# marlam/wurblpt

Measured on AMD Instinct MI355X. Metric: Msamples/s, higher is better.
Workload: dtype f32; 1 GPU; cornell_1024x1024_1024spp_ggx_glass; width=1024, height=1024, spp=1024, triangles=36, bvh_nodes=71, parallelism=1 launch

## Files before the change

### include/wurblpt_hip.h

```cpp
#ifndef WURBLPT_HIP_H
#define WURBLPT_HIP_H

#include <stdint.h>
#include <stddef.h>

#ifdef __cplusplus
extern "C" {
#endif

#define WPT_ABI_VERSION 5u

typedef enum {
    WPT_OK = 0,
    WPT_ERR_INVALID_ARGUMENT = 1,
    WPT_ERR_NO_DEVICE = 2,
    WPT_ERR_HIP = 3,
    WPT_ERR_UNSUPPORTED = 4,
    WPT_ERR_OUT_OF_MEMORY = 5
} wpt_status;


enum { WPT_NODE_INNER = 0, WPT_NODE_TRIANGLE = 1, WPT_NODE_SPHERE = 2, WPT_NODE_EMPTY = 3 };
typedef struct wpt_bvh_node {
    float lo[3];
// ... 392 lines not shown
wpt_status wpt_postproc_host(int op, const float* rgb_host, void* out_host, uint64_t pixels, float a, float b);

#define WPT_DENOISE_MAX_ITERATIONS 8u
#define WPT_DENOISE_MAX_NORMAL_LOG2 16u
typedef struct wpt_denoise_params {
    float sigma_l;
    float sigma_z;
    uint32_t normal_log2;
    uint32_t iterations;
} wpt_denoise_params;
wpt_status wpt_postproc_denoise(const float* frame_device, const float* moments_device, const uint16_t* samples_sqrt_device,
        const float* positions_device, const float* normals_device, const int32_t* materials_device, uint32_t width, uint32_t height,
        const wpt_denoise_params* params, float* out_device, float* variance_device, void* hip_stream);
wpt_status wpt_postproc_denoise_host(const float* frame_host, const float* moments_host, const uint16_t* samples_sqrt_host,
        const float* positions_host, const float* normals_host, const int32_t* materials_host, uint32_t width, uint32_t height,
        const wpt_denoise_params* params, float* out_host, float* variance_host);
const char* wpt_postproc_denoise_form(uint32_t step);

wpt_status wpt_first_hit_colours_device(wpt_scene* scene, const wpt_camera* camera, const wpt_params* params, uint32_t width,
        uint32_t height, float* albedo_device, float* emission_device, void* const guide_device[3], void* hip_stream);
wpt_status wpt_first_hit_colours(wpt_scene* scene, const wpt_camera* camera, const wpt_params* params, uint32_t width, uint32_t height,
        float* albedo_host, float* emission_host, void* const guide_host[3]);

wpt_status wpt_postproc_denoise_demodulated(const float* frame_device, const float* moments_device, const uint16_t* samples_sqrt_device,
        const float* positions_device, const float* normals_device, const int32_t* materials_device, const float* albedo_device,
        const float* emission_device, uint32_t width, uint32_t height, const wpt_denoise_params* params, float albedo_floor,
        float* out_device, float* variance_device, void* hip_stream);
wpt_status wpt_postproc_denoise_demodulated_host(const float* frame_host, const float* moments_host, const uint16_t* samples_sqrt_host,
        const float* positions_host, const float* normals_host, const int32_t* materials_host, const float* albedo_host,
        const float* emission_host, uint32_t width, uint32_t height, const wpt_denoise_params* params, float albedo_floor,
        float* out_host, float* variance_host);

#define WPT_TEMPORAL_HISTORY_BYTES_PER_PIXEL 48u
typedef struct wpt_temporal_params {
    float max_history;
    float normal_cos_min;
    float position_tolerance;
    uint32_t reserved;
} wpt_temporal_params;
wpt_status wpt_postproc_temporal_accumulate(const float* frame_device, const float* moments_device, const uint16_t* samples_sqrt_device,
        const float* positions_device, const float* normals_device, const int32_t* materials_device,
        const float* pixel_offset_to_prev_device, const float* camera_offset_to_prev_device, const void* history_prev_device,
        uint32_t width, uint32_t height, const wpt_temporal_params* params, void* history_out_device, float* length_out_device,
        void* hip_stream);
wpt_status wpt_postproc_temporal_accumulate_host(const float* frame_host, const float* moments_host, const uint16_t* samples_sqrt_host,
        const float* positions_host, const float* normals_host, const int32_t* materials_host, const float* pixel_offset_to_prev_host,
        const float* camera_offset_to_prev_host, const void* history_prev_host, uint32_t width, uint32_t height,
        const wpt_temporal_params* params, void* history_out_host, float* length_out_host);
wpt_status wpt_postproc_denoise_history(const void* history_device, uint32_t width, uint32_t height, const wpt_denoise_params* params,
        float* out_device, float* variance_device, void* hip_stream);
wpt_status wpt_postproc_denoise_history_host(const void* history_host, uint32_t width, uint32_t height, const wpt_denoise_params* params,
        float* out_host, float* variance_host);

wpt_status wpt_postproc_resample(const float* image_device, uint32_t width, uint32_t height, uint32_t components, uint32_t new_width,
        uint32_t new_height, float* out_device, void* hip_stream);
wpt_status wpt_postproc_resample_host(const float* image_host, uint32_t width, uint32_t height, uint32_t components, uint32_t new_width,
        uint32_t new_height, float* out_host);
wpt_status wpt_postproc_lens_warp(const float* image_device, uint32_t width, uint32_t height, uint32_t components, const wpt_camera* camera,
        int forward, float* out_device, void* hip_stream);
wpt_status wpt_postproc_lens_warp_host(const float* image_host, uint32_t width, uint32_t height, uint32_t components, const wpt_camera* camera,
        int forward, float* out_host);
wpt_status wpt_postproc_despeckle(const float* rgb_device, uint32_t width, uint32_t height, uint32_t components, float min_factor,
        float* out_device, void* hip_stream);
wpt_status wpt_postproc_despeckle_host(const float* rgb_host, uint32_t width, uint32_t height, uint32_t components, float min_factor,
        float* out_host);
wpt_status wpt_postproc_distance_to_coords(const float* distances_device, uint32_t width, uint32_t height, uint32_t components,
        const wpt_camera* camera, int pmd_space, float* coords_device, void* hip_stream);
wpt_status wpt_postproc_distance_to_coords_host(const float* distances_host, uint32_t width, uint32_t height, uint32_t components,
        const wpt_camera* camera, int pmd_space, float* coords_host);
const char* wpt_postproc_despeckle_form(void);
wpt_status wpt_set_despeckle_form(int form);
void wpt_postproc_image_ops_tile(uint32_t* width, uint32_t* height);

wpt_status wpt_set_launch_config(uint32_t threads_per_group, uint32_t variant);
wpt_status wpt_set_top_nodes(uint32_t nodes);
#define WPT_WALK_WIDE 1u
#define WPT_WALK_FULL_SHADOW 2u
#define WPT_WALK_COUNT_PRODUCT 4u
#define WPT_WALK_TRIANGLES_AS_GIVEN 8u
#define WPT_WALK_SELECT_CORNERS 16u
#define WPT_WALK_NO_FOLD 32u
#define WPT_WALK_NO_BYPASS 64u
#define WPT_WALK_SMALL_WORKGROUPS 128u
wpt_status wpt_set_walk(uint32_t flags);
wpt_status wpt_scene_folded_links(const wpt_scene* scene, uint32_t* folded);
wpt_status wpt_fold_plan(const wpt_scene_desc* desc, uint32_t* folded, uint32_t* lds_words);
wpt_status wpt_scene_bypassed_nodes(const wpt_scene* scene, uint32_t* count);
wpt_status wpt_bypass_plan(const wpt_scene_desc* desc, uint32_t* count, uint32_t* words);
wpt_status wpt_set_bypass(uint32_t mode);
#define WPT_SLICES_DECLINE_ODD 0x100u
wpt_status wpt_slices_plan(uint32_t block_size, uint32_t lanes_at_once, uint32_t samples_sqrt, uint32_t* units, uint32_t* rows);
wpt_status wpt_set_slices(uint32_t n);
wpt_status wpt_last_slice_stats(uint64_t* taken, uint64_t* continued);
wpt_status wpt_set_wavefront(uint32_t mode, uint32_t groups, uint32_t chunk, uint32_t flags);

#define WPT_SCHED_STATS 72
wpt_status wpt_set_scheduler_stats(unsigned long long* stats_device);

const char* wpt_kernel_name(void);
const char* wpt_kernel_form(void);
uint32_t wpt_kernel_workgroup(uint32_t* ordered_boxes);
wpt_status wpt_kernel_choice(uint32_t need, uint32_t sensor, uint32_t count, uint32_t node_count, uint32_t tri_count, uint32_t material_count,
        uint32_t scene_has_wide, uint32_t variant, uint32_t walk, const char** name, const char** form, uint32_t key[4],
        uint64_t* scene_lds_bytes, uint32_t* materials_in_lds);
wpt_status wpt_kernel_table_entry(uint32_t index, uint32_t key[4], const char** name);
enum { WPT_PLAN_WAVEFRONT, WPT_PLAN_WAVEFRONT_FALLS_BACK, WPT_PLAN_POOLED, WPT_PLAN_STRATEGY, WPT_PLAN_UNITS, WPT_PLAN_ROWS, WPT_PLAN_PASSES,
    WPT_PLAN_WORDS };
enum { WPT_STRATEGY_ONE_PASS, WPT_STRATEGY_TWO_PASSES, WPT_STRATEGY_ADAPTIVE_ORDER, WPT_STRATEGY_SLICED };
wpt_status wpt_launch_plan(uint32_t sensor, uint32_t count, uint32_t need, uint32_t scene_in_lds, uint32_t block_size, uint32_t samples_sqrt,
        uint32_t cu_count, uint32_t variant, uint32_t wavefront_mode, uint32_t slices, uint32_t plan[WPT_PLAN_WORDS]);
const char* wpt_device_name(int device);
uint32_t wpt_last_render_passes(void);
const char* wpt_build_info(void);

const char* wpt_last_error(void);

#ifdef __cplusplus
}
#endif

#endif
```

### wurblpt_amd/_abi.py

```python
import ctypes as C

WPT_ABI_VERSION = 5
WPT_OK = 0

NODE_INNER, NODE_TRIANGLE, NODE_SPHERE, NODE_EMPTY = 0, 1, 2, 3
MATF_TOF_LIGHT = 16
TOF_MAX_PHASES = 8
LIGHT_GROUPS_MAX, LIGHT_GROUP_NONE = 255, 0xff
VIEWS_MAX_PIXELS = 0x7fffffff
SPLIT_PIXELS_PER_LANE = 4
MAT_NONE, MAT_LAMBERTIAN, MAT_LIGHT_DIFFUSE, MAT_MIRROR, MAT_GGX, MAT_GLASS, MAT_MODPHONG, MAT_TWOSIDED, MAT_RGL, MAT_LIGHT_SPOT = range(10)


class BvhNode(C.Structure):
    _fields_ = [("lo", C.c_float * 3), ("hi", C.c_float * 3), ("link", C.c_uint32), ("kind", C.c_uint32)]


class TriGeom(C.Structure):
    _fields_ = [("v0", C.c_float * 3), ("instance", C.c_uint32), ("v1", C.c_float * 3), ("material", C.c_uint32),
                ("v2", C.c_float * 3), ("flags", C.c_uint32)]


class TriAttr(C.Structure):
    _fields_ = [("n0", C.c_float * 3), ("n1", C.c_float * 3), ("n2", C.c_float * 3),
# ... 156 lines not shown
    "wpt_scene_bypassed_nodes": (_I, [_P, _pU]),
    "wpt_render_block_device": (_I, _SCP + [_U] * 5 + [_P] * 3),
    "wpt_render_block": (_I, _SCP + [_U] * 5 + [_P]),
    "wpt_render_bands_device": (_I, [_P] * 3 + [_U] * 6 + [_P] * 3),
    "wpt_render_bands": (_I, [_P] * 3 + [_U] * 6 + [_P]),
    "wpt_render_transient_block_device": (_I, _SCP + [_P] + [_U] * 6 + [_P] * 3),
    "wpt_render_transient_block": (_I, _SCP + [_P] + [_U] * 6 + [_P] * 2),
    "wpt_render_light_groups_block_device": (_I, _SCP + [_P] + [_U] * 8 + [_P] * 3),
    "wpt_render_light_groups_block": (_I, _SCP + [_P] + [_U] * 8 + [_P] * 2),
    "wpt_render_tof_block_device": (_I, _SCP + [_TOF] + [_U] * 5 + [_P] * 2),
    "wpt_render_tof_block": (_I, _SCP + [_TOF] + [_U] * 5 + [_P]),
    "wpt_tof_accumulate_host": (_I, [_TOF, _U, _F, _F, _I, _P]),
    "wpt_render_views_device": (_I, [_P, _CAM, _U, _PAR, _U, _U, _U] + [_P] * 3),
    "wpt_render_views": (_I, [_P, _CAM, _U, _PAR, _U, _U, _U, _P]),
    "wpt_render_view_streams_device": (_I, [_P, _CAM, _P, _U, _PAR, _U, _U, _U] + [_P] * 3),
    "wpt_render_view_streams": (_I, [_P, _CAM, _P, _U, _PAR, _U, _U, _U, _P]),
    "wpt_render_split_device": (_I, _SCP + [_U] * 5 + [_P] * 4),
    "wpt_render_split": (_I, _SCP + [_U] * 5 + [_P] * 2),
    "wpt_split_plan": (_I, [_Q, _U, _U, _pU, _pU]),
    "wpt_render_adaptive_block_device": (_I, _SCP + [_U, _U, _P, _U, _U] + [_P] * 3),
    "wpt_render_adaptive_block": (_I, _SCP + [_U, _U, _P, _U, _U] + [_P] * 2),
    "wpt_ground_truth_device": (_I, [_P] * 6 + [_U, _U, _P, _P]),
    "wpt_ground_truth": (_I, [_P] * 6 + [_U, _U, _P]),
    "wpt_first_hit_colours_device": (_I, [_P] * 3 + [_U, _U] + [_P] * 4),
    "wpt_first_hit_colours": (_I, [_P] * 3 + [_U, _U] + [_P] * 3),
    "wpt_progress_covers": (_I, [_U, _U, _U]),
    "wpt_progress_begin": (_I, _SCP + [_U] * 5 + [_Q, _pP]),
    "wpt_progress_advance_device": (_I, [_P, _U, _P, _P]),
    "wpt_progress_advance": (_I, [_P, _U, _P]),
    "wpt_progress_rows_done": (_U, [_P]),
    "wpt_progress_rows_total": (_U, [_P]),
    "wpt_progress_preview_device": (_I, [_P, _P, _P]),
    "wpt_progress_preview": (_I, [_P, _P]),
    "wpt_progress_end": (None, [_P]),
    "wpt_progress_state_bytes": (_I, [_P, _pQ]),
    "wpt_progress_save": (_I, [_P, _P, _Q]),
    "wpt_progress_restore": (_I, [_P, _P, _Q, _CAM, _PAR, _Q, _pP]),
    "wpt_progress_state_info": (_I, [_P, _Q, C.POINTER(ProgressInfo)]),
    "wpt_postproc_to_srgb": (_I, [_P, _P, _Q, _P]),
    "wpt_postproc_max_luminance": (_I, [_P, _Q, _P, _P]),
    "wpt_postproc_uniform_rational_quantization": (_I, [_P, _P, _Q, _F, _F, _P]),
    "wpt_postproc_scale_luminance": (_I, [_P, _P, _Q, _F, _F, _P]),
    "wpt_postproc_host": (_I, [_I, _P, _P, _Q, _F, _F]),
    "wpt_postproc_mix_planes": (_I, [_P, _U, _Q, _Q, _P, _P, _P]),
    "wpt_postproc_mix_planes_host": (_I, [_P, _U, _Q, _Q, _P, _P]),
    "wpt_postproc_mean_planes": (_I, [_P, _U, _Q, _Q, _P, _P, _P]),
    "wpt_postproc_mean_planes_host": (_I, [_P, _U, _Q, _Q, _P, _P]),
    "wpt_postproc_merge_means": (_I, [_P, _U, _P, _U, _Q, _P, _P]),
    "wpt_postproc_merge_means_host": (_I, [_P, _U, _P, _U, _Q, _P]),
    "wpt_postproc_denoise": (_I, [_P] * 6 + [_U, _U, _DEN] + [_P] * 3),
    "wpt_postproc_denoise_host": (_I, [_P] * 6 + [_U, _U, _DEN] + [_P] * 2),
    "wpt_postproc_denoise_form": (_S, [_U]),
    "wpt_postproc_denoise_demodulated": (_I, [_P] * 8 + [_U, _U, _DEN, _F] + [_P] * 3),
    "wpt_postproc_denoise_demodulated_host": (_I, [_P] * 8 + [_U, _U, _DEN, _F] + [_P] * 2),
    "wpt_postproc_temporal_accumulate": (_I, [_P] * 9 + [_U, _U, _TMP] + [_P] * 3),
    "wpt_postproc_temporal_accumulate_host": (_I, [_P] * 9 + [_U, _U, _TMP] + [_P] * 2),
    "wpt_postproc_denoise_history": (_I, [_P, _U, _U, _DEN] + [_P] * 3),
    "wpt_postproc_denoise_history_host": (_I, [_P, _U, _U, _DEN] + [_P] * 2),
    "wpt_postproc_resample": (_I, [_P] + [_U] * 5 + [_P, _P]),
    "wpt_postproc_resample_host": (_I, [_P] + [_U] * 5 + [_P]),
    "wpt_postproc_lens_warp": (_I, _WARP + [_P]),
    "wpt_postproc_lens_warp_host": (_I, _WARP),
    "wpt_postproc_distance_to_coords": (_I, _WARP + [_P]),
    "wpt_postproc_distance_to_coords_host": (_I, _WARP),
    "wpt_postproc_despeckle": (_I, [_P, _U, _U, _U, _F, _P, _P]),
    "wpt_postproc_despeckle_host": (_I, [_P, _U, _U, _U, _F, _P]),
    "wpt_postproc_despeckle_form": (_S, []),
    "wpt_postproc_image_ops_tile": (None, [_pU, _pU]),
    "wpt_set_despeckle_form": (_I, [_I]),
    "wpt_set_launch_config": (_I, [_U, _U]),
    "wpt_set_wavefront": (_I, [_U] * 4),
    "wpt_set_walk": (_I, [_U]),
    "wpt_set_top_nodes": (_I, [_U]),
    "wpt_set_slices": (_I, [_U]),
    "wpt_set_bypass": (_I, [_U]),
    "wpt_set_scheduler_stats": (_I, [_P]),
    "wpt_slices_plan": (_I, [_U, _U, _U, _pU, _pU]),
    "wpt_last_slice_stats": (_I, [_pQ, _pQ]),
    "wpt_fold_plan": (_I, [_P, _pU, _P]),
    "wpt_bypass_plan": (_I, [_P, _pU, _P]),
    "wpt_kernel_name": (_S, []),
    "wpt_kernel_form": (_S, []),
    "wpt_kernel_workgroup": (_U, [_pU]),
    "wpt_kernel_choice": (_I, [_U] * 9 + [_pS, _pS, _pU, _pQ, _pU]),
    "wpt_kernel_table_entry": (_I, [_U, _pU, _pS]),
    "wpt_launch_plan": (_I, [_U] * 10 + [_pU]),
    "wpt_last_render_passes": (_U, []),
}

TEST_HOOK_FUNCTIONS = {
    "wpt_selftest_math": (_I, [_I, _I, _P, _P, _P]),
    "wpt_selftest_aabb": (_I, [_I, _P, _P, _P]),
    "wpt_selftest_triangle": (_I, [_I, _I, _P, _P]),
    "wpt_selftest_rayaux": (_I, [_I, _P, _P]),
    "wpt_selftest_sphere": (_I, [_I, _P, _P, _P]),
    "wpt_selftest_hits": (_I, [_P, _I, _P, _P]),
    "wpt_selftest_hits_host": (_I, [_P, _I, _P, _P]),
    "wpt_scene_get_envmap_tables": (_I, [_P] * 4),
}
```

### wurblpt_amd/csrc/wpt_blocks.h

```cpp
#ifndef WPT_BLOCKS_H
#define WPT_BLOCKS_H

#include "wpt_device.h"
#include "wpt_lens.h"
#include "wpt_tof.h"

namespace wptk {

using namespace wptd;

constexpr uint32_t NO_HIT = 0xffffffffu;

enum { RAY_PATH = 0, RAY_NEE_LIGHT = 1, RAY_NEE_ENV = 2, RAY_PATH_WAITED = 3  };
enum { NEXT_TRACE = 0, NEXT_NEW = 1, NEXT_DONE = 2, NEXT_WAIT = 3, NEXT_HANDED_ON = 4  };

enum { SEC_NODE_STEP = 0, SEC_LEAF_TEST, SEC_BEGIN_RAY, SEC_MISS, SEC_HIT_RECORD, SEC_SCATTER_LAMBERT, SEC_SCATTER_GGX, SEC_SCATTER_GLASS, SEC_SCATTER_OTHER,
       SEC_EMISSION, SEC_LIGHT_SAMPLE, SEC_PDF_SETUP, SEC_PDF_LIGHT, SEC_EVAL_LAMBERT, SEC_EVAL_GGX, SEC_EVAL_OTHER, SEC_NEE_SETUP, SEC_ADVANCE, SEC_NEE_END,
       SEC_NEE_END_LIGHT, SEC_NEW_SAMPLE, SEC_PIXEL_DONE, SEC_LOOK, SEC_LOOK_INNER, SEC_COUNT };

struct LaneCounters {
    uint32_t rays, nodes, leaves, pdfs, scatters;
    unsigned long long shadeClock[8];
    uint32_t secWave[SEC_COUNT], secLane[SEC_COUNT];
};
// ... 166 lines not shown
    return make_float4(faceNormal.x, faceNormal.y, faceNormal.z, faceArea);
}

template<bool FACE>
WPT_D float hotSpotPdfValue(float4 g0, float4 g1, float4 g2, f3 org, f3 dir, const RayAux& h, float4 face)
{
    const f3 v0 = mk3(g0.x, g0.y, g0.z), v1 = mk3(g1.x, g1.y, g1.z), v2 = mk3(g2.x, g2.y, g2.z);
    Candidate c;
    float value = 0.0f;
    if (triangleTest(v0, v1, v2, org, h, 0.0f, k_maxval, c)) {
        if (!FACE)
            face = hotSpotFace(v0, v1, v2);
        float cosine = __builtin_fabsf(dot(mk3(face.x, face.y, face.z), neg(dir)));
        float distance_squared = c.a * c.a;
        value = distance_squared / (cosine * face.w);
    }
    return value;
}

WPT_D float hotSpotPdfValueRotated(float4 g0, float4 g1, float4 g2, f3 orgR, f3 dir, const RayAux& h, float4 face)
{
    Candidate c;
    float value = 0.0f;
    if (triangleTestRotated(mk3(g0.x, g0.y, g0.z), mk3(g1.x, g1.y, g1.z), mk3(g2.x, g2.y, g2.z), orgR, h.Sx, h.Sy, h.inv.x,
            (uint32_t)h.k & (uint32_t)RAY_FLIP, 0.0f, k_maxval, c)) {
        float cosine = __builtin_fabsf(dot(mk3(face.x, face.y, face.z), neg(dir)));
        float distance_squared = c.a * c.a;
        value = distance_squared / (cosine * face.w);
    }
    return value;
}
WPT_D uint32_t rotatedCopyOffset(int kz, uint32_t triCount) { return (kz == 2 ? 0u : (uint32_t)(kz + 1)) * (3u * triCount); }

WPT_CALL float spherePdfValue(const wpt_sphere& sp, const wpt_sphere& spHit, f3 org, f3 dir)
{
    const f3 cmo = sub(ld3(sp.center), org);
    const float distanceSquared = dot(cmo, cmo);
    const float radiusSquared = sp.radius * sp.radius;
    float value = 0.0f;
    if (distanceSquared <= radiusSquared) {
        value = 0.25f * k_inv_pi;
    } else {
        float a;
        if (sphereTest(spHit, org, dir, 0.0f, k_maxval, a)) {
            const float discriminant = 1.0f - radiusSquared / distanceSquared;
            const float cosThetaMax = discriminant > 0.0f ? __builtin_sqrtf(discriminant) : 0.0f;
            const float solidAngle = 2.0f * k_pi * (1.0f - cosThetaMax);
            value = 1.0f / solidAngle;
        }
    }
    return value;
}

struct DirectionDraw {
    f3 dir;
    Prng prng;
};
WPT_CALL DirectionDraw sphereDirection(const wpt_sphere& sp, f3 org, Prng prng)
{
    DirectionDraw r;
    const f3 cmo = sub(ld3(sp.center), org);
    const float distanceSquared = dot(cmo, cmo);
    const float radiusSquared = sp.radius * sp.radius;
    if (distanceSquared <= radiusSquared) {
        r.dir = onUnitSphere(in01x2(prng));
    } else {
        const float discriminant = 1.0f - radiusSquared / distanceSquared;
        const float cosThetaMax = discriminant > 0.0f ? __builtin_sqrtf(discriminant) : 0.0f;
        r.dir = toSphere(normalize(cmo), cosThetaMax, in01x2(prng));
    }
    r.prng = prng;
    return r;
}

template<uint32_t F, bool COUNT, class Tri4>
WPT_D void hotSpotsMeanPdfPair(const SceneView& sv, Tri4 tri4, f3 org, f3 dirA, f3 dirB, PathHot& ps, LaneCounters& lc, float& meanA, float& meanB)
{
    if constexpr ((F & FEAT_ROTATED) != 0) {
        auto meanPdf = [&](f3 dir) {
            const RayAux h = rayAuxRotated<true>(dir);
            const f3 orgR = rotated(org, auxKz(h));
            const uint32_t off = rotatedCopyOffset(auxKz(h), sv.triCount);
            float sum = 0.0f;
            for (uint32_t i = 0; i < sv.hotspotCount; i++) {
                const uint32_t p = off + 3 * sv.hotspots[i].prim;
                sum += hotSpotPdfValueRotated(tri4(p), tri4(p + 1), tri4(p + 2), orgR, dir, h, sv.hotspotFace[i]);
            }
            return sum * here(sv.invHotspotCount);
        };
        meanA = meanPdf(dirA);
        meanB = meanPdf(dirB);
        return;
    }
    const RayAux hA = rayAux<true>(dirA), hB = rayAux<true>(dirB);
    float sumA = 0.0f, sumB = 0.0f;
    for (uint32_t i = 0; i < sv.hotspotCount; i++) {
        sec<COUNT>(lc, SEC_PDF_LIGHT);
        const uint32_t p = sv.hotspots[i].prim;
        if ((F & FEAT_SPHERES) && sv.hotspots[i].kind == WPT_HOTSPOT_SPHERE) {
            const wpt_sphere& sp = sv.spheres[p];
            if ((F & FEAT_ANIM) && sp.animation >= 0) {
                const wptanim::Trs T = animationTrs(sv, ps, sp.animation);
                const wpt_sphere forPdf = sphereMovedForPdf(sp, T), moved = sphereMoved(sp, T);
                sumA += spherePdfValue(forPdf, moved, org, dirA);
                sumB += spherePdfValue(forPdf, moved, org, dirB);
            } else {
                sumA += spherePdfValue(sp, sp, org, dirA);
                sumB += spherePdfValue(sp, sp, org, dirB);
            }
        } else if ((F & FEAT_ANIM) && sv.hotspots[i].animation >= 0) {
            float4 g0 = tri4(3 * p), g1 = tri4(3 * p + 1), g2 = tri4(3 * p + 2);
            const float* animationM = animationMatrix(sv, ps, sv.hotspots[i].animation);
            const f3 v0 = animatePoint(animationM, mk3(g0.x, g0.y, g0.z)), v1 = animatePoint(animationM, mk3(g1.x, g1.y, g1.z)),
                     v2 = animatePoint(animationM, mk3(g2.x, g2.y, g2.z));
            g0.x = v0.x; g0.y = v0.y; g0.z = v0.z;
            g1.x = v1.x; g1.y = v1.y; g1.z = v1.z;
            g2.x = v2.x; g2.y = v2.y; g2.z = v2.z;
            sumA += hotSpotPdfValue<false>(g0, g1, g2, org, dirA, hA, g0);
            sumB += hotSpotPdfValue<false>(g0, g1, g2, org, dirB, hB, g0);
        } else {
            const float4 g0 = tri4(3 * p), g1 = tri4(3 * p + 1), g2 = tri4(3 * p + 2), face = sv.hotspotFace[i];
            sumA += hotSpotPdfValue<true>(g0, g1, g2, org, dirA, hA, face);
            sumB += hotSpotPdfValue<true>(g0, g1, g2, org, dirB, hB, face);
        }
        if (COUNT)
            lc.pdfs += 2;
    }
    meanA = sumA * here(sv.invHotspotCount);
    meanB = sumB * here(sv.invHotspotCount);
}

template<class PS> WPT_D void accumulateRadiance(const wpt_params& par, f3 opl, float distanceToLight, f4 radiance, PS& ps)
{
    const bool dOk = distanceToLight >= par.min_dist_to_light && distanceToLight <= par.max_dist_to_light;
    if (!dOk)
        return;
    Slot acc = ps.get(SLOT_ACC);
    if (opl.x >= par.min_path_len && opl.x <= par.max_path_len)
        acc.x += radiance.x;
    if (opl.y >= par.min_path_len && opl.y <= par.max_path_len)
        acc.y += radiance.y;
    if (opl.z >= par.min_path_len && opl.z <= par.max_path_len)
        acc.z += radiance.z;
    ps.set3(SLOT_ACC, mk3(acc.x, acc.y, acc.z));
}

struct BinsView {
    const float* edges;
    float* bins;
    size_t stride;
    uint32_t binCount;
    uint32_t width;
    float guessScale;
    uint32_t rule;
};
enum : uint32_t {
    BINS_BY_EMITTER = 0x100u,
    BINS_GROUP_NONE = 0xffu
};

WPT_D int binOf(const BinsView& b, float x)
{
    const uint32_t K = b.binCount;
    if (!(x >= b.edges[0] && x < b.edges[K]))
        return -1;
    const float g = __builtin_fminf((x - b.edges[0]) * b.guessScale, (float)(K - 1));
    uint32_t k = (uint32_t)g;
    if (!(b.edges[k] <= x && x < b.edges[k + 1])) {
        uint32_t lo = 0, hi = K;
// ... 259 lines not shown
        }
        return NEXT_NEW;
    }
    Ray ray;
    ray.o = ps.o;
    ray.d = ps.d;
    ray.ri = ps.get4(SLOT_RI);
    const Slot oplSlot = ps.get(SLOT_OPL);
    const uint32_t pathComponent = oplSlot.w;
    const f3 opl = add(mk3(oplSlot.x, oplSlot.y, oplSlot.z), scl(best.a, sensorChannels<F>(ray.ri)));
    if (!(pathComponent + 1 < par.max_path_components))
        return NEXT_NEW;
    long long tSection = 0;
    auto section = [&](int k) {
        if (COUNT) {
            const long long now = clock64();
            lc.shadeClock[k] += (unsigned long long)(now - tSection);
            tSection = now;
        }
    };
    if (COUNT)
        tSection = clock64();
    sec<COUNT>(lc, SEC_HIT_RECORD);
    Hit h = finishHit<F>(sv, best, ray.o, ray.d, ps.time, tri4);
    const wpt_material& m = resolveMaterial<F>(sv, h.material, h);
    if ((F & ~(FEAT_GGX | FEAT_GLASS | FEAT_TRANSIENT | FEAT_ADAPTIVE | FEAT_ROTATED | FEAT_SLICED | ((F & FEAT_TOF) ? (FEAT_TOF | FEAT_SPOT | FEAT_TWOSIDED) : 0u))) == 0 && waitBelow > 0) {
        const bool waited = ps.rayKind == RAY_PATH_WAITED;
        const unsigned long long here = __ballot(true);
        bool wait = false;
        for (uint32_t kind = WPT_MAT_LAMBERTIAN; kind <= WPT_MAT_RGL; kind++) {
            if (kind == WPT_MAT_LIGHT_DIFFUSE || kind == WPT_MAT_TWOSIDED)
                continue;
            const unsigned long long lanes = __ballot(m.type == kind);
            if (lanes != 0 && lanes != here && __popcll(lanes) < waitBelow && __ballot(m.type == kind && waited) == 0 && m.type == kind)
                wait = true;
        }
        if (wait) {
            ps.rayKind = RAY_PATH_WAITED;
            return NEXT_WAIT;
        }
    }
    ps.set3(SLOT_OPL, opl);
    if (COUNT)
        lc.scatters++;
    section(0);
    sec<COUNT>(lc, SEC_SCATTER_LAMBERT, m.type == WPT_MAT_LAMBERTIAN);
    sec<COUNT>(lc, SEC_SCATTER_GGX, m.type == WPT_MAT_GGX);
    sec<COUNT>(lc, SEC_SCATTER_GLASS, m.type == WPT_MAT_GLASS || m.type == WPT_MAT_MIRROR);
    sec<COUNT>(lc, SEC_SCATTER_OTHER, m.type != WPT_MAT_LAMBERTIAN && m.type != WPT_MAT_GGX && m.type != WPT_MAT_GLASS && m.type != WPT_MAT_MIRROR && m.type != WPT_MAT_LIGHT_DIFFUSE
            && !((F & FEAT_SPOT) && m.type == WPT_MAT_LIGHT_SPOT));
    sec<COUNT>(lc, SEC_EMISSION);
    Prng prng = loadPrng(ps);
#ifdef WPT_MATERIAL_CACHE
    MatCache mc = matCacheEmpty();
    const Scatter sr = materialScatter<F>(sv, m, ray, h, prng, mc);
#else
    MatCache mcScatter = matCacheEmpty(), mc = matCacheEmpty();
    const Scatter sr = materialScatter<F>(sv, m, ray, h, prng, mcScatter);
#endif
    section(1);
    const f4 att = ps.get4(SLOT_ATT);
    {
        f4 rad = mul(att, materialEmitted<F>(sv, m, h, ray.d));
        accumulate<F>(par, bins, opl, (pathComponent == 0 ? 0.0f : h.a), rad, ps, isTofLight<F>(m), emitterOf<F>(m), sv.materials);
    }
    section(2);
    if (sr.type == SCATTER_NONE) {
        storePrng(ps, prng);
        return NEXT_NEW;
    }
    f4 nextAtt = mul(att, sr.att);
    if (sr.type == SCATTER_RANDOM) {
        if (sr.pdf > 0.0f)
            nextAtt = divs(nextAtt, sr.pdf);
        else
            nextAtt = mk4(0.0f, 0.0f, 0.0f, 0.0f);
    }
    sec<COUNT>(lc, SEC_LIGHT_SAMPLE, sr.type == SCATTER_RANDOM && sv.hotspotCount > 0);
    if (sr.type == SCATTER_RANDOM && sv.hotspotCount > 0) {
        uint32_t idx = (uint32_t)(in01(prng) * (float)sv.hotspotCount);
        idx = idx < sv.hotspotCount - 1 ? idx : sv.hotspotCount - 1;
        const wpt_hotspot& hs = sv.hotspots[idx];
        f3 directDir;
        uint32_t hotSpotPrim = hs.prim;
        if ((F & FEAT_SPHERES) && hs.kind == WPT_HOTSPOT_SPHERE) {
            const DirectionDraw draw = sphereDirection(sphereNow<F>(sv, ps, sv.spheres[hs.prim]), h.p, prng);
            directDir = draw.dir;
            prng = draw.prng;
            hotSpotPrim = PRIM_SPHERE | hs.prim;
        } else {
            const f3 bary = inTriangle(in01x2(prng));
            f3 p = add(add(scl(bary.x, ld3(hs.p0)), scl(bary.y, ld3(hs.p1))), scl(bary.z, ld3(hs.p2)));
            if (hs.transform)
                p = mat4mulPoint(hs.M, p);
            if ((F & FEAT_ANIM) && hs.animation >= 0)
                p = animatePoint(animationMatrix(sv, ps, hs.animation), p);
            directDir = normalize(sub(p, h.p));
        }
        section(4);
        float hotSpotsPdf, directPdf;
        sec<COUNT>(lc, SEC_PDF_SETUP);
        hotSpotsMeanPdfPair<F, COUNT>(sv, tri4, h.p, sr.dir, directDir, ps, lc, hotSpotsPdf, directPdf);
        nextAtt = sclr(nextAtt, powerHeuristicWeight(sr.pdf, hotSpotsPdf));
        section(5);
        sec<COUNT>(lc, SEC_EVAL_LAMBERT, directPdf > 0.0f && m.type == WPT_MAT_LAMBERTIAN);
        sec<COUNT>(lc, SEC_EVAL_GGX, directPdf > 0.0f && m.type == WPT_MAT_GGX);
        sec<COUNT>(lc, SEC_EVAL_OTHER, directPdf > 0.0f && m.type != WPT_MAT_LAMBERTIAN && m.type != WPT_MAT_GGX);
        if (directPdf > 0.0f) {
            float dpdf;
            f4 directAtt;
            materialEval<F>(sv, m, ray, h, directDir, directAtt, dpdf, mc);
            sec<COUNT>(lc, SEC_NEE_SETUP, dpdf > 0.0f);
            if (dpdf > 0.0f) {
                const f4 neeFactor = sclr(divs(mul(att, directAtt), directPdf), powerHeuristicWeight(directPdf, dpdf));
                const f3 neeChannels = sensorChannels<F>(neeFactor);
                Slot nee;
                nee.x = neeChannels.x; nee.y = neeChannels.y; nee.z = neeChannels.z;
                nee.w = hotSpotPrim;
                ps.set(SLOT_NEE, nee);
                if (MERGED) {
                    ps.set3(SLOT_NEXTATT, opl);
                    ps.set3(SLOT_SRDIR, mk3(ray.ri.x, ray.ri.y, ray.ri.z));
                    ps.neeO = h.p;
                    ps.neeD = directDir;
                    ps.neeKind = RAY_NEE_LIGHT;
                } else {
                    ps.set4(SLOT_NEXTATT, nextAtt);
                    ps.set3(SLOT_SRDIR, sr.dir);
                    storePrng(ps, prng);
                    ps.o = h.p;
                    ps.d = directDir;
                    ps.rayKind = RAY_NEE_LIGHT;
                    section(6);
                    return NEXT_TRACE;
                }
            }
        }
    } else if ((F & FEAT_ENVMAP) && sr.type == SCATTER_RANDOM && haveEnv && sv.envN > 0) {
        const float lightsP = envP(sv, sr.dir);
        nextAtt = sclr(nextAtt, powerHeuristicWeight(sr.pdf, lightsP));
        const f3 lightDir = envD(sv, prng);
        const float directPdf = envP(sv, lightDir);
        float dpdf;
        f4 directAtt;
        materialEval<F>(sv, m, ray, h, lightDir, directAtt, dpdf, mc);
        if (dpdf > 0.0f) {
            const f4 neeFactor = sclr(divs(mul(att, directAtt), directPdf), powerHeuristicWeight(directPdf, dpdf));
            ps.set3(SLOT_NEE, sensorChannels<F>(neeFactor));
            if (MERGED) {
                ps.neeO = h.p;
                ps.neeD = lightDir;
                ps.neeKind = RAY_NEE_ENV;
            } else {
                ps.set4(SLOT_NEXTATT, nextAtt);
                ps.set3(SLOT_SRDIR, sr.dir);
                storePrng(ps, prng);
                ps.o = h.p;
                ps.d = lightDir;
                ps.rayKind = RAY_NEE_ENV;
                section(7);
                return NEXT_TRACE;
            }
        }
    }
    sec<COUNT>(lc, SEC_ADVANCE);
    ps.o = h.p;
    if (sr.type == SCATTER_EXPLICIT)
        ps.set4(SLOT_RI, sr.ri);
    const int next = advancePath(par, ps, nextAtt, sr.dir, pathComponent, prng);
    storePrng(ps, prng);
    section(7);
    return next;
}

template<uint32_t F, class Tri4, class PS>
WPT_D int blockNeeEnd(const SceneView& sv, const wpt_params& par, Tri4 tri4, PS& ps, const Candidate& best, const BinsView& bins = BinsView{})
{
    const Slot oplSlot = ps.get(SLOT_OPL);
    if (ps.rayKind == RAY_NEE_LIGHT) {
        const Slot nee = ps.get(SLOT_NEE);
// ... 53 lines not shown
```

### wurblpt_amd/csrc/wpt_capi.hip

```cpp
#include <atomic>
#include <cstring>

#include "wpt_capi_common.h"
#include "wpt_scene_layout.h"
#include "wpt_leaf_words.h"
#include "wpt_streams.h"

using namespace wptd;
using namespace wptk;
using namespace wptc;

namespace {

thread_local std::string g_error;

std::atomic<uint32_t> g_lastPasses{1};
std::atomic<const char*> g_kernelName{nullptr};
std::atomic<const char*> g_kernelForm{""};

std::atomic<unsigned long long*> g_lastSliceStats{nullptr};

std::atomic<uint32_t> g_lastWorkgroup{uint32_t(WG)};

static_assert(wptk::PLAN_WG == uint32_t(WG) && wptk::PLAN_SLICE_SLOT_MAX == wptk::SLICE_SLOT_MASK && wptk::SLICE_UNITS_TARGET <= wptk::SLICE_UNITS_MAX
        && wptk::PLAN_FRAME == wptk::SENSOR_FRAME && wptk::PLAN_VIEWS == wptk::SENSOR_VIEWS && wptk::PLAN_ADAPTIVE == wptk::SENSOR_ADAPTIVE
        && wptk::PLAN_SENSORS == wptk::SENSOR_COUNT, "wpt_launch_plan.h restates the kernels' constants and the sensors");
static_assert(wptl::NODE_CHILD == NODE_CHILD && wptl::NODE_INDEX_MASK == NODE_INDEX_MASK && wptl::PRIM_SPHERE == PRIM_SPHERE && wptl::WIDE_STACK == WIDE_STACK
        && wptl::WIDE_NONE == WIDE_NONE && wptl::LDS_SCENE_MAX_BYTES == LDS_SCENE_MAX_BYTES && wptl::ORDERED_COPIES == wptk::ORDERED_COPIES,
        "wpt_scene_layout.h restates the kernels' node words and limits");
static_assert(wptw::LEAF_NODE_SHIFT == wptk::LEAF_NODE_SHIFT && wptw::LEAF_NODE_MAX == wptk::LEAF_NODE_MAX && wptw::LEAF_CORNER_MASK == wptk::LEAF_CORNER_MASK
        && LDS_SCENE_MAX_BYTES / 32 <= wptw::LEAF_NODE_MAX && LDS_SCENE_MAX_BYTES / 16 <= wptw::LEAF_CORNER_MASK,
        "wpt_leaf_words.h restates the rotated kernels' leaf word, which has room for every tree that fits LDS");

}

namespace wptc {

Settings settings;

wpt_status fail(wpt_status s, const std::string& msg)
{
    g_error = msg;
    return s;
}

void recordLaunch(const char* name, const char* form, uint32_t passes, unsigned long long* sliceStats)
{
    g_kernelName.store(name, std::memory_order_relaxed);
    g_kernelForm.store(form, std::memory_order_relaxed);
    g_lastPasses.store(passes, std::memory_order_relaxed);
    g_lastSliceStats.store(sliceStats, std::memory_order_relaxed);
    g_lastWorkgroup.store(uint32_t(WG), std::memory_order_relaxed);
}

void recordWorkgroup(uint32_t lanes, bool orderedBoxes)
{
    g_lastWorkgroup.store(lanes | (orderedBoxes ? 0x80000000u : 0u), std::memory_order_relaxed);
}

const char* kernelForm(bool rotated, uint32_t units, bool leafLinksFromNodes)
{
    static const std::vector<std::string> forms = [] {
        std::vector<std::string> f;
        for (int r = 0; r < 3; r++)
            for (uint32_t u = 0; u <= wptk::SLICE_UNITS_MAX; u++)
                f.push_back(std::string(r ? "rotated corners" : "") + (r == 2 ? ", leaf links from the nodes" : "")
                        + (u > 1 ? ", sliced x" + std::to_string(u) : std::string()));
        return f;
    }();
    return forms[(rotated ? (leafLinksFromNodes ? 2 : 1) * (wptk::SLICE_UNITS_MAX + 1) : 0) + (units <= wptk::SLICE_UNITS_MAX ? units : 0)].c_str();
}

wpt_status lookupKernel(uint32_t features, bool count, bool ldsScene, bool wide, const wptk::KernelEntry** entry)
{
    *entry = wptk::findKernel(features, count, ldsScene, wide);
    if (!*entry)
        return fail(WPT_ERR_UNSUPPORTED, "the library has no kernel wpt_pathtrace<F = " + std::to_string(features) + ", COUNT = " + std::to_string(count)
                + ", LDSSCENE = " + std::to_string(ldsScene) + ", WIDE = " + std::to_string(wide) + ">");
    return WPT_OK;
}

}

extern "C" {

int wpt_device_count(void)
{
    int n = 0;
    hipError_t e = hipGetDeviceCount(&n);
    if (e != hipSuccess) {
        g_error = std::string("hipGetDeviceCount: ") + hipGetErrorString(e);
        return 0;
    }
    return n;
}

wpt_status wpt_select_device(int device)
{
    HIP_TRY(hipSetDevice(device));
    return WPT_OK;
}

wpt_status wpt_current_device(int* device)
{
    if (!device)
        return fail(WPT_ERR_INVALID_ARGUMENT, "device is NULL");
    HIP_TRY(hipGetDevice(device));
    return WPT_OK;
}

const char* wpt_device_name(int device)
{
    thread_local std::string name;
    name.clear();
    hipDeviceProp_t prop;
    if (hipGetDeviceProperties(&prop, device) == hipSuccess)
        name = std::string(prop.name) + " (" + prop.gcnArchName + ", " + std::to_string(prop.multiProcessorCount) + " CUs)";
    return name.c_str();
}

wpt_status wpt_device_lanes(int device, uint32_t* lanes)
{
    if (!lanes)
        return fail(WPT_ERR_INVALID_ARGUMENT, "device lanes: NULL argument");
    hipDeviceProp_t prop;
    HIP_TRY(hipGetDeviceProperties(&prop, device));
    *lanes = uint32_t(prop.multiProcessorCount) * 1024u;
    return WPT_OK;
}

const char* wpt_build_info(void)
{
#if defined(__clang_version__)
    return "hipcc / clang " __clang_version__ ", --offload-arch=gfx950 -O3 -ffp-contract=off -fhip-fp32-correctly-rounded-divide-sqrt "
           "-fno-gpu-flush-denormals-to-zero";
#else
    return "unknown compiler";
#endif
}

const char* wpt_last_error(void)
{
    return g_error.c_str();
}

const char* wpt_kernel_name(void)
{
    const char* name = g_kernelName.load(std::memory_order_relaxed);
    return name ? name : "wpt_pathtrace";
}

const char* wpt_kernel_form(void)
{
    return g_kernelForm.load(std::memory_order_relaxed);
}

uint32_t wpt_kernel_workgroup(uint32_t* ordered_boxes)
{
    const uint32_t w = g_lastWorkgroup.load(std::memory_order_relaxed);
    if (ordered_boxes)
        *ordered_boxes = w >> 31;
    return w & 0x7fffffffu;
}

uint32_t wpt_last_render_passes(void)
{
    return g_lastPasses.load(std::memory_order_relaxed);
}

wpt_status wpt_last_slice_stats(uint64_t* taken, uint64_t* continued)
{
    if (!taken || !continued)
        return fail(WPT_ERR_INVALID_ARGUMENT, "NULL argument");
    *taken = 0;
    *continued = 0;
    const unsigned long long* stats = g_lastSliceStats.load(std::memory_order_relaxed);
    if (!stats)
        return WPT_OK;
    unsigned long long host[2] = { 0, 0 };
    HIP_TRY(hipDeviceSynchronize());
    HIP_TRY(hipMemcpy(host, stats, sizeof(host), hipMemcpyDeviceToHost));
    *taken = host[0];
    *continued = host[1];
    return WPT_OK;
}

wpt_status wpt_set_launch_config(uint32_t threads_per_group, uint32_t variant)
{
    if (threads_per_group != 0 && threads_per_group != WG)
        return fail(WPT_ERR_UNSUPPORTED, "this build uses 256 threads per workgroup");
    settings.threadsPerGroup = WG;
    settings.variant = variant & 0xffu;
    settings.leaveEighths = 0;
    settings.heavyMin = 0;
    settings.leafBias = 0;
    if ((variant >> 8) & 0xffu)
        settings.leaveEighths = ((variant >> 8) & 0xffu) - 1;
    if ((variant >> 16) & 0xffu)
        settings.heavyMin = ((variant >> 16) & 0xffu) - 1;
    if ((variant >> 24) & 0xffu)
        settings.leafBias = (variant >> 24) & 0xffu;
    return WPT_OK;
}

wpt_status wpt_set_wavefront(uint32_t mode, uint32_t groups, uint32_t chunk, uint32_t flags)
{
    if (mode > 2u)
        return fail(WPT_ERR_INVALID_ARGUMENT, "wavefront mode must be 0, 1 or 2");
    settings.wfMode = mode;
    settings.wfConfig.groups = groups & 0xffu;
    settings.wfConfig.tracePerCu = (groups >> 8) & 0xffu;
    settings.wfConfig.shadePerKind = (groups >> 16) & 1u;
    settings.wfConfig.chunk = chunk;
    settings.wfConfig.buckets = (flags & 1u) ? 0u : 1u;
    settings.wfConfig.refillIdle = (flags >> 8) & 0x3fu;
    settings.wfConfig.leafBias = 0;
    settings.wfConfig.stepBudget = (flags >> 16) == 0xffffu ? 0xffffffffu : (flags >> 16);
    settings.wfConfig.topNodes = ((flags >> 1) & 0x7fu) == 0x7fu ? 0xffffffffu : ((flags >> 1) & 0x7fu) * 128u;
    return WPT_OK;
}

wpt_status wpt_set_top_nodes(uint32_t nodes)
{
    settings.topNodes = nodes & 0x7fffffffu;
    return WPT_OK;
}

wpt_status wpt_set_walk(uint32_t flags)
{
    if (flags & ~(WPT_WALK_WIDE | WPT_WALK_FULL_SHADOW | WPT_WALK_COUNT_PRODUCT | WPT_WALK_TRIANGLES_AS_GIVEN | WPT_WALK_SELECT_CORNERS | WPT_WALK_NO_FOLD | WPT_WALK_NO_BYPASS
            | WPT_WALK_SMALL_WORKGROUPS))
        return fail(WPT_ERR_INVALID_ARGUMENT, "unknown walk flag");
    settings.walk = flags;
    return WPT_OK;
}

wpt_status wpt_set_slices(uint32_t n)
{
    if ((n & ~WPT_SLICES_DECLINE_ODD) > wptk::SLICE_UNITS_MAX)
        return fail(WPT_ERR_INVALID_ARGUMENT, "slices: 0 (the library's plan), 1 (never) or 2 .. 15 units, with or without WPT_SLICES_DECLINE_ODD");
    settings.slices = n;
    return WPT_OK;
}

wpt_status wpt_set_bypass(uint32_t mode)
{
    if (mode > wptb::MODE_ALL_ELIGIBLE)
        return fail(WPT_ERR_INVALID_ARGUMENT, "bypass mode: 0 (the cost model's choice) or 1 (every eligible inner node)");
    settings.bypassMode = mode;
    return WPT_OK;
}

wpt_status wpt_set_scheduler_stats(unsigned long long* stats_device)
{
    settings.schedStats = stats_device;
    return WPT_OK;
}

wpt_status wpt_slices_plan(uint32_t block_size, uint32_t lanes_at_once, uint32_t samples_sqrt, uint32_t* units, uint32_t* rows)
{
    if (!units || !rows)
        return fail(WPT_ERR_INVALID_ARGUMENT, "NULL argument");
    wptk::slicesPlan(block_size, lanes_at_once, samples_sqrt, units, rows);
    return WPT_OK;
}

wpt_status wpt_kernel_choice(uint32_t need, uint32_t sensor, uint32_t count, uint32_t node_count, uint32_t tri_count, uint32_t material_count,
        uint32_t scene_has_wide, uint32_t variant, uint32_t walk, const char** name, const char** form, uint32_t key[4],
        uint64_t* scene_lds_bytes, uint32_t* materials_in_lds)
{
    if (!name || !form || !key || !scene_lds_bytes || !materials_in_lds)
        return fail(WPT_ERR_INVALID_ARGUMENT, "NULL argument");
    if (sensor >= wptk::SENSOR_COUNT)
        return fail(WPT_ERR_INVALID_ARGUMENT, "sensor: 0 frame, 1 transient, 2 views, 3 adaptive, 4 time of flight");
    const wptk::KernelChoice choice = wptk::selectKernel({ need, wptk::Sensor(sensor), count != 0, node_count, tri_count, material_count,
            scene_has_wide != 0, variant, walk });
    const wptk::KernelEntry* kernel = nullptr;
    const wpt_status found = lookupKernel(choice.features, choice.count, choice.ldsScene, choice.wide, &kernel);
    if (found != WPT_OK)
        return found;
    *name = kernel->name;
    *form = kernelForm(choice.rotated);
    key[0] = kernel->features;
    key[1] = kernel->count;
    key[2] = kernel->ldsScene;
    key[3] = kernel->wide;
    *scene_lds_bytes = choice.sceneLdsBytes;
    *materials_in_lds = choice.materialsInLds;
    return WPT_OK;
}

wpt_status wpt_launch_plan(uint32_t sensor, uint32_t count, uint32_t need, uint32_t scene_in_lds, uint32_t block_size, uint32_t samples_sqrt,
        uint32_t cu_count, uint32_t variant, uint32_t wavefront_mode, uint32_t slices, uint32_t plan[WPT_PLAN_WORDS])
{
    if (!plan)
        return fail(WPT_ERR_INVALID_ARGUMENT, "NULL argument");
    if (sensor >= wptk::SENSOR_COUNT)
        return fail(WPT_ERR_INVALID_ARGUMENT, "sensor: 0 frame, 1 transient, 2 views, 3 adaptive, 4 time of flight");
    if (wavefront_mode > 2u)
        return fail(WPT_ERR_INVALID_ARGUMENT, "wavefront mode must be 0, 1 or 2");
    const wptk::LaunchPlan p = wptk::planLaunch({ sensor, count != 0, (need & FEAT_RGL) != 0, (need & FEAT_ANIM) != 0, scene_in_lds != 0,
            block_size, samples_sqrt, cu_count, variant, wavefront_mode, slices });
    const uint32_t words[WPT_PLAN_WORDS] = { p.wavefront, p.wavefrontFallBack, p.pooled, p.strategy, p.units, p.rows, p.passes };
    memcpy(plan, words, sizeof(words));
    return WPT_OK;
}

wpt_status wpt_kernel_table_entry(uint32_t index, uint32_t key[4], const char** name)
{
    if (!key || !name)
        return fail(WPT_ERR_INVALID_ARGUMENT, "NULL argument");
    if (index >= wptk::KERNEL_TABLE_ROWS)
        return fail(WPT_ERR_INVALID_ARGUMENT, "the kernel table has " + std::to_string(wptk::KERNEL_TABLE_ROWS) + " rows");
    const wptk::KernelEntry& k = wptk::KERNEL_TABLE[index];
// ... 19 lines not shown
```

### wurblpt_amd/csrc/wpt_capi_common.h

```cpp
#ifndef WPT_CAPI_COMMON_H
#define WPT_CAPI_COMMON_H

#include <hip/hip_runtime.h>

#include <cassert>
#include <cstdint>
#include <string>
#include <vector>

#include "../../include/wurblpt_hip.h"
#ifndef WPT_CAPI_OUTPUT_SIDE
#include "wpt_kernel_table.h"
#include "wpt_launch_plan.h"
#include "wpt_wavefront.inc.h"
#include "wpt_bypass.h"
#endif

namespace wptc __attribute__((visibility("hidden"))) {

wpt_status fail(wpt_status s, const std::string& msg);

#define HIP_TRY(expr)                                                                              \
    do {                                                                                           \
        hipError_t e_ = (expr);                                                                    \
        if (e_ != hipSuccess)                                                                      \
            return fail(WPT_ERR_HIP, std::string(#expr) + ": " + hipGetErrorString(e_));           \
    } while (0)
#define WPT_TRY(expr)                                                                              \
    do {                                                                                           \
        const wpt_status s_ = (expr);                                                              \
        if (s_ != WPT_OK)                                                                          \
            return s_;                                                                             \
    } while (0)

inline wpt_status hipStatus(const char* what, hipError_t e, bool oomToo = false)
{
    if (e == hipSuccess)
        return WPT_OK;
    return fail(oomToo && e == hipErrorOutOfMemory ? WPT_ERR_OUT_OF_MEMORY : WPT_ERR_HIP, std::string(what) + ": " + hipGetErrorString(e));
}

inline bool overlaps(const void* a, size_t bytesA, const void* b, size_t bytesB)
{
    const uintptr_t x = reinterpret_cast<uintptr_t>(a), y = reinterpret_cast<uintptr_t>(b);
    return x < y + bytesB && y < x + bytesA;
}

struct StreamScratch {
    hipStream_t stream;
    void* held[5] = {};
    uint32_t count = 0;
    explicit StreamScratch(hipStream_t s) : stream(s) {}
    StreamScratch(const StreamScratch&) = delete;
    ~StreamScratch()
    {
        for (uint32_t i = 0; i < count; i++)
            (void)hipFreeAsync(held[i], stream);
    }
    template<typename T> hipError_t get(size_t n, T** p)
    {
        assert(count < sizeof(held) / sizeof(held[0]));
        const hipError_t e = hipMallocAsync(reinterpret_cast<void**>(p), n * sizeof(T), stream);
        if (e == hipSuccess)
            held[count++] = *p;
        return e;
    }
    template<typename T> T* get(size_t n)
    {
        T* p = nullptr;
        if (get(n, &p) != hipSuccess) {
            (void)hipGetLastError();
            return nullptr;
        }
        return p;
    }
};

#ifndef WPT_CAPI_OUTPUT_SIDE

}

struct wpt_scene {
    int device;
    wptd::SceneView view;
    uint32_t features;
    uint32_t nodeCount, triCount;
    uint32_t foldedLinks;
    uint32_t* ldsLinks = nullptr;
    bool leafOneToOne = false;
    const float4* orderedNodes = nullptr;
    uint32_t bypassedNodes = 0;
    uint32_t animationCount;
    std::vector<void*> allocations;
    int cuCount;
    std::vector<float> envM, envMcs;
    std::vector<int32_t> envMs;
};

namespace wptc __attribute__((visibility("hidden"))) {

struct Settings {
    uint32_t threadsPerGroup = wptk::WG;
    uint32_t variant = 0;
    uint32_t leaveEighths = 0;
    uint32_t heavyMin = 0;
    uint32_t leafBias = 0;
    uint32_t topNodes = 65536;
    unsigned long long* schedStats = nullptr;
    uint32_t wfMode = 0;
    wptk::WfConfig wfConfig = { 0, 0, 0, 1, 0, 0, 0, 0, 0 };
    uint32_t walk = 0;
    uint32_t bypassMode = wptb::MODE_MODEL;
    uint32_t slices = 0;
};
extern Settings settings;

void recordLaunch(const char* name, const char* form, uint32_t passes, unsigned long long* sliceStats);
void recordWorkgroup(uint32_t lanes, bool orderedBoxes);
const char* kernelForm(bool rotated, uint32_t units = 0, bool leafLinksFromNodes = false);
wpt_status lookupKernel(uint32_t features, bool count, bool ldsScene, bool wide, const wptk::KernelEntry** entry);

struct LaunchRequest {
    wpt_scene* scene;
    const wpt_camera* camera;
    const wpt_params* params;
    uint32_t width, height, samplesSqrt, blockStart, blockSize;
    float* frame;
    void* stream;
    wpt_counters* counters = nullptr;
    uint32_t bandPixels = 0, bandFirst = 0, bandStride = 0;
    wptk::Sensor sensor = wptk::SENSOR_FRAME;
    wptk::BinsView bins = {};
    wptk::ViewsView views = {};
    wptk::AdaptiveView adaptive = {};
};

wpt_status checkFrameBlock(uint32_t width, uint32_t height, const uint32_t* samplesSqrt, uint32_t blockStart, uint32_t blockSize,
        uint32_t frames = 1, const char* prefix = "", bool session = false);
wpt_status launchSetUp(const wpt_scene* scene, const wpt_camera* camera, uint32_t cameraCount, bool batch, const wpt_params* params,
        uint32_t width, uint32_t height, uint32_t samples_sqrt, uint32_t block_start, uint32_t block_size,
        uint32_t band_pixels, uint32_t band_first, uint32_t band_stride, bool count, wptk::KernelArgs& args, uint32_t& need);
hipError_t runSingleKernel(const wpt_scene* scene, wptk::KernelArgs& args, const wptk::KernelChoice& choice, const wptk::KernelEntry* kernel,
        const wptk::KernelEntry* slicedTwin, const wptk::LaunchPlan& plan, hipStream_t stream);
wpt_status renderLaunch(const LaunchRequest& rq);

constexpr size_t ORDER_WORK_WORDS = 3 * wptk::ORDER_BUCKETS + 1;

inline void orderByCost(const wptk::KernelArgs& measured, uint32_t* order, uint32_t* work, hipStream_t stream, wptk::KernelArgs& next)
{
    wptk::launchOrderBuild(measured, order, work, stream);
    next.order = order;
    next.orderCount = work + ORDER_WORK_WORDS - 1;
}

struct StagedBlock {
    void* device = nullptr;
    size_t bytes = 0;
    StagedBlock() = default;
    StagedBlock(const StagedBlock&) = delete;
    ~StagedBlock() { (void)hipFree(device); }
    hipError_t allocate(size_t n) { return hipMalloc(&device, bytes = n); }
    hipError_t allocatePixels(size_t pixels, size_t planes = 1) { return allocate(pixels * 3 * sizeof(float) * planes); }
    hipError_t upload(const void* host) { return hipMemcpy(device, host, bytes, hipMemcpyHostToDevice); }
    hipError_t download(void* host) const { return device ? hipMemcpy(host, device, bytes, hipMemcpyDeviceToHost) : hipSuccess; }
    float* biased(uint32_t blockStart) const { return device ? static_cast<float*>(device) - size_t(blockStart) * 3 : nullptr; }
};

inline wpt_status finishStaged(wpt_status launched, wpt_scene* check, const StagedBlock& a, void* hostA, const StagedBlock* b = nullptr, void* hostB = nullptr)
{
    const wpt_status st = launched == WPT_OK && check ? wpt_scene_check(check) : launched;
    hipError_t e = st == WPT_OK ? a.download(hostA) : hipSuccess;
    if (st == WPT_OK && e == hipSuccess && b)
        e = b->download(hostB);
    return e == hipSuccess ? st : hipStatus("hipMemcpy", e);
}

#endif

}

#endif
```

### wurblpt_amd/csrc/wpt_capi_render.hip

```cpp
#include <atomic>

#include "wpt_capi_common.h"
#include "wpt_leaf_words.h"

using namespace wptd;
using namespace wptk;
using namespace wptc;

namespace {

constexpr int SLICE_STATS_DEVICES = 64;
std::atomic<unsigned long long*> g_sliceStats[SLICE_STATS_DEVICES];

unsigned long long* sliceStatsOfCurrentDevice()
{
    int dev = 0;
    if (hipGetDevice(&dev) != hipSuccess || dev < 0 || dev >= SLICE_STATS_DEVICES)
        return nullptr;
    unsigned long long* p = g_sliceStats[dev].load(std::memory_order_acquire);
    if (!p) {
        if (hipMalloc(reinterpret_cast<void**>(&p), 2 * sizeof(unsigned long long)) != hipSuccess) {
            (void)hipGetLastError();
            return nullptr;
        }
// ... 76 lines not shown
    if ((session && blockSize == 0) || uint64_t(blockStart) + blockSize > uint64_t(width) * height * frames)
        return fail(WPT_ERR_INVALID_ARGUMENT, std::string(prefix) + (session ? "pixel block is empty or lies outside the frame"
                : "pixel block lies outside the frame"));
    return WPT_OK;
}

wpt_status launchSetUp(const wpt_scene* scene, const wpt_camera* camera, uint32_t cameraCount, bool batch, const wpt_params* params,
        uint32_t width, uint32_t height, uint32_t samples_sqrt, uint32_t block_start, uint32_t block_size,
        uint32_t band_pixels, uint32_t band_first, uint32_t band_stride, bool count, wptk::KernelArgs& args, uint32_t& need)
{
    args.bandPixels = band_pixels;
    args.bandFirst = band_first;
    args.bandStride = band_stride;
    args.sv = scene->view;
    args.cam = *camera;
    args.par = *params;
    args.width = width;
    args.height = height;
    args.samplesSqrt = samples_sqrt;
    args.invWidth = 1.0f / float(width);
    args.invHeight = 1.0f / float(height);
    args.invSamplesSqrt = 1.0f / float(samples_sqrt);
    args.invSamples = 1.0f / float(samples_sqrt * samples_sqrt);
    args.blockStart = block_start;
    args.blockSize = block_size;
    args.fuse = (settings.variant & 0x20u) ? 0u : 1u;

    args.tiled = (width % 8 == 0 && block_start % width == 0 && block_size % (8 * width) == 0
            && (band_stride == 0 || band_pixels % (8 * width) == 0)) ? 1u : 0u;
    if (batch)
        args.tiled = (width % 8 == 0 && height % 8 == 0) ? 1u : 0u;
    need = scene->features;
    for (uint32_t v = 0; v < cameraCount; v++) {
        const wpt_camera* c = camera + v;
        need |= (c->lens_radius > 0.0f || c->distortion_type != WPT_DISTORTION_NONE || c->surround_mode != WPT_SURROUND_OFF
                || c->stereoscopic_distance > 0.0f) ? FEAT_LENS : 0u;
        if (c->surround_mode > WPT_SURROUND_360)
            return fail(WPT_ERR_UNSUPPORTED, "camera surround mode is not known to the kernel");
        if (c->distortion_type > WPT_DISTORTION_OPENCV)
            return fail(WPT_ERR_UNSUPPORTED, "lens distortion model is not known to the kernel");
        if (c->animation >= int32_t(scene->animationCount))
            return fail(WPT_ERR_INVALID_ARGUMENT, batch ? "camera " + std::to_string(v) + " refers to an animation outside the scene's array"
                    : std::string("camera refers to an animation outside the scene's array"));
        if (batch && c->animation >= 0)
            need |= FEAT_ANIM;
    }
    if (params->t0 != params->t1)
        need |= FEAT_ANIM;
    args.shadowWalksEnd = (settings.walk & WPT_WALK_FULL_SHADOW) ? 0u : (count ? ((settings.walk & WPT_WALK_COUNT_PRODUCT) ? 1u : 0u) : 1u);
    const bool smallScene = size_t(scene->nodeCount) * 32 + size_t(scene->triCount) * 48 <= LDS_SCENE_MAX_BYTES;
    args.leaveEighths = settings.leaveEighths ? (settings.leaveEighths > 8u ? 8u : settings.leaveEighths) : (smallScene ? 1u : 3u);
    args.heavyMin = settings.heavyMin ? settings.heavyMin : (smallScene ? 16u : 8u);
    args.leafBias = settings.leafBias ? settings.leafBias : (smallScene ? 16u : 32u);
    static const uint32_t waitBelowChoices[4] = { 6u, 0u, 3u, 12u };
    args.waitBelow = waitBelowChoices[(settings.variant >> 2) & 0x3u];
    args.cuCount = uint32_t(scene->cuCount);
    return WPT_OK;
}

hipError_t runSingleKernel(const wpt_scene* scene, wptk::KernelArgs& args, const wptk::KernelChoice& choice, const wptk::KernelEntry* kernel,
        const wptk::KernelEntry* slicedTwin, const wptk::LaunchPlan& plan, hipStream_t stream)
{
    StreamScratch scratch(stream);
    args.pool = plan.pooled ? scratch.get<uint32_t>(1) : nullptr;
    args.materialsInLds = choice.materialsInLds;
    if (choice.ldsScene) {
        if (!scene->ldsLinks)
            return hipErrorInvalidValue;
        const size_t words = 2 * size_t(scene->nodeCount) + 4;
        const bool fold = (choice.materialsInLds & wptk::LDS_FOLD) != 0;
        const bool bypass = fold && !(settings.walk & WPT_WALK_NO_BYPASS) && !args.sv.boxesMayBeNan;
        args.sv.spheres = reinterpret_cast<const wpt_sphere*>(scene->ldsLinks + (fold ? words : 0));
        args.sv.wideNodes = reinterpret_cast<const float4*>(scene->ldsLinks + (bypass ? 2 * words : fold ? words : 0));
        if (choice.rotated) {
            const size_t leafWords = wptw::leafWordsSize(scene->nodeCount, scene->triCount);
            const uint32_t* sets = scene->ldsLinks + 3 * words;
            args.sv.spheres = reinterpret_cast<const wpt_sphere*>(sets + (fold ? leafWords : 0));
            args.sv.wideNodes = reinterpret_cast<const float4*>(sets + (bypass ? 2 * leafWords : fold ? leafWords : 0));
            if (scene->leafOneToOne)
                args.materialsInLds |= wptk::LDS_LEAF_LINKS;
        }
    }
    size_t largeLdsBytes = 0;
    const bool large = wptk::selectLargeForm(choice, settings.walk, scene->orderedNodes != nullptr, args.sv.boxesMayBeNan != 0, scene->nodeCount, &largeLdsBytes);
    if (large && wptk::LARGE_ORDERED)
        args.sv.rglData = reinterpret_cast<const float*>(scene->orderedNodes);
    const SingleKernel run = large
            ? SingleKernel{ wptk::launchPathtraceLarge<FEAT_BASIC | FEAT_ROTATED>, dim3((args.blockSize + WG_LARGE - 1) / WG_LARGE), largeLdsBytes, stream }
            : SingleKernel{ kernel->launch, dim3((args.blockSize + WG - 1) / WG), choice.sceneLdsBytes, stream };
    bool done = false;
    unsigned long long* sliceStats = nullptr;
    if (args.pool && plan.strategy == wptk::TWO_PASSES)
        done = runTwoPasses(args, run, scratch);
    else if (args.pool && plan.strategy == wptk::ADAPTIVE_ORDER)
        done = runAdaptiveOrder(args, run, scratch);
    else if (args.pool && plan.strategy == wptk::SLICED)
        done = (sliceStats = runSliced(args, SingleKernel{ large ? wptk::launchPathtraceLarge<FEAT_BASIC | FEAT_ROTATED | FEAT_SLICED> : slicedTwin->launch, run.grid, run.sceneLdsBytes, stream },
                plan, scratch)) != nullptr;
    if (!done)
        run(args);
    recordLaunch(kernel->name, kernelForm(choice.rotated, sliceStats ? plan.units : 0, choice.rotated && !scene->leafOneToOne), done ? plan.passes : 1u,
            sliceStats);
    if (large)
        recordWorkgroup(WG_LARGE, wptk::LARGE_ORDERED);
    return hipGetLastError();
}

wpt_status renderLaunch(const LaunchRequest& rq)
{
    const bool planes = rq.sensor == wptk::SENSOR_TRANSIENT || rq.sensor == wptk::SENSOR_TOF, views = rq.sensor == wptk::SENSOR_VIEWS;
    if (!rq.scene || !rq.camera || !rq.params || !(rq.frame || planes))
        return fail(WPT_ERR_INVALID_ARGUMENT, "NULL argument");
    const uint32_t cameraCount = views ? rq.views.viewCount : 1u;
    const wpt_status checked = checkFrameBlock(rq.width, rq.height, &rq.samplesSqrt, rq.blockStart, rq.bandStride ? 0u : rq.blockSize, cameraCount);
    if (checked != WPT_OK || rq.blockSize == 0)
        return checked;
    KernelArgs args = {};
    uint32_t need = 0;
    const bool count = rq.counters != nullptr;
    WPT_TRY(launchSetUp(rq.scene, rq.camera, cameraCount, views, rq.params, rq.width, rq.height, rq.samplesSqrt, rq.blockStart,
            rq.blockSize, rq.bandPixels, rq.bandFirst, rq.bandStride, count, args, need));
    args.frame = rq.frame;
    args.counters = rq.counters;
    args.schedStats = settings.schedStats;
    if (views)
        args.views = rq.views;
    else if (rq.sensor == wptk::SENSOR_ADAPTIVE)
        args.adaptive = rq.adaptive;
    else if (planes)
        args.bins = rq.bins;
    args.rowStop = rq.samplesSqrt;
    const wptk::KernelChoice choice = wptk::selectKernel({ need, rq.sensor, count, rq.scene->nodeCount, rq.scene->triCount,
            uint32_t(rq.scene->view.materialCount), rq.scene->view.wideNodes != nullptr, settings.variant, settings.walk });
    const wptk::KernelEntry *kernel = nullptr, *slicedTwin = nullptr;
    wpt_status found = lookupKernel(choice.features, choice.count, choice.ldsScene, choice.wide, &kernel);
    if (found == WPT_OK && choice.sceneInLds && rq.sensor == wptk::SENSOR_FRAME && !count)
        found = lookupKernel(choice.features | FEAT_SLICED, choice.count, choice.ldsScene, choice.wide, &slicedTwin);
    if (found != WPT_OK)
        return found;
    const bool rgl = (need & FEAT_RGL) != 0;
    hipStream_t stream = static_cast<hipStream_t>(rq.stream);
    const wptk::LaunchPlan plan = wptk::planLaunch({ rq.sensor, count, rgl, (need & FEAT_ANIM) != 0, choice.sceneInLds, rq.blockSize, rq.samplesSqrt,
            uint32_t(rq.scene->cuCount), settings.variant, settings.wfMode, settings.slices });
    if (plan.wavefront) {
        uint32_t launches = 0;
        const hipError_t e = wptk::renderWavefront(args, rgl ? wptk::wfFullRgl() : (choice.basic ? wptk::wfBasic() : wptk::wfFull()), settings.wfConfig, stream, &launches);
        if (e == hipSuccess) {
            recordLaunch("wf_trace + wf_shade", "", launches, nullptr);
            return WPT_OK;
        }
        if (!plan.wavefrontFallBack || e != hipErrorOutOfMemory)
            return hipStatus("wavefront render", e, true);
        (void)hipGetLastError();
    }
    HIP_TRY(runSingleKernel(rq.scene, args, choice, kernel, slicedTwin, plan, stream));
    return WPT_OK;
}

}

extern "C" {

wpt_status wpt_render_block_device(wpt_scene* scene, const wpt_camera* camera, const wpt_params* params,
        uint32_t width, uint32_t height, uint32_t samples_sqrt, uint32_t block_start, uint32_t block_size,
        float* frame_device, wpt_counters* counters_device, void* hip_stream)
{
    LaunchRequest rq = { scene, camera, params, width, height, samples_sqrt, block_start, block_size, frame_device, hip_stream };
    rq.counters = counters_device;
    return renderLaunch(rq);
}

wpt_status wpt_render_bands_device(wpt_scene* scene, const wpt_camera* camera, const wpt_params* params,
        uint32_t width, uint32_t height, uint32_t samples_sqrt, uint32_t band_rows, uint32_t first_band, uint32_t band_stride,
        float* frame_device, wpt_counters* counters_device, void* hip_stream)
{
    if (band_rows == 0 || band_stride == 0 || first_band >= band_stride || width == 0 || height == 0)
        return fail(WPT_ERR_INVALID_ARGUMENT, "bands need band_rows > 0 and first_band < band_stride");
    const uint64_t bandPixels = uint64_t(band_rows) * width;
    const uint64_t bands = (uint64_t(height) + band_rows - 1) / band_rows;
    const uint64_t mine = first_band < bands ? (bands - first_band + band_stride - 1) / band_stride : 0;
    if (bandPixels > 0xffffffffull || mine * bandPixels > 0xffffffffull)
        return fail(WPT_ERR_INVALID_ARGUMENT, "bands too large");
    LaunchRequest rq = { scene, camera, params, width, height, samples_sqrt, 0, uint32_t(mine * bandPixels), frame_device, hip_stream };
    rq.bandPixels = uint32_t(bandPixels);
    rq.bandFirst = first_band;
    rq.bandStride = band_stride;
    rq.counters = counters_device;
// ... 41 lines not shown
```

### wurblpt_amd/csrc/wpt_capi_scene.hip

```cpp
#include <cstring>
#include <memory>

#include "wpt_capi_common.h"
#include "wpt_scene_layout.h"
#include "wpt_leaf_words.h"

using namespace wptd;
using namespace wptk;
using namespace wptc;

namespace {

__global__ void wpt_env_importance_kernel(SceneView sv, int N, float* importance)
{
    int i = blockIdx.x * blockDim.x + threadIdx.x;
    if (i >= N * N)
        return;
    int x = i % N, y = i / N;
    f2 uv;
    uv.y = ((float)y + 0.5f) / (float)N;
    uv.x = ((float)x + 0.5f) / (float)N;
    f4 L = envL(sv, envInvM(uv));
    importance[i] = L.x + L.y + L.z + L.w;
}
// ... 145 lines not shown
    for (uint32_t i = 0; i < d->sphere_count; i++)
        if (d->spheres[i].animation >= 0)
            f |= FEAT_ANIM;
    return f;
}

wpt_status validate(const wpt_scene_desc* d)
{
    return layoutStatus(wptl::validate(d));
}

}

extern "C" {

wpt_status wpt_scene_upload(const wpt_scene_desc* desc, wpt_scene** out_scene)
{
    if (!out_scene)
        return fail(WPT_ERR_INVALID_ARGUMENT, "out_scene is NULL");
    *out_scene = nullptr;
    WPT_TRY(validate(desc));
    if (wpt_device_count() <= 0)
        return fail(WPT_ERR_NO_DEVICE, "no HIP device is available; the path tracer has no CPU fallback");
    const uint32_t walk = settings.walk, topNodes = settings.topNodes;
    std::unique_ptr<wpt_scene, SceneFree> owner(new wpt_scene);
    wpt_scene* s = owner.get();
    SceneView& view = s->view;
    HIP_TRY(hipGetDevice(&s->device));
    s->features = sceneFeatures(desc);
    s->nodeCount = desc->node_count;
    s->triCount = desc->tri_count;
    memset(&view, 0, sizeof(view));
    const std::vector<uint32_t> triNew = wptl::triangleOrder(desc, (walk & WPT_WALK_TRIANGLES_AS_GIVEN) != 0);
    const bool fitsLds = size_t(desc->node_count) * 32 + size_t(desc->tri_count) * 48 <= LDS_SCENE_MAX_BYTES;
    std::vector<uint32_t> ldsNodes;
    {
        wptl::DeviceNodes nodes;
        WPT_TRY(layoutStatus(wptl::deviceNodes(desc, triNew, topNodes, &nodes)));
        view.nodeCount = desc->node_count;
        view.boxesMayBeNan = nodes.boxesMayBeNan;
        WPT_TRY(uploadQuads(s, nodes.quads, &view.nodes));
        s->foldedLinks = 0;
        if (fitsLds) {
            s->foldedLinks = wptl::countFoldedLinks(reinterpret_cast<const uint32_t*>(nodes.quads.data()), desc->node_count, nullptr);
            ldsNodes.resize(size_t(desc->node_count) * 8);
            memcpy(ldsNodes.data(), nodes.quads.data(), ldsNodes.size() * 4);
        }
    }
    if (walk & WPT_WALK_WIDE) {
        const std::vector<wptl::Quad> wide = wptl::wideNodes(desc, triNew);
        if (!wide.empty())
            WPT_TRY(uploadQuads(s, wide, &view.wideNodes));
    }
    {
        const std::vector<wpt_tri_geom> g = wptl::permuted(desc->tri_geom, triNew);
        WPT_TRY(uploadArray(s, reinterpret_cast<const float4*>(g.data()), size_t(desc->tri_count) * 3, &view.triGeom));
        if (fitsLds) {
            const wptb::Plan plan = wptb::plan(ldsNodes.data(), desc->node_count, g.data(), desc->tri_count, settings.bypassMode);
            std::vector<uint32_t> words(plan.plain);
            words.insert(words.end(), plan.folded.begin(), plan.folded.end());
            words.insert(words.end(), plan.bypass.begin(), plan.bypass.end());
            s->leafOneToOne = true;
            for (const std::vector<uint32_t>* links : { &plan.plain, &plan.folded, &plan.bypass }) {
                const wptw::LeafWords leaf = wptw::leafWords(links->data(), desc->node_count, desc->tri_count);
                if (leaf.verdict == wptw::TOO_LARGE)
                    return fail(WPT_ERR_UNSUPPORTED, "a tree that fits LDS has indices beyond its leaf words");
                s->leafOneToOne = s->leafOneToOne && leaf.verdict == wptw::ONE_TO_ONE;
                words.insert(words.end(), leaf.words.begin(), leaf.words.end());
            }
            const uint32_t* onDevice = nullptr;
            WPT_TRY(uploadArray(s, words.data(), words.size(), &onDevice));
            s->ldsLinks = const_cast<uint32_t*>(onDevice);
            s->bypassedNodes = plan.outCount;
            std::vector<wptl::Quad> ordered;
            if (wptl::orderedBoxCopies(ldsNodes.data(), desc->node_count, &ordered))
                WPT_TRY(uploadQuads(s, ordered, &s->orderedNodes));
        }
    }
    {
        const std::vector<wpt_tri_attr> a = wptl::permuted(desc->tri_attr, triNew);
        WPT_TRY(uploadArray(s, reinterpret_cast<const float4*>(a.data()), size_t(desc->tri_count) * 6, &view.triAttr));
    }
    WPT_TRY(uploadArray(s, desc->instances, desc->instance_count, &view.instances));
    WPT_TRY(uploadArray(s, desc->materials, desc->material_count, &view.materials));
    view.materialCount = desc->material_count;
    {
        size_t texelCount = 0;
        const std::vector<wpt_texture> devTex = wptl::texelOffsets(desc, &texelCount);
        WPT_TRY(uploadArray(s, devTex.data(), devTex.size(), &view.textures));
        WPT_TRY(decodeTexels(s, desc, devTex, texelCount));
    }
    {
        const std::vector<wpt_hotspot> h = wptl::remappedHotspots(desc, triNew);
        WPT_TRY(uploadArray(s, h.data(), h.size(), &view.hotspots));
    }
    WPT_TRY(uploadArray(s, desc->spheres, desc->sphere_count, &view.spheres));
    WPT_TRY(uploadArray(s, desc->rgl_brdfs, desc->rgl_count, &view.rglBrdfs));
    {
        const wptl::RglPool rgl = wptl::rglPool(desc);
        WPT_TRY(uploadArray(s, rgl.pool.data(), rgl.pool.size(), &view.rglData));
        WPT_TRY(uploadArray(s, rgl.rgbl.data(), rgl.rgbl.size(), &view.rglRgbl));
    }
    WPT_TRY(uploadArray(s, desc->animations, desc->animation_count, &view.animations));
    WPT_TRY(uploadArray(s, desc->keyframes, desc->keyframe_count, &view.keyframes));
    s->animationCount = desc->animation_count;
    view.sphereCount = desc->sphere_count;
    for (int k = 0; k < 6; k++)
        view.envCube[k] = desc->envmap.cube_tex[k];
    {
        hipDeviceProp_t prop;
        s->cuCount = hipGetDeviceProperties(&prop, s->device) == hipSuccess ? prop.multiProcessorCount : 256;
    }
    view.triCount = desc->tri_count;
    view.hotspotCount = desc->hotspot_count;
    view.invHotspotCount = desc->hotspot_count ? 1.0f / float(desc->hotspot_count) : 0.0f;
    if (desc->hotspot_count > 0)
        WPT_TRY(hotspotFaces(s));
    view.envType = desc->envmap.type;
    view.envCompat = desc->envmap.compat;
    view.envTex = desc->envmap.tex;
    view.envN = 0;
    view.envLog2N = -1;
    if (desc->envmap.type != WPT_ENV_NONE && desc->envmap.N > 0) {
        const int N = desc->envmap.N;
        const size_t bins = size_t(N) * N;
        if (desc->envmap.M && desc->envmap.Ms && desc->envmap.Mcs) {
            s->envM.assign(desc->envmap.M, desc->envmap.M + bins);
            s->envMs.assign(desc->envmap.Ms, desc->envmap.Ms + bins);
            s->envMcs.assign(desc->envmap.Mcs, desc->envmap.Mcs + bins);
        } else {
            std::vector<float> importance;
            WPT_TRY(envImportance(view, N, &importance));
            wptl::EnvTables t = wptl::envTablesFromImportance(importance.data(), bins);
            s->envM.swap(t.M);
            s->envMs.swap(t.Ms);
            s->envMcs.swap(t.Mcs);
        }
        WPT_TRY(uploadArray(s, s->envM.data(), bins, &view.envM));
        WPT_TRY(uploadArray(s, s->envMs.data(), bins, &view.envMs));
        WPT_TRY(uploadArray(s, s->envMcs.data(), bins, &view.envMcs));
        const std::vector<int32_t> lut = wptl::envStartTable(s->envMcs.data(), bins);
        if (!lut.empty()) {
            WPT_TRY(uploadArray(s, lut.data(), lut.size(), &view.envLut));
            view.envLutSize = wptl::ENV_LUT_SIZE;
        }
        view.envN = N;
        view.envLog2N = wptl::envLog2(N);
    }
    *out_scene = owner.release();
    return WPT_OK;
}

void wpt_scene_free(wpt_scene* scene)
{
    if (!scene)
        return;
    for (void* p : scene->allocations)
        (void)hipFree(p);
    delete scene;
}

wpt_status wpt_scene_get_envmap_tables(const wpt_scene* scene, float* M, int32_t* Ms, float* Mcs)
{
    if (!scene || scene->view.envN <= 0)
        return fail(WPT_ERR_INVALID_ARGUMENT, "scene has no importance tables");
    size_t bins = scene->envM.size();
// ... 68 lines not shown
```

### wurblpt_amd/csrc/wpt_device.h

```cpp
#ifndef WPT_DEVICE_H
#define WPT_DEVICE_H

#include <hip/hip_runtime.h>
#include <stdint.h>

#include "../../include/wurblpt_hip.h"
#include "wpt_math.h"
#include "wpt_triangle.h"
#include "wpt_anim.h"
#include "wpt_rgl.h"

namespace wptd {

#define WPT_CALL static inline __device__ __attribute__((noinline))


WPT_D float dot(f2 a, f2 b) { float d = 0.0f; d += a.x * b.x; d += a.y * b.y; return d; }
WPT_D float dot(f3 a, f3 b) { float d = 0.0f; d += a.x * b.x; d += a.y * b.y; d += a.z * b.z; return d; }
WPT_D f3 normalize(f3 v) { return divs(v, __builtin_sqrtf(dot(v, v))); }
WPT_D f3 cross(f3 v, f3 w) { return mk3(v.y * w.z - v.z * w.y, v.z * w.x - v.x * w.z, v.x * w.y - v.y * w.x); }
WPT_D f3 reflect(f3 i, f3 n) { return sub(i, scl(2.0f * dot(n, i), n)); }
WPT_D f3 refract(f3 i, f3 n, float eta)
{
    const float d = dot(n, i);
    const float k = 1.0f - eta * eta * (1.0f - d * d);
    if (k <= 0.0f)
        return mk3(0.0f, 0.0f, 0.0f);
    return sub(sclr(i, eta), sclr(n, eta * d + __builtin_sqrtf(k)));
}
WPT_D float max4(f4 a)
{
    float r = a.x;
    if (a.y > r) r = a.y;
    if (a.z > r) r = a.z;
    if (a.w > r) r = a.w;
    return r;
}
WPT_D float average3(f3 a)
{
    const float inv_N = 1.0f / 3.0f;
    float sum = 0.0f;
    sum += a.x; sum += a.y; sum += a.z;
    return inv_N * sum;
}

WPT_D f3 mat3mul(const float* m, f3 w)
{
    f3 r;
    r.x = 0.0f; r.x += m[0] * w.x; r.x += m[3] * w.y; r.x += m[6] * w.z;
    r.y = 0.0f; r.y += m[1] * w.x; r.y += m[4] * w.y; r.y += m[7] * w.z;
    r.z = 0.0f; r.z += m[2] * w.x; r.z += m[5] * w.y; r.z += m[8] * w.z;
    return r;
}
WPT_D f3 mat4mulPoint(const float* m, f3 p)
{
    f3 r;
    r.x = 0.0f; r.x += m[0] * p.x; r.x += m[4] * p.y; r.x += m[8] * p.z; r.x += m[12] * 1.0f;
    r.y = 0.0f; r.y += m[1] * p.x; r.y += m[5] * p.y; r.y += m[9] * p.z; r.y += m[13] * 1.0f;
    r.z = 0.0f; r.z += m[2] * p.x; r.z += m[6] * p.y; r.z += m[10] * p.z; r.z += m[14] * 1.0f;
    return r;
}
WPT_D f3 quatRotate(const float* q, f3 v)
{
    f3 s = mk3(q[0], q[1], q[2]);
    f3 t = scl(2.0f, cross(s, v));
    return add(add(v, scl(q[3], t)), cross(s, t));
}

struct Prng {
    uint32_t s0, s1, s2, s3;
};
WPT_D uint64_t splitmix64(uint64_t x)
{
    uint64_t z = (x += 0x9e3779b97f4a7c15ull);
    z = (z ^ (z >> 30)) * 0xbf58476d1ce4e5b9ull;
    z = (z ^ (z >> 27)) * 0x94d049bb133111ebull;
    return z ^ (z >> 31);
}
WPT_D void prngSeed(Prng& p, uint64_t index)
{
    uint64_t seed = index + 42ull;
    uint64_t s01 = splitmix64(seed);
    uint64_t s23 = splitmix64(s01);
    p.s0 = (uint32_t)(s01 >> 32);
    p.s1 = (uint32_t)(s01 & 0xffffffffull);
    p.s2 = (uint32_t)(s23 >> 32);
    p.s3 = (uint32_t)(s23 & 0xffffffffull);
}
WPT_D void prngSeed(Prng& p, uint32_t pixelIndex)
{
    prngSeed(p, (uint64_t)pixelIndex);
}
// ... 294 lines not shown
    for (int k = 0; k < 3; k++)
        r.center[k] = sp.center[k] + T.t[k];
    r.radius = sp.radius * m;
    const float x = sp.rotation[0], y = sp.rotation[1], z = sp.rotation[2], w = sp.rotation[3];
    const float qx = T.q[0], qy = T.q[1], qz = T.q[2], qw = T.q[3];
    r.rotation[0] = w * qx + x * qw + y * qz - z * qy;
    r.rotation[1] = w * qy + y * qw + z * qx - x * qz;
    r.rotation[2] = w * qz + z * qw + x * qy - y * qx;
    r.rotation[3] = w * qw - x * qx - y * qy - z * qz;
    return r;
}
template<uint32_t F> WPT_D wpt_sphere sphereAt(const SceneView& sv, const wpt_sphere& sp, float time)
{
    if ((F & FEAT_ANIM) && sp.animation >= 0)
        return sphereMoved(sp, animationAt(sv, sp.animation, time));
    return sp;
}
struct SphereScene {
    const wpt_sphere* spheres;
    const wpt_animation* animations;
    const wpt_keyframe* keyframes;
};
WPT_D SphereScene sphereScene(const SceneView& sv)
{
    SphereScene v;
    v.spheres = sv.spheres;
    v.animations = sv.animations;
    v.keyframes = sv.keyframes;
    return v;
}
WPT_D wpt_sphere sphereMovedForPdf(const wpt_sphere& sp, const wptanim::Trs& T)
{
    wpt_sphere r = sp;
    float m = T.s[0];
    if (T.s[1] > m)
        m = T.s[1];
    if (T.s[2] > m)
        m = T.s[2];
    wptanim::applyTrs(T, sp.center, r.center);
    r.radius = sp.radius * m;
    return r;
}

#ifdef WPT_SPHERE_HIT_INLINE
#define WPT_SPHERE_HIT WPT_D
#else
#define WPT_SPHERE_HIT static __device__ __attribute__((noinline))
#endif
template<uint32_t F = 0> WPT_SPHERE_HIT Hit finishSphereHit(SphereScene sv, Candidate c, f3 org, f3 dir, float time = 0.0f)
{
    wpt_sphere sp = sv.spheres[c.prim & ~PRIM_SPHERE];
    if ((F & FEAT_ANIM) && sp.animation >= 0) {
        const wpt_animation a = sv.animations[sp.animation];
        sp = sphereMoved(sp, wptanim::at<DeviceAnimMath>(sv.keyframes + a.first_keyframe, a.keyframe_count, time));
    }
    Hit h;
    h.a = c.a;
    h.prim = c.prim;
    h.material = sp.material;
    h.p = add(org, scl(c.a, dir));
    f3 n = normalize(sub(h.p, ld3(sp.center)));
    const f3 rn = quatRotate(sp.rotation, n);
    const float alpha = wptm::atan2f_(rn.x, rn.z);
    const float beta = wptm::asinf_(clampr(rn.y, -1.0f, +1.0f));
    h.tc.x = 0.5f * k_inv_pi * (alpha + k_pi);
    h.tc.y = k_inv_pi * (beta + 0.5f * k_pi);
    f3 t = mk3(wptm::cosf_(alpha), 0.0f, -wptm::sinf_(alpha));
    if (__builtin_fabsf(dot(rn, t)) >= k_cosOrthoAngleTolerance)
        t = mk3(0.0f, 0.0f, 0.0f);
    h.backside = false;
    if (dot(n, neg(dir)) < 0.0f) {
        h.backside = true;
        n = neg(n);
    }
    h.n = n;
    h.t = t;
    return h;
}

struct TriGeomFromScene {
    const float4* triGeom;
    WPT_D float4 operator()(uint32_t i) const { return triGeom[i]; }
};
template<uint32_t F = 0, class Tri4 = TriGeomFromScene>
WPT_D Hit finishHit(const SceneView& sv, const Candidate& c, f3 org, f3 dir, float time, Tri4 tri4)
{
    if ((F & FEAT_SPHERES) && (c.prim & PRIM_SPHERE))
        return finishSphereHit<F>(sphereScene(sv), c, org, dir, time);
    Hit h;
    h.a = c.a;
    h.prim = c.prim;
    uint32_t instance, flags;
    if constexpr ((F & FEAT_ROTATED) != 0) {
        (void)tri4;
        const uint32_t* words = reinterpret_cast<const uint32_t*>(sv.triGeom + 3 * (size_t)c.prim);
        instance = words[3];
        h.material = words[7];
        flags = words[11];
    } else {
        const float4 g0 = tri4(3 * c.prim + 0);
        const float4 g1 = tri4(3 * c.prim + 1);
        const float4 g2 = tri4(3 * c.prim + 2);
        instance = __float_as_uint(g0.w);
        h.material = __float_as_uint(g1.w);
        flags = __float_as_uint(g2.w);
    }
    const bool backfacing = c.invDet < 0.0f;
    const float bx = c.invDet * c.U, by = c.invDet * c.V, bz = c.invDet * c.W;
    h.p = add(org, scl(c.a, dir));
    const float4* at = sv.triAttr + 6 * (size_t)c.prim;
    const float4 a0 = at[0], a1 = at[1], a2 = at[2], a3 = at[3], a4 = at[4], a5 = at[5];
    const f3 n0 = mk3(a0.x, a0.y, a0.z), n1 = mk3(a0.w, a1.x, a1.y), n2 = mk3(a1.z, a1.w, a2.x);
    f3 nrm = add(add(scl(bx, n0), scl(by, n1)), scl(bz, n2));
    const bool transform = (flags & WPT_TRI_TRANSFORM) != 0;
    const float* N = sv.instances[instance].N;
    if (transform)
        nrm = mat3mul(N, nrm);
    float animationN[9];
    const bool animate = (F & FEAT_ANIM) && (flags & WPT_TRI_ANIMATE);
    if (animate) {
        const wptanim::Trs T = animationAt(sv, sv.instances[instance].animation, time);
        wptanim::toMat3(T.q, animationN);
        nrm = mat3mul(animationN, nrm);
    }
    nrm = normalize(nrm);
    if (backfacing)
        nrm = neg(nrm);
    h.n = nrm;
    h.tc.x = 0.0f;
    h.tc.y = 0.0f;
    if (flags & WPT_TRI_HAVE_TEXCOORDS) {
        h.tc.x = bx * a2.y + by * a2.w + bz * a3.y;
        h.tc.y = bx * a2.z + by * a3.x + bz * a3.z;
    }
    f3 tan = mk3(0.0f, 0.0f, 0.0f);
    if (flags & WPT_TRI_HAVE_TANGENTS) {
        const f3 t0 = mk3(a3.w, a4.x, a4.y), t1 = mk3(a4.z, a4.w, a5.x), t2 = mk3(a5.y, a5.z, a5.w);
        tan = add(add(scl(bx, t0), scl(by, t1)), scl(bz, t2));
        if (dot(tan, tan) > 0.0f) {
            if (transform)
                tan = mat3mul(N, tan);
            if (animate)
                tan = mat3mul(animationN, tan);
            tan = normalize(sub(tan, scl(dot(nrm, tan), nrm)));
        }
    }
    h.t = tan;
    h.backside = backfacing;
    return h;
}
template<uint32_t F = 0>
WPT_D Hit finishHit(const SceneView& sv, const Candidate& c, f3 org, f3 dir, float time = 0.0f)
{
    TriGeomFromScene fromScene;
    fromScene.triGeom = sv.triGeom;
    return finishHit<F>(sv, c, org, dir, time, fromScene);
}

WPT_D float srgbToRgb(float x)
{
    return (x <= 0.04045f ? (x * (1.0f / 12.92f)) : wptm::powf_((x + 0.055f) * (1.0f / 1.055f), 2.4f));
}

WPT_D f4 imageTexelDecode(const uint8_t* pool, const wpt_texture& t, size_t x, size_t y)
{
    const uint8_t* base = pool + t.texel_offset;
    const size_t idx = (y * (size_t)t.width + x) * t.comps;
    float d[4] = { 0.0f, 0.0f, 0.0f, 0.0f };
    const bool lin = t.linearize_srgb != 0;
    for (uint32_t k = 0; k < t.comps; k++) {
        float raw;
        if (t.texel_type == WPT_TEXEL_U8)
            raw = (float)base[idx + k] / 255.0f;
        else if (t.texel_type == WPT_TEXEL_U16)
            raw = (float)((const uint16_t*)base)[idx + k] / 65535.0f;
        else
            raw = ((const float*)base)[idx + k];
        const bool isAlpha = (t.comps == 2 && k == 1) || (t.comps == 4 && k == 3);
        d[k] = (lin && !isAlpha) ? srgbToRgb(raw) : raw;
    }
    if (t.comps == 3)
        return mk4(d[0], d[1], d[2], 1.0f);
    if (t.comps == 4)
        return mk4(d[0], d[1], d[2], d[3]);
    if (t.comps == 1)
        return mk4(d[0], d[0], d[0], 1.0f);
    return mk4(d[0], d[0], d[0], d[1]);
}

WPT_D f4 imageTexel(const SceneView& sv, const wpt_texture& t, size_t x, size_t y)
{
    if (x >= t.width)
        x = t.width - 1;
    if (y >= t.height)
        y = t.height - 1;
    const float4 v = sv.texels4[t.texel_offset + y * (size_t)t.width + x];
    return mk4(v.x, v.y, v.z, v.w);
}

WPT_D f4 mix4(f4 a, f4 b, float k)
{
    return mk4(mixr(a.x, b.x, k), mixr(a.y, b.y, k), mixr(a.z, b.z, k), mixr(a.w, b.w, k));
}

WPT_D f4 textureValue(const SceneView& sv, int tex, f2 tc)
{
    int chain[4];
    int depth = 0;
    const wpt_texture* t = sv.textures + tex;
    while (t->type == WPT_TEX_TRANSFORMER && depth < 4) {
        tc.x = t->coord_factor[0] * tc.x + t->coord_offset[0];
        tc.y = t->coord_factor[1] * tc.y + t->coord_offset[1];
        chain[depth++] = tex;
        tex = t->child;
        t = sv.textures + tex;
    }
    f4 val;
    if (t->type == WPT_TEX_CONSTANT) {
        val = ld4(t->a);
    } else if (t->type == WPT_TEX_CHECKER) {
        int row = (int)(tc.y * (float)(int)t->height);
        int col = (int)(tc.x * (float)(int)t->width);
        val = (row % 2 == col % 2) ? ld4(t->a) : ld4(t->b);
    } else {
// ... 734 lines not shown
```

### wurblpt_amd/csrc/wpt_kernel_table.h

```cpp
#ifndef WPT_KERNEL_TABLE_H
#define WPT_KERNEL_TABLE_H

#include "wpt_pathtrace.inc.h"

namespace wptk {

struct KernelEntry {
    uint32_t features;
    bool count, ldsScene, wide;
    void (*launch)(const KernelArgs&, dim3 grid, size_t sceneLdsBytes, hipStream_t);
    const char* name;
};

#define WPT_KERNEL_ROW(F, COUNT, LDSSCENE, WIDE, NAME) { (F), COUNT, LDSSCENE, WIDE, launchPathtrace<(F), COUNT, LDSSCENE, WIDE>, NAME }
static const KernelEntry KERNEL_TABLE[] = {
    WPT_KERNEL_ROW(FEAT_BASIC, false, true, false, "wpt_pathtrace"),
    WPT_KERNEL_ROW(FEAT_BASIC | FEAT_ROTATED, false, true, false, "wpt_pathtrace"),
    WPT_KERNEL_ROW(FEAT_BASIC | FEAT_SLICED, false, true, false, "wpt_pathtrace"),
    WPT_KERNEL_ROW(FEAT_BASIC | FEAT_ROTATED | FEAT_SLICED, false, true, false, "wpt_pathtrace"),
    WPT_KERNEL_ROW(FEAT_BASIC, false, false, false, "wpt_pathtrace"),
    WPT_KERNEL_ROW(FEAT_BASIC, true, false, false, "wpt_pathtrace"),
    WPT_KERNEL_ROW(FEAT_ALL, false, false, false, "wpt_pathtrace"),
    WPT_KERNEL_ROW(FEAT_ALL, false, false, true, "wpt_pathtrace, wide walk"),
    WPT_KERNEL_ROW(FEAT_ALL, true, false, false, "wpt_pathtrace"),
// ... 44 lines not shown
    uint32_t need;
    Sensor sensor;
    bool count;
    uint32_t nodeCount, triCount, materialCount;
    bool sceneHasWide;
    uint32_t variant;
    uint32_t walk;
};

struct KernelChoice {
    uint32_t features;
    bool count, ldsScene, wide;
    bool basic;
    bool sceneInLds;
    bool rotated;
    uint32_t materialsInLds;
    size_t sceneLdsBytes;
};

inline KernelChoice selectKernel(const KernelFacts& f)
{
    const bool frame = f.sensor == SENSOR_FRAME, tof = f.sensor == SENSOR_TOF, count = f.count;
    const uint32_t force = f.variant & 0x3u;
    const bool rgl = (f.need & FEAT_RGL) != 0;
    const bool anim = (f.need & FEAT_ANIM) != 0;
    const size_t sceneBytes = size_t(f.nodeCount) * 32 + size_t(f.triCount) * 48;
    const size_t ldsBytes = sceneBytes + 32;
    const bool lds = sceneBytes <= LDS_SCENE_MAX_BYTES && force != 1;
    const bool basic = (f.need & ~(tof ? FEAT_BASIC | FEAT_SPOT | FEAT_TWOSIDED : FEAT_BASIC)) == 0 && force != 2;
    const bool ldsSensor = basic && lds && !anim && !rgl;
    const bool wide = f.sceneHasWide && frame && !count && !anim && !(basic && lds);
    const size_t rotatedBytes = ldsBytes + 2 * size_t(f.triCount) * 48;
    const bool rotated = frame && ldsSensor && !count && !(f.walk & WPT_WALK_SELECT_CORNERS)
            && COLD_BYTES + rotatedBytes <= LDS_BYTES_PER_WORKGROUP_AT_FOUR;

    KernelChoice c = {};
    c.basic = basic;
    c.sceneInLds = ldsSensor;
    c.rotated = rotated;
    c.count = count;
    const uint32_t all = rgl ? FEAT_ALL | FEAT_RGL | FEAT_ANIM : anim ? FEAT_ALL | FEAT_ANIM : FEAT_ALL;
    switch (f.sensor) {
    case SENSOR_TOF:
    case SENSOR_TRANSIENT: {
        const uint32_t sensor = tof ? FEAT_TOF : FEAT_TRANSIENT;
        c.ldsScene = ldsSensor;
        c.features = sensor | (ldsSensor ? (tof ? FEAT_BASIC | FEAT_TWOSIDED | FEAT_SPOT : FEAT_BASIC) : all);
        break;
    }
    case SENSOR_ADAPTIVE:
    case SENSOR_VIEWS:
        c.ldsScene = ldsSensor && !count;
        c.features = (f.sensor == SENSOR_VIEWS ? FEAT_VIEWS : FEAT_ADAPTIVE) | (c.ldsScene ? FEAT_BASIC : (rgl || anim) ? all : basic ? FEAT_BASIC : FEAT_ALL);
        break;
    default:
        if (anim) {
            c.features = rgl ? FEAT_ALL | FEAT_RGL | FEAT_ANIM : FEAT_ALL | FEAT_ANIM;
        } else if (count) {
            c.features = basic ? FEAT_BASIC : rgl ? FEAT_ALL | FEAT_RGL : FEAT_ALL;
        } else if (rgl) {
            c.features = FEAT_ALL | FEAT_RGL;
            c.wide = wide;
        } else if (basic && lds) {
            c.features = rotated ? FEAT_BASIC | FEAT_ROTATED : FEAT_BASIC;
            c.ldsScene = true;
        } else if (wide) {
            c.features = FEAT_ALL;
            c.wide = true;
        } else {
            c.features = basic ? FEAT_BASIC : FEAT_ALL;
        }
        break;
    }
    const size_t materialBytes = size_t(f.materialCount) * sizeof(wpt_material);
    const size_t sceneLdsBytes = rotated ? rotatedBytes : ldsBytes;
    if (!(f.variant & 0x80u) && COLD_BYTES + sceneLdsBytes + materialBytes <= LDS_BYTES_PER_WORKGROUP_AT_FOUR)
        c.materialsInLds = LDS_MATERIALS;
    c.sceneLdsBytes = !c.ldsScene ? 0 : sceneLdsBytes + (c.materialsInLds ? materialBytes : 0);
    if (!(f.walk & WPT_WALK_NO_FOLD))
        c.materialsInLds |= LDS_FOLD;
    return c;
}

inline bool selectLargeForm(const KernelChoice& c, uint32_t walk, bool hasOrderedCopies, bool boxesMayBeNan, uint32_t nodeCount, size_t* sceneLdsBytes)
{
    size_t bytes = c.sceneLdsBytes;
    if (LARGE_ORDERED) {
        uint32_t base, stride;
        const uint32_t nodeQuads = 2 * nodeCount + 2;
        bytes = size_t(orderedPlaces(nodeQuads, uint32_t(c.sceneLdsBytes / 16) - nodeQuads, base, stride)) * 16;
    }
    *sceneLdsBytes = bytes;
    return c.rotated && c.ldsScene && c.features == (FEAT_BASIC | FEAT_ROTATED) && !(walk & WPT_WALK_SMALL_WORKGROUPS) && hasOrderedCopies
            && !boxesMayBeNan && COLD_BYTES_LARGE + bytes <= LDS_BYTES_PER_CU;
}

}

#endif
```

### wurblpt_amd/csrc/wpt_pathtrace.inc.h

```cpp
#ifndef WPT_PATHTRACE_INC_H
#define WPT_PATHTRACE_INC_H

#include <hip/hip_runtime.h>

#include "../../include/wurblpt_hip.h"
#include "wpt_blocks.h"

namespace wptk {

using namespace wptd;

constexpr int WG = 256;
constexpr int WG_LARGE = 1024;
constexpr uint32_t LDS_BYTES_PER_CU = 160 * 1024;
constexpr uint32_t COLD_AT_LARGE = 32 * 1024;
constexpr uint32_t ORDERED_COPIES = 8;
__host__ __device__ inline uint32_t orderedPlaces(uint32_t nodeQuads, uint32_t behind, uint32_t& base, uint32_t& stride)
{
    const uint32_t used = nodeQuads + behind;
    stride = ((nodeQuads + 13u) & ~15u) + 2u;
    base = used > stride ? ((used - stride + 15u) & ~15u) : 0u;
    return base + ORDERED_COPIES * stride;
}
#ifdef WPT_LARGE_PLAIN_STEP
constexpr bool LARGE_ORDERED = false;
#else
constexpr bool LARGE_ORDERED = true;
#endif
constexpr uint32_t NODE_CHILD = 0xc0000000u;
constexpr uint32_t NODE_INDEX_MASK = 0x3fffffffu;
constexpr uint32_t TABLE_BYTES = WPT_MATH_TABLE_WORDS * 8;
constexpr uint32_t COLD_BYTES = TABLE_BYTES + SLOT_COUNT * WG * 16;
constexpr uint32_t LDS_SCENE_MAX_BYTES = 20 * 1024;
constexpr uint32_t LDS_BYTES_PER_WORKGROUP_AT_FOUR = 160 * 1024 / 4;
constexpr uint32_t LDS_MATERIALS = 1u;
constexpr uint32_t LDS_FOLD = 2u;
constexpr uint32_t LDS_LEAF_LINKS = 4u;
constexpr uint32_t LEAF_NODE_SHIFT = 16, LEAF_NODE_MAX = 0x7fffu, LEAF_CORNER_MASK = 0xffffu;
static_assert(sizeof(wpt_material) % 16 == 0 && alignof(wpt_material) <= 16, "wpt_material must be a whole number of quadwords");
struct ViewsView {
    const wpt_camera* cams;
    uint32_t viewPixels;
    uint32_t viewCount;
    const uint32_t* streams;
};
struct AdaptiveView {
    const uint16_t* samplesSqrt;
    float* moments;
};
struct SlicesView {
    uint32_t* words;
    float4* carry;
    unsigned long long* stats;
    uint32_t rows, units;
    uint32_t declineOdd;
};
constexpr uint32_t SLICE_UNITS_MAX = 15;
constexpr uint32_t SLICE_SLOT_BITS = 28;
constexpr uint32_t SLICE_SLOT_MASK = (1u << SLICE_SLOT_BITS) - 1u;
struct KernelArgs {
    SceneView sv;
    wpt_camera cam;
    wpt_params par;
    uint32_t width, height, samplesSqrt;
    float invWidth, invHeight, invSamplesSqrt, invSamples;
    uint32_t blockStart, blockSize;
    uint32_t tiled;
    uint32_t bandPixels, bandFirst, bandStride;
    uint32_t leaveEighths;
    uint32_t heavyMin;
    uint32_t leafBias;
    uint32_t waitBelow;
    uint32_t fuse;
    uint32_t shadowWalksEnd;
    float* frame;
    uint32_t* pool;
    uint32_t rowStop;
    float4* carry;
    uint32_t* cost;
    const uint32_t* order;
    const uint32_t* orderCount;
    uint32_t cuCount;
    uint32_t materialsInLds;
    wpt_counters* counters;
    unsigned long long* schedStats;
    union {
        BinsView bins;
        ViewsView views;
        AdaptiveView adaptive;
        SlicesView slices;
    };
};
static_assert(sizeof(AdaptiveView) <= sizeof(BinsView) && alignof(AdaptiveView) <= alignof(BinsView), "AdaptiveView must fit in BinsView's place");
static_assert(sizeof(SlicesView) <= sizeof(BinsView) && alignof(SlicesView) <= alignof(BinsView), "SlicesView must fit in BinsView's place");
static_assert(sizeof(ViewsView) <= sizeof(BinsView) && alignof(ViewsView) <= alignof(BinsView), "ViewsView must fit in BinsView's place");

WPT_D bool lanePixel(const KernelArgs& args, uint32_t gid, uint32_t& pixel)
{
    bool inBlock = gid < args.blockSize;
    if (args.tiled) {
        const uint32_t tilesPerRow = args.width >> 3;
        const uint32_t tile = gid >> 6, lane = gid & 63u;
        const uint32_t tx = tile % tilesPerRow;
        uint32_t ty = tile / tilesPerRow;
        if (args.bandStride) {
            const uint32_t tileRowsPerBand = args.bandPixels / (args.width << 3);
            ty = (args.bandFirst + (ty / tileRowsPerBand) * args.bandStride) * tileRowsPerBand + ty % tileRowsPerBand;
        }
        pixel = args.blockStart + ((ty << 3) + (lane >> 3)) * args.width + (tx << 3) + (lane & 7u);
    } else if (args.bandStride) {
        pixel = (args.bandFirst + (gid / args.bandPixels) * args.bandStride) * args.bandPixels + gid % args.bandPixels;
    } else {
        pixel = args.blockStart + gid;
    }
    if (args.bandStride && pixel >= args.width * args.height)
        inBlock = false;
    if (!inBlock)
        pixel = args.blockStart;
    return inBlock;
}

enum { S_NODE = 0, S_LEAF = 1, S_SHADE = 2, S_NEEEND = 3, S_NEW = 4, S_DONE = 5, S_START = 6  };

constexpr uint32_t WIDE_STACK = 96;
constexpr uint32_t WIDE_NONE = 0xffffffffu;
constexpr int RAY_WALK_BINARY = 0x80;

WPT_D uint2 exactLinks(const SceneView& sv, uint32_t n)
{
    return *reinterpret_cast<const uint2*>(reinterpret_cast<const char*>(sv.spheres) + (n << 3));
}

template<uint32_t F, bool COUNT, bool LDSSCENE, int OCC, bool WIDE = false>
__global__ __launch_bounds__(WG, OCC) void wpt_pathtrace(const KernelArgs args)
{
    constexpr int WGS = WG;
    constexpr bool ORDERED = false;
#include "wpt_pathtrace_body.inc.h"
}

template<uint32_t F, int OCC, bool ORDERED>
__global__ __launch_bounds__(WG_LARGE, OCC) void wpt_pathtrace_large(const KernelArgs args)
{
    constexpr int WGS = WG_LARGE;
    constexpr bool COUNT = false, LDSSCENE = true, WIDE = false;
#include "wpt_pathtrace_body.inc.h"
}

template<class Kernel>
inline void launchMaybePooled(Kernel kernel, const KernelArgs& args, dim3 grid, size_t ldsBytes, hipStream_t stream, int lanes = WG)
{
    KernelArgs a = args;
    if (ldsBytes > 64 * 1024)
        (void)hipFuncSetAttribute(reinterpret_cast<const void*>(kernel), hipFuncAttributeMaxDynamicSharedMemorySize, (int)ldsBytes);
    if (a.pool) {
        int perCu = 0;
        if (hipOccupancyMaxActiveBlocksPerMultiprocessor(&perCu, kernel, lanes, ldsBytes) != hipSuccess)
            perCu = 0;
        const uint64_t resident = (uint64_t)(perCu < 0 ? 0 : perCu) * a.cuCount;
        if (resident == 0 || grid.x <= resident
                || hipMemsetD32Async((hipDeviceptr_t)a.pool, (int)(resident * lanes), 1, stream) != hipSuccess)
            a.pool = nullptr;
        else
            grid.x = (uint32_t)resident;
    }
    hipLaunchKernelGGL(kernel, grid, dim3(lanes), ldsBytes, stream, a);
}

constexpr uint32_t FEAT_BASIC = FEAT_GGX | FEAT_GLASS;
constexpr uint32_t FEAT_ALL = FEAT_TEXTURES | FEAT_MODPHONG | FEAT_ENVMAP | FEAT_LENS | FEAT_TWOSIDED | FEAT_GGX | FEAT_GLASS | FEAT_SPHERES | FEAT_SPOT;

struct GroundTruthArgs {
    SceneView scene;
    wpt_camera cam, camPrev, camNext;
    wpt_params par;
    float t0, tPrev, tNext;
    uint32_t width, height;
    void* array[WPT_GT_ARRAY_COUNT];
};
void launchGroundTruth(const GroundTruthArgs& args, hipStream_t stream);
void launchSelftestHits(const SceneView& scene, int n, const float* rays8, float* out15, hipStream_t stream);

constexpr uint32_t ORDER_BUCKETS = 128;
void launchOrderBuild(const KernelArgs& args, uint32_t* order, uint32_t* work, hipStream_t stream);
template<uint32_t F, bool COUNT, bool LDSSCENE, bool WIDE>
void launchPathtrace(const KernelArgs& args, dim3 grid, size_t sceneLdsBytes, hipStream_t stream);
#define WPT_PATHTRACE_LAUNCHER(F, COUNT, LDSSCENE, OCC, WIDE)                                                                  \
    template<> void launchPathtrace<(F), COUNT, LDSSCENE, WIDE>(const KernelArgs& args, dim3 grid, size_t sceneLdsBytes, hipStream_t stream) \
    {                                                                                                                          \
        launchMaybePooled(wpt_pathtrace<(F), COUNT, LDSSCENE, OCC, WIDE>, args, grid, COLD_BYTES + sceneLdsBytes, stream);     \
    }
constexpr uint32_t COLD_BYTES_LARGE = TABLE_BYTES + SLOT_COUNT * WG_LARGE * 16;
static_assert(COLD_AT_LARGE + SLOT_COUNT * WG_LARGE * 16 == LDS_BYTES_PER_CU && TABLE_BYTES <= COLD_AT_LARGE, "the large form's cold words end the unit's LDS");
template<uint32_t F>
void launchPathtraceLarge(const KernelArgs& args, dim3 grid, size_t sceneLdsBytes, hipStream_t stream);
#define WPT_PATHTRACE_LARGE_LAUNCHER(F, OCC, ORDERED)                                                                          \
    template<> void launchPathtraceLarge<(F)>(const KernelArgs& args, dim3 grid, size_t sceneLdsBytes, hipStream_t stream)     \
    {                                                                                                                          \
           \
        if (COLD_BYTES_LARGE + sceneLdsBytes <= LDS_BYTES_PER_CU)                                                              \
            launchMaybePooled(wpt_pathtrace_large<(F), OCC, ORDERED>, args, grid, LDS_BYTES_PER_CU, stream, WG_LARGE);         \
    }
void launchAdaptiveCost(const KernelArgs& args, hipStream_t stream);

}

#endif
```

### wurblpt_amd/csrc/wpt_pathtrace_body.inc.h

```cpp
    static_assert(!ORDERED || ((F & FEAT_ROTATED) && LDSSCENE && WGS == WG_LARGE), "ordered box copies: the large form of the rotated kernels with the scene in LDS");
    static_assert(!WIDE || (!LDSSCENE && !COUNT), "the wide walk: product kernels that fetch the scene from HBM (counting launches walk like the reference)");
    static_assert(!LDSSCENE || !(F & FEAT_SPHERES), "the LDS copy of the tree tells leaves (complemented word) from inner nodes by the sign bit: triangle leaves only");
    static_assert(!((F & FEAT_VIEWS) && (F & FEAT_TRANSIENT)), "a batch of views has no transient film (they share KernelArgs' union)");
    static_assert(!((F & FEAT_ADAPTIVE) && (F & (FEAT_VIEWS | FEAT_TRANSIENT))), "adaptive sampling has no views and no transient film (they share KernelArgs' union)");
    static_assert(!((F & FEAT_ADAPTIVE) && COUNT), "adaptive sampling has no counting build");
    static_assert(!((F & FEAT_TOF) && ((F & (FEAT_VIEWS | FEAT_TRANSIENT | FEAT_ADAPTIVE)) || COUNT)), "the time-of-flight sensor: one view, no other film, no counting build");
    static_assert(!((F & FEAT_SLICED) && ((F & (FEAT_VIEWS | FEAT_TRANSIENT | FEAT_ADAPTIVE | FEAT_TOF)) || COUNT)), "pixels in slices: plain product launches (they share KernelArgs' union)");
    static_assert(!LDSSCENE || (!WIDE && !(F & FEAT_SPHERES)), "the kernels with the scene in LDS carry their link words in SceneView::wideNodes and ::spheres (wpt_device.h): they may read neither as what it is named");
    constexpr bool VIEWS = (F & FEAT_VIEWS) != 0;
    constexpr bool ADAPTIVE = (F & FEAT_ADAPTIVE) != 0;
    constexpr bool SLICED = (F & FEAT_SLICED) != 0;
    constexpr bool ROTATED = (F & FEAT_ROTATED) != 0;
    static_assert(!ROTATED || (LDSSCENE && !(F & FEAT_ANIM)), "rotated copies of the corners: scenes at rest in LDS");
    constexpr bool PREFETCH = !LDSSCENE && !WIDE;
    constexpr int STEPS = LDSSCENE ? 3 : 1;
    constexpr int NEE_IN_WALK = LDSSCENE ? 0 : 4;
    constexpr int PRIORITY_WALK = 2, PRIORITY_LONG = 0;
    extern __shared__ float4 lds[];
    constexpr bool LARGE = WGS == WG_LARGE;
    float4* const ldsCold = LARGE ? lds + COLD_AT_LARGE / 16 : lds + TABLE_BYTES / 16;
    float4* const ldsScene = LARGE ? lds + TABLE_BYTES / 16 : ldsCold + SLOT_COUNT * WGS;
#if defined(WPT_MATH_TABLES_IN_LDS) && defined(__HIP_DEVICE_COMPILE__)
    wptm::tables_to_lds(threadIdx.x);
#endif

    SceneView svInLds = args.sv;
    const SceneView& sv = LDSSCENE ? static_cast<const SceneView&>(svInLds) : args.sv;
    const wpt_params& par = args.par;
    const uint32_t nodeCount = sv.nodeCount;
    uint32_t orderedBase = 0, orderedStride = 0;

    if (LDSSCENE) {
        const uint32_t n4 = 2 * nodeCount, t4 = 3 * sv.triCount;
        for (uint32_t i = threadIdx.x; i < n4; i += WGS) {
            float4 q = sv.nodes[i];
            if (i & 1) {
                const uint2 links = reinterpret_cast<const uint2*>(sv.wideNodes)[i >> 1];
                q.z = __uint_as_float(links.x);
                q.w = __uint_as_float(links.y);
            }
            ldsScene[i] = q;
        }
        if (threadIdx.x < 2)
            ldsScene[n4 + threadIdx.x] = threadIdx.x == 0 ? make_float4(0.0f, 0.0f, 0.0f, 0.0f)
                    : make_float4(0.0f, 0.0f, __uint_as_float(nodeCount), __uint_as_float(nodeCount));
        if (ROTATED) {
            const uint32_t* const triSkip = reinterpret_cast<const uint32_t*>(sv.wideNodes) + n4 + 4;
            const uint32_t* const triExact = reinterpret_cast<const uint32_t*>(sv.spheres) + n4 + 4;
            for (uint32_t i = threadIdx.x; i < t4; i += WGS) {
                const float4 g = sv.triGeom[i];
                const uint32_t tri = i / 3u, corner = i - 3u * tri;
                const float w = __uint_as_float(corner == 0 ? triSkip[tri] : corner == 1 ? triExact[tri] : tri);
                ldsScene[n4 + 2 + i] = make_float4(g.x, g.y, g.z, w);
                ldsScene[n4 + 2 + t4 + i] = make_float4(g.y, g.z, g.x, w);
                ldsScene[n4 + 2 + 2 * t4 + i] = make_float4(g.z, g.x, g.y, w);
            }
        } else {
            for (uint32_t i = threadIdx.x; i < t4; i += WGS)
                ldsScene[n4 + 2 + i] = sv.triGeom[i];
        }
        const uint32_t c4 = ROTATED ? 3 * t4 : t4;
        if (args.materialsInLds & LDS_MATERIALS) {
            const uint32_t m4 = sv.materialCount * (uint32_t)(sizeof(wpt_material) / 16);
            const float4* from = reinterpret_cast<const float4*>(sv.materials);
            for (uint32_t i = threadIdx.x; i < m4; i += WGS)
                ldsScene[n4 + 2 + c4 + i] = from[i];
            svInLds.materials = reinterpret_cast<const wpt_material*>(ldsScene + n4 + 2 + c4);
        }
        if constexpr (ORDERED) {
            const uint32_t m4 = (args.materialsInLds & LDS_MATERIALS) ? sv.materialCount * (uint32_t)(sizeof(wpt_material) / 16) : 0u;
            orderedPlaces(n4 + 2, c4 + m4, orderedBase, orderedStride);
            const float4* const copies = reinterpret_cast<const float4*>(sv.rglData);
            for (uint32_t i = n4 + 2 + threadIdx.x; i < ORDERED_COPIES * (n4 + 2); i += WGS) {
                float4 q = copies[i];
                const uint32_t k = i / (n4 + 2), at = i - k * (n4 + 2);
                if (at & 1) {
                    const uint2 links = at < n4 ? reinterpret_cast<const uint2*>(sv.wideNodes)[at >> 1] : make_uint2(nodeCount, nodeCount);
                    q.z = __uint_as_float(links.x);
                    q.w = __uint_as_float(links.y);
                }
                ldsScene[orderedBase + k * orderedStride + at] = q;
            }
        }
    }
    __syncthreads();
    auto node4 = [&](uint32_t i) -> float4 {
        if constexpr (LDSSCENE)
            return ldsScene[i];
        else
            return sv.nodes[i];
    };
    auto tri4 = [&](uint32_t i) -> float4 {
        if constexpr (LDSSCENE)
            return ldsScene[2 * nodeCount + 2 + i];
        else
            return sv.triGeom[i];
    };

    uint32_t walkStart = 0;
    if constexpr (LDSSCENE)
        walkStart = reinterpret_cast<const uint2*>(sv.wideNodes)[nodeCount + 1].x;

    auto pixelOf = [&](uint32_t gid, uint32_t& pixel) -> bool { return lanePixel(args, gid, pixel); };
    const bool firstPass = !ADAPTIVE && args.rowStop < args.samplesSqrt;
    const uint32_t laneLimit = args.order ? *args.orderCount : args.blockSize;
    uint32_t sliceUnits = 1, sliceRows = 0;
    if constexpr (SLICED) {
        sliceUnits = args.pool ? args.slices.units : 1u;
        sliceRows = args.pool ? args.slices.rows : args.samplesSqrt;
    }
    FrameArgs fa;
    fa.cam = args.cam;
    fa.par = args.par;
    fa.width = args.width;
    fa.height = args.height;
    fa.samplesSqrt = args.samplesSqrt;
    fa.invWidth = args.invWidth;
    fa.invHeight = args.invHeight;
    fa.invSamplesSqrt = args.invSamplesSqrt;

    std::conditional_t<ADAPTIVE, PathLdsSum<WG>, PathLds<WG>> ps;
    ps.base = LARGE ? ldsCold + (threadIdx.x / WG) * (SLOT_COUNT * WG) + threadIdx.x % WG : ldsCold + threadIdx.x;
    uint32_t view = 0;
    uint32_t laneSqrt = 0;
    uint32_t unit = 0;
    auto startPixel = [&](uint32_t at) -> bool {
        uint32_t pixel = args.blockStart;
        bool have;
        if constexpr (SLICED) {
            uint32_t g = 0, slot = at;
            if (at >= laneLimit) {
                g = at / laneLimit;
                slot = at - g * laneLimit;
            }
            have = pixelOf(slot, pixel);
            if (g > 0) {
                have = false;
                if (g < sliceUnits) {
                    const uint32_t before = __hip_atomic_fetch_or(args.slices.words + slot, 1u << (16 + g), __ATOMIC_ACQUIRE, __HIP_MEMORY_SCOPE_AGENT);
                    have = ((before >> g) & 1u) != 0 && !(args.slices.declineOdd && (slot & 1u));
                }
            }
            unit = slot | (g << SLICE_SLOT_BITS);
            pathStateInit(ps, pixel, pixel % args.width, pixel / args.width);
            if (have && g > 0) {
                ps.base[SLOT_PRNG * WG] = args.slices.carry[2 * (size_t)slot];
                ps.base[SLOT_ACC * WG] = args.slices.carry[2 * (size_t)slot + 1];
                atomicAdd(args.slices.stats, 1ull);
            }
            return have;
        }
        if (args.order) {
            have = at < laneLimit;
            if (have)
                pixel = args.order[at];
        } else if constexpr (VIEWS) {
            have = at < args.blockSize;
            view = have ? at / args.views.viewPixels : 0u;
            pixelOf(at - view * args.views.viewPixels, pixel);
        } else {
            have = pixelOf(at, pixel);
        }
        if constexpr (VIEWS) {
            const uint64_t stream = args.views.streams ? args.views.streams[view] : 0u;
            pathStateInit(ps, (uint64_t)pixel + stream * args.views.viewPixels, pixel % args.width, pixel / args.width);
        } else {
            pathStateInit(ps, pixel, pixel % args.width, pixel / args.width);
        }
        if constexpr (ADAPTIVE) {
            laneSqrt = have ? (uint32_t)args.adaptive.samplesSqrt[pixel] : 0u;
            ps.sampleSum = mk3(0.0f, 0.0f, 0.0f);
            if (laneSqrt > 0 && args.adaptive.moments) {
                float* m = args.adaptive.moments + 3 * (size_t)pixel;
                m[0] = 0.0f;
                m[1] = 0.0f;
                m[2] = 0.0f;
            }
        }
        if (!ADAPTIVE && have && args.order) {
            ps.base[SLOT_PRNG * WG] = args.carry[2 * (size_t)pixel];
            ps.base[SLOT_ACC * WG] = args.carry[2 * (size_t)pixel + 1];
// ... 292 lines not shown
                } else {
                    if (COUNT) {
                        sched[1]++;
                        sched[2] += nNode;
                    }
                    if constexpr (WIDE) {
                        if (state == S_NODE && !(aux.k & (RAY_MAY_NAN | RAY_WALK_BINARY))) {
                            const uint32_t ref = curRef;
                            const bool admitted = curEntry <= amax;
                            uint2 top = make_uint2(WIDE_NONE, 0u);
                            if (sp > 0)
                                top = pend[sp - 1];
                            curRef = WIDE_NONE;
                            if (admitted && ref < NODE_CHILD) {
                                leafPrim = ref;
                                state = S_LEAF;
                            } else if (admitted) {
                                const float4* w = sv.wideNodes + 8 * (size_t)(ref & NODE_INDEX_MASK);
                                const float4 lx = w[0], ly = w[1], lz = w[2], hx = w[3], hy = w[4], hz = w[5], rf = w[6];
                                const float amin = par.min_hit_distance;
                                auto entryOf = [&](float lox, float loy, float loz, float hix, float hiy, float hiz, uint32_t r) {
                                    const float t0x = (lox - ps.o.x) * aux.inv.x, t0y = (loy - ps.o.y) * aux.inv.y, t0z = (loz - ps.o.z) * aux.inv.z;
                                    const float t1x = (hix - ps.o.x) * aux.inv.x, t1y = (hiy - ps.o.y) * aux.inv.y, t1z = (hiz - ps.o.z) * aux.inv.z;
                                    const float near = __builtin_fmaxf(__builtin_fmaxf(amin, __builtin_fminf(t0x, t1x)),
                                            __builtin_fmaxf(__builtin_fminf(t0y, t1y), __builtin_fminf(t0z, t1z)));
                                    const float far = __builtin_fminf(__builtin_fminf(amax, __builtin_fmaxf(t0x, t1x)),
                                            __builtin_fminf(__builtin_fmaxf(t0y, t1y), __builtin_fmaxf(t0z, t1z)));
                                    if (r != WIDE_NONE && near <= far) {
                                        if (curRef != WIDE_NONE)
                                            pend[sp++] = make_uint2(curRef, __float_as_uint(curEntry));
                                        curRef = r;
                                        curEntry = near;
                                    }
                                };
                                entryOf(lx.w, ly.w, lz.w, hx.w, hy.w, hz.w, __float_as_uint(rf.w));
                                entryOf(lx.z, ly.z, lz.z, hx.z, hy.z, hz.z, __float_as_uint(rf.z));
                                entryOf(lx.y, ly.y, lz.y, hx.y, hy.y, hz.y, __float_as_uint(rf.y));
                                entryOf(lx.x, ly.x, lz.x, hx.x, hy.x, hz.x, __float_as_uint(rf.x));
                            }
                            if (curRef == WIDE_NONE && top.x != WIDE_NONE) {
                                curRef = top.x;
                                curEntry = __uint_as_float(top.y);
                                sp--;
                            }
                            if (state == S_NODE && curRef == WIDE_NONE)
                                state = endOfRayState();
                        }
                        if (__ballot(state == S_NODE && (aux.k & (RAY_MAY_NAN | RAY_WALK_BINARY))) != 0) {
                            if (state == S_NODE && (aux.k & (RAY_MAY_NAN | RAY_WALK_BINARY)))
                                binaryStep();
                        }
                    } else if constexpr (LDSSCENE) {
                        static_assert(!COUNT, "the LDS kernel has no counting build: ldsStep counts nothing");
                        if (nanPossible) {
#pragma unroll
                            for (int step = 0; step < STEPS; step++)
                                ldsStep(std::true_type());
                        } else {
#pragma unroll
                            for (int step = 0; step < STEPS; step++)
                                ldsStep(std::false_type());
                        }
                    } else {
#pragma unroll
                        for (int step = 0; step < STEPS; step++) {
                            sec<COUNT>(lc, SEC_NODE_STEP, state == S_NODE);
                            if (state == S_NODE)
                                binaryStep();
                        }
                    }
                }
            }
        }
        if (COUNT && pick == S_NODE)
            sched[11] += (unsigned long long)(clock64() - tBlock);
        if (pick != S_NODE && (fused ? cShade > 0 : pick == S_SHADE)) {
            if (COUNT) {
                tBlock = clock64();
                sched[5]++;
                sched[6] += cShade;
            }
            if (state == S_SHADE) {
                realOrigin();
                afterBlock(blockShade<F, COUNT>(sv, par, tri4, ps, best, lc, cTrav != 0 ? (int)args.waitBelow : 0, args.bins));
            }
            if (COUNT)
                sched[12] += (unsigned long long)(clock64() - tBlock);
        }
        if (pick != S_NODE && (fused ? cNee > 0 : pick == S_NEEEND)) {
            if (COUNT) {
                tBlock = clock64();
                sched[7]++;
                sched[8] += cNee;
            }
            sec<COUNT>(lc, SEC_NEE_END, state == S_NEEEND);
            sec<COUNT>(lc, SEC_NEE_END_LIGHT, state == S_NEEEND && ps.rayKind == RAY_NEE_LIGHT && best.prim == ps.getW(SLOT_NEE));
            if (state == S_NEEEND) {
                realOrigin();
                afterBlock(blockNeeEnd<F>(sv, par, tri4, ps, best, args.bins));
            }
            if (COUNT)
                sched[13] += (unsigned long long)(clock64() - tBlock);
        }
        if (pick != S_NODE && (fused ? __ballot(state == S_NEW) != 0 : pick == S_NEW)) {
            if (COUNT) {
                tBlock = clock64();
                sched[9]++;
                sched[10] += __popcll(__ballot(state == S_NEW));
            }
            sec<COUNT>(lc, SEC_NEW_SAMPLE, state == S_NEW);
            if (state == S_NEW) {
                const bool passEnds = firstPass && (ps.getW(SLOT_ACC) >> 16) >= args.rowStop;
                int next;
                if constexpr (SLICED) {
                    const uint32_t g = unit >> SLICE_SLOT_BITS;
                    const uint32_t rowEnd = (g + 1) * sliceRows < args.samplesSqrt ? (g + 1) * sliceRows : args.samplesSqrt;
                    next = (ps.getW(SLOT_ACC) >> 16) >= rowEnd ? (int)NEXT_DONE : blockNew<F>(fa, ps, sv);
                    if (next == NEXT_DONE && rowEnd < args.samplesSqrt) {
                        const uint32_t slot = unit & SLICE_SLOT_MASK;
                        args.slices.carry[2 * (size_t)slot] = ps.base[SLOT_PRNG * WG];
                        args.slices.carry[2 * (size_t)slot + 1] = ps.base[SLOT_ACC * WG];
                        const uint32_t before = __hip_atomic_fetch_or(args.slices.words + slot, 1u << (g + 1), __ATOMIC_RELEASE, __HIP_MEMORY_SCOPE_AGENT);
                        next = NEXT_HANDED_ON;
                        if (((before >> (17 + g)) & 1u) != 0 || (args.slices.declineOdd && (slot & 1u))) {
                            unit += 1u << SLICE_SLOT_BITS;
                            atomicAdd(args.slices.stats + 1, 1ull);
                            next = NEXT_NEW;
                        }
                    }
                } else if constexpr (ADAPTIVE) {
                    const f3 s = ps.sampleSum;
                    if (args.adaptive.moments && ps.getW(SLOT_ACC) != 0) {
                        const uint32_t pxy = ps.getW(SLOT_SRDIR);
                        float* m = args.adaptive.moments + 3 * ((size_t)(pxy >> 16) * args.width + (pxy & 0xffffu));
                        m[0] = m[0] + s.x * s.x;
                        m[1] = m[1] + s.y * s.y;
                        m[2] = m[2] + s.z * s.z;
                    }
                    ps.sampleSum = mk3(0.0f, 0.0f, 0.0f);
                    FrameArgs fl = fa;
                    fl.samplesSqrt = laneSqrt;
                    fl.invSamplesSqrt = 1.0f / (float)laneSqrt;
                    next = blockNew<F>(fl, ps, sv);
                } else if constexpr (VIEWS) {
                    const uint32_t first = (uint32_t)__builtin_amdgcn_readfirstlane((int)view);
                    if (passEnds)
                        next = NEXT_DONE;
                    else if (__ballot(view != first) == 0)
                        next = blockNewFrom<F, true>(fa, args.views.cams[first], ps, sv);
                    else
                        next = blockNewFrom<F, false>(fa, args.views.cams[view], ps, sv);
                } else {
                    next = passEnds ? (int)NEXT_DONE : blockNew<F>(fa, ps, sv);
                }
                sec<COUNT>(lc, SEC_PIXEL_DONE, next == NEXT_DONE);
                if (next == NEXT_DONE) {
                    const uint32_t pxy = ps.getW(SLOT_SRDIR);
                    const size_t at = (VIEWS ? (size_t)view * args.views.viewPixels : 0u) + (size_t)(pxy >> 16) * args.width + (pxy & 0xffffu);
                    if (firstPass) {
                        args.carry[2 * at] = ps.base[SLOT_PRNG * WG];
                        args.carry[2 * at + 1] = ps.base[SLOT_ACC * WG];
                        args.cost[at] = (uint32_t)clock64() - args.cost[at];
                    } else if (ADAPTIVE) {
                        if (laneSqrt > 0) {
                            const float invSamples = 1.0f / (float)(laneSqrt * laneSqrt);
                            const Slot acc = ps.get(SLOT_ACC);
                            float* out = args.frame + 3 * at;
                            out[0] = invSamples * acc.x;
                            out[1] = invSamples * acc.y;
                            out[2] = invSamples * acc.z;
                            if (args.adaptive.moments) {
                                float* m = args.adaptive.moments + 3 * at;
                                m[0] = invSamples * m[0];
                                m[1] = invSamples * m[1];
                                m[2] = invSamples * m[2];
                            }
                        }
                    } else if (!(F & (FEAT_TRANSIENT | FEAT_TOF)) || args.frame) {
                        const Slot acc = ps.get(SLOT_ACC);
                        float* out = args.frame + 3 * at;
                        out[0] = args.invSamples * acc.x;
                        out[1] = args.invSamples * acc.y;
// ... 41 lines not shown
```

### wurblpt_amd/csrc/wpt_scene_layout.h

```cpp
#ifndef WPT_SCENE_LAYOUT_H
#define WPT_SCENE_LAYOUT_H

#include <algorithm>
#include <cmath>
#include <cstdint>
#include <cstring>
#include <vector>

#include "../../include/wurblpt_hip.h"
#include "wpt_fold.h"
#include "wpt_rgl.h"

namespace wptl {

constexpr uint32_t NODE_CHILD = 0xc0000000u, NODE_INDEX_MASK = 0x3fffffffu, PRIM_SPHERE = 0x80000000u;
constexpr uint32_t WIDE_STACK = 96, WIDE_NONE = 0xffffffffu;
constexpr uint32_t LDS_SCENE_MAX_BYTES = 20 * 1024;
static_assert(NODE_CHILD == wptf::FOLD_NODE_CHILD && NODE_INDEX_MASK == wptf::FOLD_INDEX_MASK, "wpt_fold.h reads the words deviceNodes writes");

struct Quad {
    float x, y, z, w;
};
static_assert(sizeof(Quad) == 16, "a quadword is 16 bytes");

inline Quad quad(float x, float y, float z, float w)
{
    const Quad q = { x, y, z, w };
    return q;
}

struct Status {
    wpt_status code;
    const char* message;
};

inline Status refuse(wpt_status code, const char* message)
{
    const Status s = { code, message };
    return s;
}

inline Status validate(const wpt_scene_desc* d)
{
    if (!d)
        return refuse(WPT_ERR_INVALID_ARGUMENT, "scene description is NULL");
    if (d->abi_version != WPT_ABI_VERSION)
        return refuse(WPT_ERR_INVALID_ARGUMENT, "scene description has a different ABI version");
    if (d->node_count == 0 || !d->nodes)
        return refuse(WPT_ERR_INVALID_ARGUMENT, "scene has no BVH nodes (run Scene::updateBVH)");
    if (d->tri_count > 0 && !d->tri_geom)
        return refuse(WPT_ERR_INVALID_ARGUMENT, "triangle geometry array (tri_geom) is NULL");
    if (d->tri_count > 0 && !d->tri_attr)
        return refuse(WPT_ERR_INVALID_ARGUMENT, "triangle attribute array (tri_attr) is NULL");
    if (d->instance_count > 0 && !d->instances)
        return refuse(WPT_ERR_INVALID_ARGUMENT, "instance array (instances) is NULL");
    if (d->material_count > 0 && !d->materials)
        return refuse(WPT_ERR_INVALID_ARGUMENT, "material array (materials) is NULL");
    if (d->texture_count > 0 && !d->textures)
        return refuse(WPT_ERR_INVALID_ARGUMENT, "texture array (textures) is NULL");
    if (d->hotspot_count > 0 && !d->hotspots)
        return refuse(WPT_ERR_INVALID_ARGUMENT, "hot spot array (hotspots) is NULL");
    if (d->texel_bytes > 0 && !d->texels)
        return refuse(WPT_ERR_INVALID_ARGUMENT, "texel pool (texels) is NULL");
    for (uint32_t i = 0; i < d->node_count; i++) {
        const wpt_bvh_node& n = d->nodes[i];
        if (n.kind == WPT_NODE_INNER) {
            if (n.link >= d->node_count || n.link <= i || i + 1 >= d->node_count)
                return refuse(WPT_ERR_INVALID_ARGUMENT, "BVH inner node links outside the node array");
        } else if (n.kind == WPT_NODE_TRIANGLE) {
            if (n.link >= d->tri_count || n.link >= PRIM_SPHERE)
                return refuse(WPT_ERR_INVALID_ARGUMENT, "BVH leaf references a triangle outside the array");
        } else if (n.kind == WPT_NODE_SPHERE) {
            if (n.link >= d->sphere_count || n.link >= (NODE_CHILD & ~PRIM_SPHERE))
                return refuse(WPT_ERR_INVALID_ARGUMENT, "BVH leaf references a sphere outside the array");
        } else if (n.kind != WPT_NODE_EMPTY) {
            return refuse(WPT_ERR_UNSUPPORTED, "BVH node kind is not known to the kernel");
        }
    }
    {
        std::vector<uint32_t> end(d->node_count);
        for (uint32_t i = d->node_count; i-- > 0;) {
            const wpt_bvh_node& n = d->nodes[i];
            if (n.kind == WPT_NODE_INNER) {
                if (n.link != end[i + 1])
                    return refuse(WPT_ERR_INVALID_ARGUMENT, "BVH nodes are not one depth-first tree (second child does not follow the first child's subtree)");
                end[i] = end[n.link];
            } else {
                end[i] = i + 1;
            }
        }
        if (end[0] != d->node_count)
            return refuse(WPT_ERR_INVALID_ARGUMENT, "BVH nodes are not one depth-first tree (nodes behind the root's subtree)");
    }
// ... 189 lines not shown
    if (n > NODE_INDEX_MASK)
        return refuse(WPT_ERR_UNSUPPORTED, "more than 2^30 - 1 BVH nodes");
    const std::vector<uint32_t> end = subtreeEnds(desc);
    std::vector<uint32_t> place;
    const Status placed = nodePlaces(desc, end, topNodes, &place);
    if (placed.code != WPT_OK)
        return placed;
    std::vector<Quad> dev(size_t(n) * 2 + 2, quad(0.0f, 0.0f, 0.0f, 0.0f));
    uint32_t boxesMayBeNan = 0u;
    for (uint32_t i = 0; i < n; i++) {
        const wpt_bvh_node& nd = desc->nodes[i];
        const uint32_t skip = place[end[i]];
        const uint32_t word = nd.kind == WPT_NODE_INNER ? (NODE_CHILD | place[i + 1]) : nd.kind == WPT_NODE_TRIANGLE ? triNew[nd.link]
            : nd.kind == WPT_NODE_SPHERE ? (PRIM_SPHERE | nd.link) : (NODE_CHILD | skip);
        float sk, wd;
        memcpy(&sk, &skip, 4);
        memcpy(&wd, &word, 4);
        dev[2 * size_t(place[i])] = quad(nd.lo[0], nd.hi[0], nd.lo[1], nd.lo[2]);
        dev[2 * size_t(place[i]) + 1] = quad(nd.hi[1], nd.hi[2], sk, wd);
        for (int a = 0; a < 3; a++)
            if (nd.lo[a] != nd.lo[a] || nd.hi[a] != nd.hi[a])
                boxesMayBeNan = 1u;
    }
    out->quads.swap(dev);
    out->boxesMayBeNan = boxesMayBeNan;
    return refuse(WPT_OK, nullptr);
}

inline uint32_t countFoldedLinks(const uint32_t* nodes, uint32_t nodeCount, uint32_t* words)
{
    uint32_t folded = 0;
    for (uint32_t i = 0; i < nodeCount; i++) {
        uint32_t links;
        const uint32_t word = wptf::foldLdsWord(nodes, nodeCount, i, true, &links);
        folded += links > 0 ? 1u : 0u;
        if (words)
            words[i] = word;
    }
    return folded;
}

constexpr uint32_t ORDERED_COPIES = 8;

inline bool orderedBoxCopies(const uint32_t* nodes, uint32_t nodeCount, std::vector<Quad>* out)
{
    out->clear();
    std::vector<Quad> plain(2 * size_t(nodeCount) + 2, quad(0.0f, 0.0f, 0.0f, 0.0f));
    if (nodeCount > 0)
        memcpy(plain.data(), nodes, 2 * size_t(nodeCount) * sizeof(Quad));
    for (uint32_t i = 0; i < nodeCount; i++) {
        const Quad &q0 = plain[2 * size_t(i)], &q1 = plain[2 * size_t(i) + 1];
        if (!(q0.x <= q0.y && q0.z <= q1.x && q0.w <= q1.y))
            return false;
    }
    std::vector<Quad> copies;
    copies.reserve(ORDERED_COPIES * plain.size());
    for (uint32_t k = 0; k < ORDERED_COPIES; k++)
        for (uint32_t i = 0; i <= nodeCount; i++) {
            Quad q0 = plain[2 * size_t(i)], q1 = plain[2 * size_t(i) + 1];
            if (i < nodeCount) {
                if (k & 1u) {
                    const float lo = q0.x;
                    q0.x = -q0.y;
                    q0.y = -lo;
                }
                if (k & 2u) {
                    const float lo = q0.z;
                    q0.z = -q1.x;
                    q1.x = -lo;
                }
                if (k & 4u) {
                    const float lo = q0.w;
                    q0.w = -q1.y;
                    q1.y = -lo;
                }
            }
            copies.push_back(q0);
            copies.push_back(q1);
        }
    out->swap(copies);
    return true;
}

inline std::vector<Quad> wideNodes(const wpt_scene_desc* desc, const std::vector<uint32_t>& triNew, uint32_t* worstStack = nullptr)
{
    const uint32_t n = desc->node_count;
    if (worstStack)
        *worstStack = 0xffffffffu;
    bool ok = true;
    for (uint32_t i = 0; i < n && ok; i++) {
        const wpt_bvh_node& nd = desc->nodes[i];
        for (int a = 0; a < 3; a++)
            ok = ok && std::isfinite(nd.lo[a]) && std::isfinite(nd.hi[a]);
        if (nd.kind == WPT_NODE_INNER) {
            const uint32_t child[2] = { i + 1, nd.link };
            for (int k = 0; k < 2; k++)
                for (int a = 0; a < 3; a++)
                    ok = ok && desc->nodes[child[k]].lo[a] >= nd.lo[a] && desc->nodes[child[k]].hi[a] <= nd.hi[a];
        }
    }
    std::vector<Quad> wide;
    std::vector<uint32_t> made;
    std::vector<uint32_t> entries;
    if (ok) {
        std::vector<uint32_t> todo(1, 0u);
        while (!todo.empty()) {
            const uint32_t x = todo.back();
            todo.pop_back();
            made.push_back(x);
            uint32_t entry[4] = { 0xffffffffu, 0xffffffffu, 0xffffffffu, 0xffffffffu };
            int count = 0;
            if (desc->nodes[x].kind == WPT_NODE_INNER) {
                const uint32_t child[2] = { x + 1, desc->nodes[x].link };
                for (int k = 0; k < 2; k++) {
                    if (desc->nodes[child[k]].kind == WPT_NODE_INNER) {
                        entry[count++] = child[k] + 1;
                        entry[count++] = desc->nodes[child[k]].link;
                    } else {
                        entry[count++] = child[k];
                    }
                }
            } else {
                entry[count++] = x;
            }
            for (int k = 0; k < 4; k++)
                entries.push_back(entry[k]);
            for (int k = count - 1; k >= 0; k--)
                if (desc->nodes[entry[k]].kind == WPT_NODE_INNER && entry[k] != x)
                    todo.push_back(entry[k]);
        }
        ok = made.size() <= NODE_INDEX_MASK;
    }
    if (ok) {
        std::vector<uint32_t> wideOf(n, 0xffffffffu);
        for (size_t w = 0; w < made.size(); w++)
            wideOf[made[w]] = uint32_t(w);
        std::vector<uint32_t> depth(made.size(), 0u);
        for (size_t w = made.size(); w-- > 0;) {
            int count = 0;
            while (count < 4 && entries[4 * w + count] != 0xffffffffu)
                count++;
            uint32_t worst = 0;
            for (int k = 0; k < count; k++) {
                const uint32_t e = entries[4 * w + k];
                const uint32_t below = (desc->nodes[e].kind == WPT_NODE_INNER && e != made[w]) ? depth[wideOf[e]] : 0u;
                worst = std::max(worst, uint32_t(count - 1 - k) + below);
            }
            depth[w] = worst;
        }
        if (worstStack)
            *worstStack = depth[0];
        ok = depth[0] <= WIDE_STACK;
        wide.resize(made.size() * 8, quad(0.0f, 0.0f, 0.0f, 0.0f));
        for (size_t w = 0; w < made.size() && ok; w++) {
            float q[8][4];
            uint32_t ref[4] = { WIDE_NONE, WIDE_NONE, WIDE_NONE, WIDE_NONE };
            for (int r = 0; r < 8; r++)
                for (int k = 0; k < 4; k++)
                    q[r][k] = 0.0f;
            for (int k = 0; k < 4; k++) {
                const uint32_t e = entries[4 * w + k];
                if (e == 0xffffffffu)
                    continue;
                const wpt_bvh_node& nd = desc->nodes[e];
                for (int a = 0; a < 3; a++) {
                    q[a][k] = nd.lo[a];
// ... 148 lines not shown
```

### wurblpt_amd/device.py

```python
import ctypes as C
import os

from . import _abi

_LIB = None


def lib_path():
    return os.path.join(os.path.dirname(os.path.abspath(__file__)), os.environ.get("WPT_LIB_DIR", "lib"), "libwurblpt_hip.so")


WALK_WIDE, WALK_FULL_SHADOW, WALK_COUNT_PRODUCT, WALK_TRIANGLES_AS_GIVEN, WALK_SELECT_CORNERS, WALK_NO_FOLD, WALK_NO_BYPASS = 1, 2, 4, 8, 16, 32, 64
WALK_SMALL_WORKGROUPS = 128
SLICES_DECLINE_ODD = 0x100

EXPORTS = list(_abi.FUNCTIONS)


def lib():
    global _LIB
    if _LIB is None:
        path = lib_path()
        if not os.path.exists(path):
            raise RuntimeError("%s is missing: the HIP extension must be built (python -c 'import __graft_entry__ as g; g.build()'); "
                               "there is no CPU fallback" % path)
        try:
            import torch
        except ImportError:
            pass
        L = C.CDLL(path)
        for name, (restype, argtypes) in {**_abi.FUNCTIONS, **_abi.TEST_HOOK_FUNCTIONS}.items():
            fn = getattr(L, name, None)
            if fn is not None:
                fn.restype, fn.argtypes = restype, argtypes
        _LIB = L
    return _LIB


def _check(status):
    if status != _abi.WPT_OK:
        raise RuntimeError("wurblpt_hip: %s (status %d)" % (lib().wpt_last_error().decode(), status))



def _frame_size(host_scene, width, height):
    return width or host_scene.width, height or host_scene.height


def _params(params):
    from . import host
    return params if params is not None else host.default_params()


def _stream_ptr(stream):
    return C.c_void_p(stream.cuda_stream) if stream is not None else None


def _tensor_ptr(tensor):
    return C.c_void_p(tensor.data_ptr()) if tensor is not None else None


def _array_ptr(array):
    return C.c_void_p(array.ctypes.data) if array is not None else None


COUNTER_NAMES = ("samples", "rays", "node_visits", "leaf_tests", "pdf_tests", "scatters")


def _new_counters(wanted):
    import torch
    return torch.zeros(len(COUNTER_NAMES), dtype=torch.int64, device="cuda") if wanted else None


def _counters_dict(counters):
    return dict(zip(COUNTER_NAMES, [int(x) for x in counters.cpu().tolist()]))


def uniform_edges(start, width, count):
    import numpy as np
    k = np.arange(count + 1, dtype=np.float32)
    edges = np.float32(start) + k * np.float32(width)
    if count < 1 or not np.all(np.isfinite(edges)) or not np.all(edges[1:] > edges[:-1]):
        raise ValueError("uniform_edges(%r, %r, %r): the edges do not increase" % (start, width, count))
    return edges


def _edges_array(edges):
    import numpy as np
    e = np.ascontiguousarray(np.asarray(edges, dtype=np.float32))
    assert e.ndim == 1 and e.size >= 2, "bin edges: at least two values"
    return e


def _groups_table(groups, material_count):
    import numpy as np
    a = np.asarray(groups)
# ... 482 lines not shown
def tof_accumulate_host(sensor, phase, radiance_w, opl_w, is_tof_light, acc):
    _check(lib().wpt_tof_accumulate_host(C.byref(sensor), phase, radiance_w, opl_w, 1 if is_tof_light else 0, C.c_void_p(acc.ctypes.data)))
    return acc


def tof_result(phase_differences, modulation_frequency):
    import numpy as np
    from . import host
    D = np.asarray(phase_differences, dtype=np.float32)
    n = D.shape[0]
    assert n % 4 == 0 and n > 0, "a multiple of 4 phase images"
    d0, d1, d2, d3 = D[0], D[n // 4], D[2 * n // 4], D[3 * n // 4]
    re, im = d0 - d2, d3 - d1
    zero = (np.abs(d0 - d2) <= 0) & (np.abs(d1 - d3) <= 0)
    atan2f = C.CFUNCTYPE(C.c_float, C.c_float, C.c_float)(("atan2f", C.CDLL("libm.so.6")))
    shift = np.frompyfunc(atan2f, 2, 1)(im, re).astype(np.float32)
    shift = np.where(shift < 0, (shift.astype(np.float64) + 2.0 * float(np.float32(np.pi))).astype(np.float32), shift)
    frac_c_modfreq = np.float32(host.SPEED_OF_LIGHT / float(modulation_frequency))
    distance = frac_c_modfreq * shift * np.float32(0.25) * np.float32(1.0 / np.pi)
    shift = np.where(zero, np.float32(0), shift).astype(np.float32)
    distance = np.where(zero, np.float32(0), distance).astype(np.float32)
    amplitude = (np.sqrt((d0 - d2) * (d0 - d2) + (d1 - d3) * (d1 - d3)) * np.float32(np.pi / 2)).astype(np.float32)
    intensity = (np.float32(0.5) * (d0 + d1 + d2 + d3)).astype(np.float32)
    return distance, amplitude, intensity, shift


def device_count():
    return lib().wpt_device_count()


def set_slices(n):
    _check(lib().wpt_set_slices(n))


def slices_plan(block_size, lanes_at_once, samples_sqrt):
    units, rows = C.c_uint32(), C.c_uint32()
    _check(lib().wpt_slices_plan(block_size, lanes_at_once, samples_sqrt, C.byref(units), C.byref(rows)))
    return int(units.value), int(rows.value)


SENSOR_FRAME, SENSOR_TRANSIENT, SENSOR_VIEWS, SENSOR_ADAPTIVE, SENSOR_TOF = range(5)


def kernel_choice(need, sensor, count, node_count, tri_count, material_count, scene_has_wide=False, variant=0, walk=0):
    name, form, key, lds_bytes, materials = C.c_char_p(), C.c_char_p(), (C.c_uint32 * 4)(), C.c_uint64(), C.c_uint32()
    _check(lib().wpt_kernel_choice(need, sensor, int(count), node_count, tri_count, material_count, int(scene_has_wide), variant, walk,
                                   C.byref(name), C.byref(form), key, C.byref(lds_bytes), C.byref(materials)))
    return name.value.decode(), form.value.decode(), (key[0], bool(key[1]), bool(key[2]), bool(key[3])), int(lds_bytes.value), int(materials.value)


def kernel_table():
    rows = []
    key, name = (C.c_uint32 * 4)(), C.c_char_p()
    while lib().wpt_kernel_table_entry(len(rows), key, C.byref(name)) == _abi.WPT_OK:
        rows.append(((key[0], bool(key[1]), bool(key[2]), bool(key[3])), name.value.decode()))
    return rows


STRATEGIES = ("one pass", "two passes", "adaptive order", "sliced")
PLAN_WORDS = ("wavefront", "wavefront_falls_back", "pooled", "strategy", "units", "rows", "passes")


def launch_plan(sensor, count, need, scene_in_lds, block_size, samples_sqrt, cu_count, variant=0, wavefront_mode=0, slices=0):
    w = (C.c_uint32 * len(PLAN_WORDS))()
    _check(lib().wpt_launch_plan(*[int(v) for v in (sensor, count, need, scene_in_lds, block_size, samples_sqrt, cu_count, variant, wavefront_mode,
                                                    slices)], w))
    plan = dict(zip(PLAN_WORDS, (int(v) for v in w)))
    for k in ("wavefront", "wavefront_falls_back", "pooled"):
        plan[k] = bool(plan[k])
    plan["strategy"] = STRATEGIES[plan["strategy"]]
    return plan


def last_slice_stats():
    taken, continued = C.c_uint64(), C.c_uint64()
    _check(lib().wpt_last_slice_stats(C.byref(taken), C.byref(continued)))
    return int(taken.value), int(continued.value)


def kernel_workgroup():
    ordered = C.c_uint32()
    lanes = lib().wpt_kernel_workgroup(C.byref(ordered))
    return int(lanes), bool(ordered.value)


def fold_plan(host_scene, with_words=False):
    import numpy as np
    folded = C.c_uint32()
    words = np.zeros(int(host_scene.d.node_count), np.uint32)
    _check(lib().wpt_fold_plan(C.cast(host_scene.desc, C.c_void_p), C.byref(folded), _array_ptr(words if with_words else None)))
    return (int(folded.value), words) if with_words else int(folded.value)


BYPASS_MODEL, BYPASS_ALL_ELIGIBLE = 0, 1


def set_bypass(mode):
    _check(lib().wpt_set_bypass(mode))


def bypass_plan(host_scene, with_words=False):
    import numpy as np
    count = C.c_uint32()
    n = int(host_scene.d.node_count)
    words = np.zeros(2 * n + 1, np.uint32)
    _check(lib().wpt_bypass_plan(C.cast(host_scene.desc, C.c_void_p), C.byref(count), _array_ptr(words if with_words else None)))
    return (int(count.value), words[:2 * n].reshape(n, 2), int(words[2 * n])) if with_words else int(count.value)


def progress_covers(sensor=SENSOR_FRAME, counting=False, bands=False):
    _check(lib().wpt_progress_covers(sensor, int(bool(counting)), int(bool(bands))))


def progress_state_info(state):
    state = bytes(state)
    info = _abi.ProgressInfo()
    _check(lib().wpt_progress_state_info(state, len(state), C.byref(info)))
    return {n: int(getattr(info, n)) for n, _ in info._fields_ if n != "reserved"}


class Progressive:

    def __init__(self, scene, handle, width, height, block):
        self.scene, self._handle = scene, handle
        self.width, self.height, self.block = width, height, block

    @property
    def rows_done(self):
        return int(lib().wpt_progress_rows_done(self._handle))

    @property
    def rows_total(self):
        return int(lib().wpt_progress_rows_total(self._handle))

    @property
    def finished(self):
        return self.rows_done == self.rows_total

    def advance(self, rows, frame=None, stream=None):
        if frame is not None:
            assert frame.is_cuda and frame.is_contiguous() and frame.dtype.is_floating_point and frame.element_size() == 4
            assert frame.numel() == self.width * self.height * 3
        _check(lib().wpt_progress_advance_device(self._handle, rows, _tensor_ptr(frame), _stream_ptr(stream)))
        return self.rows_done

    def preview(self, out=None, stream=None):
        import torch
        if out is None:
            out = torch.zeros((self.height, self.width, 3), dtype=torch.float32, device="cuda")
            if stream is not None:
                stream.wait_stream(torch.cuda.current_stream())
        assert out.is_cuda and out.is_contiguous() and out.element_size() == 4 and out.numel() == self.width * self.height * 3
        _check(lib().wpt_progress_preview_device(self._handle, C.c_void_p(out.data_ptr()), _stream_ptr(stream)))
        return out

    def save(self):
        n = C.c_uint64()
        _check(lib().wpt_progress_state_bytes(self._handle, C.byref(n)))
        buf = C.create_string_buffer(n.value)
        _check(lib().wpt_progress_save(self._handle, buf, n.value))
        return buf.raw

    def close(self):
        if self._handle:
            lib().wpt_progress_end(self._handle)
            self._handle = C.c_void_p()
# ... 504 lines not shown
```

Before: 1555 Msamples/s.

## Stage per-triangle hit records, hot spots and normal matrices in LDS for large form

In the large-workgroup kernel form, each workgroup copies per-triangle attributes and flags, the hot-spot light data and the instance normal matrices into LDS after the scene. Hit finishing, light sampling and the hot-spot PDF then read them from LDS rather than from global memory. The goal is to cut global memory latency in shading for small scenes such as this 36-triangle Cornell box. In exchange it uses more LDS and preload work per workgroup, adds template variants, and adds a flag that keeps this data in HBM.

```diff
diff --git a/include/wurblpt_hip.h b/include/wurblpt_hip.h
--- a/include/wurblpt_hip.h
+++ b/include/wurblpt_hip.h
@@ -498,6 +498,7 @@
 #define WPT_WALK_NO_FOLD 32u
 #define WPT_WALK_NO_BYPASS 64u
 #define WPT_WALK_SMALL_WORKGROUPS 128u
+#define WPT_WALK_HIT_DATA_IN_HBM 256u
 wpt_status wpt_set_walk(uint32_t flags);
 wpt_status wpt_scene_folded_links(const wpt_scene* scene, uint32_t* folded);
 wpt_status wpt_fold_plan(const wpt_scene_desc* desc, uint32_t* folded, uint32_t* lds_words);
@@ -516,6 +517,10 @@
 const char* wpt_kernel_name(void);
 const char* wpt_kernel_form(void);
 uint32_t wpt_kernel_workgroup(uint32_t* ordered_boxes);
+#define WPT_HIT_DATA_RECORDS 1u
+#define WPT_HIT_DATA_HOTSPOTS 2u
+#define WPT_HIT_DATA_NORMALS 4u
+uint32_t wpt_kernel_hit_data(void);
 wpt_status wpt_kernel_choice(uint32_t need, uint32_t sensor, uint32_t count, uint32_t node_count, uint32_t tri_count, uint32_t material_count,
         uint32_t scene_has_wide, uint32_t variant, uint32_t walk, const char** name, const char** form, uint32_t key[4],
         uint64_t* scene_lds_bytes, uint32_t* materials_in_lds);
diff --git a/wurblpt_amd/_abi.py b/wurblpt_amd/_abi.py
--- a/wurblpt_amd/_abi.py
+++ b/wurblpt_amd/_abi.py
@@ -262,6 +262,7 @@
     "wpt_kernel_name": (_S, []),
     "wpt_kernel_form": (_S, []),
     "wpt_kernel_workgroup": (_U, [_pU]),
+    "wpt_kernel_hit_data": (_U, []),
     "wpt_kernel_choice": (_I, [_U] * 9 + [_pS, _pS, _pU, _pQ, _pU]),
     "wpt_kernel_table_entry": (_I, [_U, _pU, _pS]),
     "wpt_launch_plan": (_I, [_U] * 10 + [_pU]),
diff --git a/wurblpt_amd/csrc/wpt_blocks.h b/wurblpt_amd/csrc/wpt_blocks.h
--- a/wurblpt_amd/csrc/wpt_blocks.h
+++ b/wurblpt_amd/csrc/wpt_blocks.h
@@ -272,9 +272,20 @@
             const f3 orgR = rotated(org, auxKz(h));
             const uint32_t off = rotatedCopyOffset(auxKz(h), sv.triCount);
             float sum = 0.0f;
+            [[maybe_unused]] const bool inLds = hitDataInLds(tri4, HIT_DATA_HOTSPOTS);
             for (uint32_t i = 0; i < sv.hotspotCount; i++) {
-                const uint32_t p = off + 3 * sv.hotspots[i].prim;
-                sum += hotSpotPdfValueRotated(tri4(p), tri4(p + 1), tri4(p + 2), orgR, dir, h, sv.hotspotFace[i]);
+                if constexpr (HasLdsHitData<Tri4>::value) {
+                    if (inLds) {
+                        const uint32_t p = off + 3 * __float_as_uint(tri4.hotspot(i, 1).x);
+                        sum += hotSpotPdfValueRotated(tri4(p), tri4(p + 1), tri4(p + 2), orgR, dir, h, tri4.hotspot(i, 0));
+                    } else {
+                        const uint32_t p = off + 3 * sv.hotspots[i].prim;
+                        sum += hotSpotPdfValueRotated(tri4(p), tri4(p + 1), tri4(p + 2), orgR, dir, h, sv.hotspotFace[i]);
+                    }
+                } else {
+                    const uint32_t p = off + 3 * sv.hotspots[i].prim;
+                    sum += hotSpotPdfValueRotated(tri4(p), tri4(p + 1), tri4(p + 2), orgR, dir, h, sv.hotspotFace[i]);
+                }
             }
             return sum * here(sv.invHotspotCount);
         };
@@ -700,20 +711,43 @@
         idx = idx < sv.hotspotCount - 1 ? idx : sv.hotspotCount - 1;
         const wpt_hotspot& hs = sv.hotspots[idx];
         f3 directDir;
-        uint32_t hotSpotPrim = hs.prim;
-        if ((F & FEAT_SPHERES) && hs.kind == WPT_HOTSPOT_SPHERE) {
-            const DirectionDraw draw = sphereDirection(sphereNow<F>(sv, ps, sv.spheres[hs.prim]), h.p, prng);
-            directDir = draw.dir;
-            prng = draw.prng;
-            hotSpotPrim = PRIM_SPHERE | hs.prim;
+        uint32_t hotSpotPrim;
+        if constexpr (HasLdsHitData<Tri4>::value) {
+            static_assert(!(F & (FEAT_SPHERES | FEAT_ANIM)), "hot spots in LDS: triangle lights at rest");
+            const f3 bary = inTriangle(in01x2(prng));
+            f3 p;
+            if (hitDataInLds(tri4, HIT_DATA_HOTSPOTS)) {
+                const float4 q1 = tri4.hotspot(idx, 1), q2 = tri4.hotspot(idx, 2), q3 = tri4.hotspot(idx, 3);
+                hotSpotPrim = __float_as_uint(q1.x);
+                p = add(add(scl(bary.x, mk3(q1.z, q1.w, q2.x)), scl(bary.y, mk3(q2.y, q2.z, q2.w))), scl(bary.z, mk3(q3.x, q3.y, q3.z)));
+                if (__float_as_uint(q1.y)) {
+                    const float4 m0 = tri4.hotspot(idx, 4), m1 = tri4.hotspot(idx, 5), m2 = tri4.hotspot(idx, 6), m3 = tri4.hotspot(idx, 7);
+                    const float M[16] = { m0.x, m0.y, m0.z, m0.w, m1.x, m1.y, m1.z, m1.w, m2.x, m2.y, m2.z, m2.w, m3.x, m3.y, m3.z, m3.w };
+                    p = mat4mulPoint(M, p);
+                }
+            } else {
+                hotSpotPrim = hs.prim;
+                p = add(add(scl(bary.x, ld3(hs.p0)), scl(bary.y, ld3(hs.p1))), scl(bary.z, ld3(hs.p2)));
+                if (hs.transform)
+                    p = mat4mulPoint(hs.M, p);
+            }
+            directDir = normalize(sub(p, h.p));
         } else {
-            const f3 bary = inTriangle(in01x2(prng));
-            f3 p = add(add(scl(bary.x, ld3(hs.p0)), scl(bary.y, ld3(hs.p1))), scl(bary.z, ld3(hs.p2)));
-            if (hs.transform)
-                p = mat4mulPoint(hs.M, p);
-            if ((F & FEAT_ANIM) && hs.animation >= 0)
-                p = animatePoint(animationMatrix(sv, ps, hs.animation), p);
-            directDir = normalize(sub(p, h.p));
+            hotSpotPrim = hs.prim;
+            if ((F & FEAT_SPHERES) && hs.kind == WPT_HOTSPOT_SPHERE) {
+                const DirectionDraw draw = sphereDirection(sphereNow<F>(sv, ps, sv.spheres[hs.prim]), h.p, prng);
+                directDir = draw.dir;
+                prng = draw.prng;
+                hotSpotPrim = PRIM_SPHERE | hs.prim;
+            } else {
+                const f3 bary = inTriangle(in01x2(prng));
+                f3 p = add(add(scl(bary.x, ld3(hs.p0)), scl(bary.y, ld3(hs.p1))), scl(bary.z, ld3(hs.p2)));
+                if (hs.transform)
+                    p = mat4mulPoint(hs.M, p);
+                if ((F & FEAT_ANIM) && hs.animation >= 0)
+                    p = animatePoint(animationMatrix(sv, ps, hs.animation), p);
+                directDir = normalize(sub(p, h.p));
+            }
         }
         section(4);
         float hotSpotsPdf, directPdf;
diff --git a/wurblpt_amd/csrc/wpt_capi.hip b/wurblpt_amd/csrc/wpt_capi.hip
--- a/wurblpt_amd/csrc/wpt_capi.hip
+++ b/wurblpt_amd/csrc/wpt_capi.hip
@@ -21,6 +21,9 @@
 std::atomic<unsigned long long*> g_lastSliceStats{nullptr};
 
 std::atomic<uint32_t> g_lastWorkgroup{uint32_t(WG)};
+std::atomic<uint32_t> g_lastHitData{0};
+static_assert(WPT_HIT_DATA_RECORDS == wptk::HIT_DATA_RECORDS && WPT_HIT_DATA_HOTSPOTS == wptk::HIT_DATA_HOTSPOTS && WPT_HIT_DATA_NORMALS == wptk::HIT_DATA_NORMALS,
+        "wpt_lds_places.h restates the header's names of the parts");
 
 static_assert(wptk::PLAN_WG == uint32_t(WG) && wptk::PLAN_SLICE_SLOT_MAX == wptk::SLICE_SLOT_MASK && wptk::SLICE_UNITS_TARGET <= wptk::SLICE_UNITS_MAX
         && wptk::PLAN_FRAME == wptk::SENSOR_FRAME && wptk::PLAN_VIEWS == wptk::SENSOR_VIEWS && wptk::PLAN_ADAPTIVE == wptk::SENSOR_ADAPTIVE
@@ -51,11 +54,13 @@
     g_lastPasses.store(passes, std::memory_order_relaxed);
     g_lastSliceStats.store(sliceStats, std::memory_order_relaxed);
     g_lastWorkgroup.store(uint32_t(WG), std::memory_order_relaxed);
-}
-
-void recordWorkgroup(uint32_t lanes, bool orderedBoxes)
+    g_lastHitData.store(0, std::memory_order_relaxed);
+}
+
+void recordWorkgroup(uint32_t lanes, bool orderedBoxes, uint32_t hitDataParts)
 {
     g_lastWorkgroup.store(lanes | (orderedBoxes ? 0x80000000u : 0u), std::memory_order_relaxed);
+    g_lastHitData.store(hitDataParts, std::memory_order_relaxed);
 }
 
 const char* kernelForm(bool rotated, uint32_t units, bool leafLinksFromNodes)
@@ -161,6 +166,11 @@
     if (ordered_boxes)
         *ordered_boxes = w >> 31;
     return w & 0x7fffffffu;
+}
+
+uint32_t wpt_kernel_hit_data(void)
+{
+    return g_lastHitData.load(std::memory_order_relaxed);
 }
 
 uint32_t wpt_last_render_passes(void)
@@ -229,7 +239,7 @@
 wpt_status wpt_set_walk(uint32_t flags)
 {
     if (flags & ~(WPT_WALK_WIDE | WPT_WALK_FULL_SHADOW | WPT_WALK_COUNT_PRODUCT | WPT_WALK_TRIANGLES_AS_GIVEN | WPT_WALK_SELECT_CORNERS | WPT_WALK_NO_FOLD | WPT_WALK_NO_BYPASS
-            | WPT_WALK_SMALL_WORKGROUPS))
+            | WPT_WALK_SMALL_WORKGROUPS | WPT_WALK_HIT_DATA_IN_HBM))
         return fail(WPT_ERR_INVALID_ARGUMENT, "unknown walk flag");
     settings.walk = flags;
     return WPT_OK;
diff --git a/wurblpt_amd/csrc/wpt_capi_common.h b/wurblpt_amd/csrc/wpt_capi_common.h
--- a/wurblpt_amd/csrc/wpt_capi_common.h
+++ b/wurblpt_amd/csrc/wpt_capi_common.h
@@ -89,6 +89,7 @@
     uint32_t* ldsLinks = nullptr;
     bool leafOneToOne = false;
     const float4* orderedNodes = nullptr;
+    uint32_t normalsNamed = 0;
     uint32_t bypassedNodes = 0;
     uint32_t animationCount;
     std::vector<void*> allocations;
@@ -116,7 +117,7 @@
 extern Settings settings;
 
 void recordLaunch(const char* name, const char* form, uint32_t passes, unsigned long long* sliceStats);
-void recordWorkgroup(uint32_t lanes, bool orderedBoxes);
+void recordWorkgroup(uint32_t lanes, bool orderedBoxes, uint32_t hitDataParts);
 const char* kernelForm(bool rotated, uint32_t units = 0, bool leafLinksFromNodes = false);
 wpt_status lookupKernel(uint32_t features, bool count, bool ldsScene, bool wide, const wptk::KernelEntry** entry);
 
diff --git a/wurblpt_amd/csrc/wpt_capi_render.hip b/wurblpt_amd/csrc/wpt_capi_render.hip
--- a/wurblpt_amd/csrc/wpt_capi_render.hip
+++ b/wurblpt_amd/csrc/wpt_capi_render.hip
@@ -182,9 +182,13 @@
         }
     }
     size_t largeLdsBytes = 0;
-    const bool large = wptk::selectLargeForm(choice, settings.walk, scene->orderedNodes != nullptr, args.sv.boxesMayBeNan != 0, scene->nodeCount, &largeLdsBytes);
+    uint32_t hitData = 0;
+    const bool large = wptk::selectLargeForm(choice, settings.walk, scene->orderedNodes != nullptr, args.sv.boxesMayBeNan != 0, scene->nodeCount,
+            { scene->triCount, args.sv.materialCount, scene->normalsNamed, args.sv.hotspotCount }, &largeLdsBytes, &hitData);
     if (large && wptk::LARGE_ORDERED)
         args.sv.rglData = reinterpret_cast<const float*>(scene->orderedNodes);
+    if (large)
+        args.materialsInLds |= hitData;
     const SingleKernel run = large
             ? SingleKernel{ wptk::launchPathtraceLarge<FEAT_BASIC | FEAT_ROTATED>, dim3((args.blockSize + WG_LARGE - 1) / WG_LARGE), largeLdsBytes, stream }
             : SingleKernel{ kernel->launch, dim3((args.blockSize + WG - 1) / WG), choice.sceneLdsBytes, stream };
@@ -202,7 +206,7 @@
     recordLaunch(kernel->name, kernelForm(choice.rotated, sliceStats ? plan.units : 0, choice.rotated && !scene->leafOneToOne), done ? plan.passes : 1u,
             sliceStats);
     if (large)
-        recordWorkgroup(WG_LARGE, wptk::LARGE_ORDERED);
+        recordWorkgroup(WG_LARGE, wptk::LARGE_ORDERED, (hitData >> wptk::LDS_HIT_DATA_SHIFT) & 7u);
     return hipGetLastError();
 }
 
diff --git a/wurblpt_amd/csrc/wpt_capi_scene.hip b/wurblpt_amd/csrc/wpt_capi_scene.hip
--- a/wurblpt_amd/csrc/wpt_capi_scene.hip
+++ b/wurblpt_amd/csrc/wpt_capi_scene.hip
@@ -251,6 +251,7 @@
         WPT_TRY(uploadArray(s, reinterpret_cast<const float4*>(a.data()), size_t(desc->tri_count) * 6, &view.triAttr));
     }
     WPT_TRY(uploadArray(s, desc->instances, desc->instance_count, &view.instances));
+    s->normalsNamed = wptl::normalsNamed(desc);
     WPT_TRY(uploadArray(s, desc->materials, desc->material_count, &view.materials));
     view.materialCount = desc->material_count;
     {
diff --git a/wurblpt_amd/csrc/wpt_device.h b/wurblpt_amd/csrc/wpt_device.h
--- a/wurblpt_amd/csrc/wpt_device.h
+++ b/wurblpt_amd/csrc/wpt_device.h
@@ -8,6 +8,7 @@
 #include "wpt_math.h"
 #include "wpt_triangle.h"
 #include "wpt_anim.h"
+#include "wpt_lds_places.h"
 #include "wpt_rgl.h"
 
 namespace wptd {
@@ -468,6 +469,27 @@
     const float4* triGeom;
     WPT_D float4 operator()(uint32_t i) const { return triGeom[i]; }
 };
+template<uint32_t PARTS>
+struct LdsHitData {
+    const float4* scene;
+    uint32_t corners;
+    uint32_t recordsAt, hotspotsAt, normalsAt;
+    WPT_D float4 operator()(uint32_t i) const { return scene[corners + i]; }
+    static constexpr WPT_D bool has(uint32_t part) { return (PARTS & part) != 0; }
+    WPT_D float4 record(uint32_t prim, uint32_t k) const { return scene[recordsAt + wptk::HIT_RECORD_QUADS * prim + k]; }
+    WPT_D float4 hotspot(uint32_t i, uint32_t k) const { return scene[hotspotsAt + wptk::HIT_HOTSPOT_QUADS * i + k]; }
+    WPT_D float4 normalColumn(uint32_t instance, uint32_t k) const { return scene[normalsAt + wptk::HIT_NORMAL_QUADS * instance + k]; }
+};
+template<class Tri4> struct HasLdsHitData { static constexpr bool value = false; };
+template<uint32_t PARTS> struct HasLdsHitData<LdsHitData<PARTS>> { static constexpr bool value = true; };
+template<class Tri4> WPT_D bool hitDataInLds(const Tri4& tri4, uint32_t part)
+{
+    if constexpr (HasLdsHitData<Tri4>::value)
+        return tri4.has(part);
+    else
+        return false;
+}
+
 template<uint32_t F = 0, class Tri4 = TriGeomFromScene>
 WPT_D Hit finishHit(const SceneView& sv, const Candidate& c, f3 org, f3 dir, float time, Tri4 tri4)
 {
@@ -476,8 +498,29 @@
     Hit h;
     h.a = c.a;
     h.prim = c.prim;
-    uint32_t instance, flags;
-    if constexpr ((F & FEAT_ROTATED) != 0) {
+    uint32_t instance = 0, flags = 0;
+    float4 a0, a1, a2, a3, a4, a5;
+    [[maybe_unused]] const bool recordInLds = hitDataInLds(tri4, wptk::HIT_DATA_RECORDS);
+    if constexpr (HasLdsHitData<Tri4>::value) {
+        static_assert((F & FEAT_ROTATED) != 0, "the large form: a kernel with rotated corners");
+        if (recordInLds) {
+            a0 = tri4.record(c.prim, 0);
+            a1 = tri4.record(c.prim, 1);
+            a2 = tri4.record(c.prim, 2);
+            a3 = tri4.record(c.prim, 3);
+            a4 = tri4.record(c.prim, 4);
+            a5 = tri4.record(c.prim, 5);
+            const float4 words = tri4.record(c.prim, 6);
+            instance = __float_as_uint(words.x);
+            h.material = __float_as_uint(words.y);
+            flags = __float_as_uint(words.z);
+        } else {
+            const uint32_t* words = reinterpret_cast<const uint32_t*>(sv.triGeom + 3 * (size_t)c.prim);
+            instance = words[3];
+            h.material = words[7];
+            flags = words[11];
+        }
+    } else if constexpr ((F & FEAT_ROTATED) != 0) {
         (void)tri4;
         const uint32_t* words = reinterpret_cast<const uint32_t*>(sv.triGeom + 3 * (size_t)c.prim);
         instance = words[3];
@@ -495,13 +538,35 @@
     const float bx = c.invDet * c.U, by = c.invDet * c.V, bz = c.invDet * c.W;
     h.p = add(org, scl(c.a, dir));
     const float4* at = sv.triAttr + 6 * (size_t)c.prim;
-    const float4 a0 = at[0], a1 = at[1], a2 = at[2], a3 = at[3], a4 = at[4], a5 = at[5];
+    if constexpr (HasLdsHitData<Tri4>::value) {
+        if (!recordInLds)
+            a0 = at[0], a1 = at[1], a2 = at[2], a3 = at[3], a4 = at[4], a5 = at[5];
+    } else {
+        a0 = at[0], a1 = at[1], a2 = at[2], a3 = at[3], a4 = at[4], a5 = at[5];
+    }
     const f3 n0 = mk3(a0.x, a0.y, a0.z), n1 = mk3(a0.w, a1.x, a1.y), n2 = mk3(a1.z, a1.w, a2.x);
     f3 nrm = add(add(scl(bx, n0), scl(by, n1)), scl(bz, n2));
     const bool transform = (flags & WPT_TRI_TRANSFORM) != 0;
     const float* N = sv.instances[instance].N;
+    [[maybe_unused]] const bool normalInLds = hitDataInLds(tri4, wptk::HIT_DATA_NORMALS);
+    [[maybe_unused]] float ldsN[9] = { 0.0f, 0.0f, 0.0f, 0.0f, 0.0f, 0.0f, 0.0f, 0.0f, 0.0f };
+    if constexpr (HasLdsHitData<Tri4>::value) {
+        if (normalInLds && transform) {
+            const float4 c0 = tri4.normalColumn(instance, 0), c1 = tri4.normalColumn(instance, 1), c2 = tri4.normalColumn(instance, 2);
+            ldsN[0] = c0.x; ldsN[1] = c0.y; ldsN[2] = c0.z;
+            ldsN[3] = c1.x; ldsN[4] = c1.y; ldsN[5] = c1.z;
+            ldsN[6] = c2.x; ldsN[7] = c2.y; ldsN[8] = c2.z;
+        }
+    }
+    auto normalMatrixTimes = [&](f3 v) {
+        if constexpr (HasLdsHitData<Tri4>::value) {
+            if (normalInLds)
+                return mat3mul(ldsN, v);
+        }
+        return mat3mul(N, v);
+    };
     if (transform)
-        nrm = mat3mul(N, nrm);
+        nrm = normalMatrixTimes(nrm);
     float animationN[9];
     const bool animate = (F & FEAT_ANIM) && (flags & WPT_TRI_ANIMATE);
     if (animate) {
@@ -525,7 +590,7 @@
         tan = add(add(scl(bx, t0), scl(by, t1)), scl(bz, t2));
         if (dot(tan, tan) > 0.0f) {
             if (transform)
-                tan = mat3mul(N, tan);
+                tan = normalMatrixTimes(tan);
             if (animate)
                 tan = mat3mul(animationN, tan);
             tan = normalize(sub(tan, scl(dot(nrm, tan), nrm)));
diff --git a/wurblpt_amd/csrc/wpt_kernel_table.h b/wurblpt_amd/csrc/wpt_kernel_table.h
--- a/wurblpt_amd/csrc/wpt_kernel_table.h
+++ b/wurblpt_amd/csrc/wpt_kernel_table.h
@@ -150,7 +150,11 @@
     return c;
 }
 
-inline bool selectLargeForm(const KernelChoice& c, uint32_t walk, bool hasOrderedCopies, bool boxesMayBeNan, uint32_t nodeCount, size_t* sceneLdsBytes)
+struct HitDataCounts {
+    uint32_t triCount, materialCount, instanceCount, hotspotCount;
+};
+inline bool selectLargeForm(const KernelChoice& c, uint32_t walk, bool hasOrderedCopies, bool boxesMayBeNan, uint32_t nodeCount, const HitDataCounts& counts,
+        size_t* sceneLdsBytes, uint32_t* hitData)
 {
     size_t bytes = c.sceneLdsBytes;
     if (LARGE_ORDERED) {
@@ -158,9 +162,21 @@
         const uint32_t nodeQuads = 2 * nodeCount + 2;
         bytes = size_t(orderedPlaces(nodeQuads, uint32_t(c.sceneLdsBytes / 16) - nodeQuads, base, stride)) * 16;
     }
+    const bool large = c.rotated && c.ldsScene && c.features == (FEAT_BASIC | FEAT_ROTATED) && !(walk & WPT_WALK_SMALL_WORKGROUPS) && hasOrderedCopies
+            && !boxesMayBeNan && COLD_BYTES_LARGE + bytes <= LDS_BYTES_PER_CU;
+    *hitData = 0;
+    if (large && !(walk & WPT_WALK_HIT_DATA_IN_HBM)) {
+        const HitDataPlaces places = hitDataPlaces(nodeCount, counts.triCount, (c.materialsInLds & LDS_MATERIALS) ? counts.materialCount : 0u,
+                counts.instanceCount, counts.hotspotCount, LARGE_ORDERED);
+        const uint32_t parts = hitDataKernelParts(places.parts);
+        if (parts && size_t(places.nodeCopiesEnd) * 16 == bytes) {
+            const uint32_t end = (parts & HIT_DATA_NORMALS) ? places.quads : places.normalsAt;
+            bytes = size_t(end) * 16;
+            *hitData = (parts << LDS_HIT_DATA_SHIFT) | ((parts & HIT_DATA_NORMALS) ? counts.instanceCount << LDS_HIT_NORMALS_SHIFT : 0u);
+        }
+    }
     *sceneLdsBytes = bytes;
-    return c.rotated && c.ldsScene && c.features == (FEAT_BASIC | FEAT_ROTATED) && !(walk & WPT_WALK_SMALL_WORKGROUPS) && hasOrderedCopies
-            && !boxesMayBeNan && COLD_BYTES_LARGE + bytes <= LDS_BYTES_PER_CU;
+    return large;
 }
 
 }
diff --git a/wurblpt_amd/csrc/wpt_lds_places.h b/wurblpt_amd/csrc/wpt_lds_places.h
--- /dev/null
+++ b/wurblpt_amd/csrc/wpt_lds_places.h
@@ -0,0 +1,78 @@
+#ifndef WPT_LDS_PLACES_H
+#define WPT_LDS_PLACES_H
+
+#include <stdint.h>
+
+#include "../../include/wurblpt_hip.h"
+
+#if defined(__HIPCC__)
+#define WPT_PLACES_FN __host__ __device__ inline
+#else
+#define WPT_PLACES_FN inline
+#endif
+
+namespace wptk {
+
+constexpr uint32_t ORDERED_COPIES = 8;
+WPT_PLACES_FN uint32_t orderedPlaces(uint32_t nodeQuads, uint32_t behind, uint32_t& base, uint32_t& stride)
+{
+    const uint32_t used = nodeQuads + behind;
+    stride = ((nodeQuads + 13u) & ~15u) + 2u;
+    base = used > stride ? ((used - stride + 15u) & ~15u) : 0u;
+    return base + ORDERED_COPIES * stride;
+}
+
+constexpr uint32_t HIT_DATA_RECORDS = 1u, HIT_DATA_HOTSPOTS = 2u, HIT_DATA_NORMALS = 4u;
+constexpr uint32_t HIT_RECORD_QUADS = 7, HIT_HOTSPOT_QUADS = 8, HIT_NORMAL_QUADS = 3;
+constexpr uint32_t LARGE_SCENE_ROOM_QUADS = (32u * 1024u - 512u) / 16u;
+constexpr uint32_t HIT_NORMALS_MAX = 0xffffu;
+constexpr uint32_t HIT_DATA_ALL = HIT_DATA_RECORDS | HIT_DATA_HOTSPOTS | HIT_DATA_NORMALS;
+WPT_PLACES_FN uint32_t hitDataKernelParts(uint32_t fit)
+{
+    const uint32_t two = HIT_DATA_RECORDS | HIT_DATA_HOTSPOTS;
+    return (fit & HIT_DATA_ALL) == HIT_DATA_ALL ? HIT_DATA_ALL : (fit & two) == two ? two : 0u;
+}
+
+struct HitDataPlaces {
+    uint32_t parts;
+    uint32_t recordsAt, hotspotsAt, normalsAt;
+    uint32_t nodeCopiesEnd;
+    uint32_t quads;
+};
+
+WPT_PLACES_FN HitDataPlaces hitDataPlaces(uint32_t nodeCount, uint32_t triCount, uint32_t materialCount, uint32_t instanceCount, uint32_t hotspotCount,
+        bool ordered = true)
+{
+    HitDataPlaces p = { 0u, 0u, 0u, 0u, 0u, 0u };
+    const uint64_t nodeQuads64 = 2ull * nodeCount + 2ull;
+    const uint64_t behind64 = 9ull * triCount + uint64_t(materialCount) * (sizeof(wpt_material) / 16);
+    if (nodeQuads64 + behind64 > LARGE_SCENE_ROOM_QUADS) {
+        p.nodeCopiesEnd = p.quads = p.recordsAt = p.hotspotsAt = p.normalsAt = 0xffffffffu;
+        return p;
+    }
+    const uint32_t nodeQuads = uint32_t(nodeQuads64), behind = uint32_t(behind64);
+    uint32_t base, stride;
+    p.nodeCopiesEnd = ordered ? orderedPlaces(nodeQuads, behind, base, stride) : nodeQuads + behind;
+    uint32_t at = p.nodeCopiesEnd;
+    bool open = at <= LARGE_SCENE_ROOM_QUADS;
+    auto part = [&](uint32_t bit, uint64_t count, uint32_t each, uint32_t& where) {
+        where = at;
+        if (count == 0)
+            return;
+        if (open && at + count * each <= LARGE_SCENE_ROOM_QUADS) {
+            p.parts |= bit;
+            at += uint32_t(count * each);
+        } else {
+            open = false;
+        }
+    };
+    part(HIT_DATA_RECORDS, triCount, HIT_RECORD_QUADS, p.recordsAt);
+    part(HIT_DATA_HOTSPOTS, hotspotCount, HIT_HOTSPOT_QUADS, p.hotspotsAt);
+    part(HIT_DATA_NORMALS, instanceCount <= HIT_NORMALS_MAX ? instanceCount : 0xffffffffull, HIT_NORMAL_QUADS, p.normalsAt);
+    p.quads = at;
+    return p;
+}
+
+}
+
+#endif
diff --git a/wurblpt_amd/csrc/wpt_pathtrace.inc.h b/wurblpt_amd/csrc/wpt_pathtrace.inc.h
--- a/wurblpt_amd/csrc/wpt_pathtrace.inc.h
+++ b/wurblpt_amd/csrc/wpt_pathtrace.inc.h
@@ -5,6 +5,7 @@
 
 #include "../../include/wurblpt_hip.h"
 #include "wpt_blocks.h"
+#include "wpt_lds_places.h"
 
 namespace wptk {
 
@@ -14,14 +15,6 @@
 constexpr int WG_LARGE = 1024;
 constexpr uint32_t LDS_BYTES_PER_CU = 160 * 1024;
 constexpr uint32_t COLD_AT_LARGE = 32 * 1024;
-constexpr uint32_t ORDERED_COPIES = 8;
-__host__ __device__ inline uint32_t orderedPlaces(uint32_t nodeQuads, uint32_t behind, uint32_t& base, uint32_t& stride)
-{
-    const uint32_t used = nodeQuads + behind;
-    stride = ((nodeQuads + 13u) & ~15u) + 2u;
-    base = used > stride ? ((used - stride + 15u) & ~15u) : 0u;
-    return base + ORDERED_COPIES * stride;
-}
 #ifdef WPT_LARGE_PLAIN_STEP
 constexpr bool LARGE_ORDERED = false;
 #else
@@ -36,6 +29,7 @@
 constexpr uint32_t LDS_MATERIALS = 1u;
 constexpr uint32_t LDS_FOLD = 2u;
 constexpr uint32_t LDS_LEAF_LINKS = 4u;
+constexpr uint32_t LDS_HIT_DATA_SHIFT = 8, LDS_HIT_NORMALS_SHIFT = 16;
 constexpr uint32_t LEAF_NODE_SHIFT = 16, LEAF_NODE_MAX = 0x7fffu, LEAF_CORNER_MASK = 0xffffu;
 static_assert(sizeof(wpt_material) % 16 == 0 && alignof(wpt_material) <= 16, "wpt_material must be a whole number of quadwords");
 struct ViewsView {
@@ -136,10 +130,11 @@
 {
     constexpr int WGS = WG;
     constexpr bool ORDERED = false;
+    constexpr uint32_t HIT = 0;
 #include "wpt_pathtrace_body.inc.h"
 }
 
-template<uint32_t F, int OCC, bool ORDERED>
+template<uint32_t F, int OCC, bool ORDERED, uint32_t HIT>
 __global__ __launch_bounds__(WG_LARGE, OCC) void wpt_pathtrace_large(const KernelArgs args)
 {
     constexpr int WGS = WG_LARGE;
@@ -192,14 +187,23 @@
     }
 constexpr uint32_t COLD_BYTES_LARGE = TABLE_BYTES + SLOT_COUNT * WG_LARGE * 16;
 static_assert(COLD_AT_LARGE + SLOT_COUNT * WG_LARGE * 16 == LDS_BYTES_PER_CU && TABLE_BYTES <= COLD_AT_LARGE, "the large form's cold words end the unit's LDS");
+static_assert(LARGE_SCENE_ROOM_QUADS * 16 == COLD_AT_LARGE - TABLE_BYTES, "wpt_lds_places.h restates the room between the math tables and the cold words");
 template<uint32_t F>
 void launchPathtraceLarge(const KernelArgs& args, dim3 grid, size_t sceneLdsBytes, hipStream_t stream);
 #define WPT_PATHTRACE_LARGE_LAUNCHER(F, OCC, ORDERED)                                                                          \
     template<> void launchPathtraceLarge<(F)>(const KernelArgs& args, dim3 grid, size_t sceneLdsBytes, hipStream_t stream)     \
     {                                                                                                                          \
            \
-        if (COLD_BYTES_LARGE + sceneLdsBytes <= LDS_BYTES_PER_CU)                                                              \
-            launchMaybePooled(wpt_pathtrace_large<(F), OCC, ORDERED>, args, grid, LDS_BYTES_PER_CU, stream, WG_LARGE);         \
+        if (COLD_BYTES_LARGE + sceneLdsBytes > LDS_BYTES_PER_CU)                                                               \
+            return;                                                                                                            \
+                    \
+        const uint32_t hit = (args.materialsInLds >> LDS_HIT_DATA_SHIFT) & HIT_DATA_ALL;                                       \
+        if (hit == HIT_DATA_ALL)                                                                                               \
+            launchMaybePooled(wpt_pathtrace_large<(F), OCC, ORDERED, HIT_DATA_ALL>, args, grid, LDS_BYTES_PER_CU, stream, WG_LARGE); \
+        else if (hit == (HIT_DATA_RECORDS | HIT_DATA_HOTSPOTS))                                                                \
+            launchMaybePooled(wpt_pathtrace_large<(F), OCC, ORDERED, HIT_DATA_RECORDS | HIT_DATA_HOTSPOTS>, args, grid, LDS_BYTES_PER_CU, stream, WG_LARGE); \
+        else                                                                                                                   \
+            launchMaybePooled(wpt_pathtrace_large<(F), OCC, ORDERED, 0u>, args, grid, LDS_BYTES_PER_CU, stream, WG_LARGE);     \
     }
 void launchAdaptiveCost(const KernelArgs& args, hipStream_t stream);
 
diff --git a/wurblpt_amd/csrc/wpt_pathtrace_body.inc.h b/wurblpt_amd/csrc/wpt_pathtrace_body.inc.h
--- a/wurblpt_amd/csrc/wpt_pathtrace_body.inc.h
+++ b/wurblpt_amd/csrc/wpt_pathtrace_body.inc.h
@@ -29,6 +29,7 @@
     const wpt_params& par = args.par;
     const uint32_t nodeCount = sv.nodeCount;
     uint32_t orderedBase = 0, orderedStride = 0;
+    LdsHitData<HIT> hitData = {};
 
     if (LDSSCENE) {
         const uint32_t n4 = 2 * nodeCount, t4 = 3 * sv.triCount;
@@ -80,6 +81,54 @@
                     q.w = __uint_as_float(links.y);
                 }
                 ldsScene[orderedBase + k * orderedStride + at] = q;
+            }
+        }
+        if constexpr (LARGE) {
+            const uint32_t m = (args.materialsInLds & LDS_MATERIALS) ? sv.materialCount : 0u;
+            const uint32_t normals = args.materialsInLds >> LDS_HIT_NORMALS_SHIFT;
+            const HitDataPlaces places = hitDataPlaces(nodeCount, sv.triCount, m, normals, sv.hotspotCount, ORDERED);
+            hitData.scene = ldsScene;
+            hitData.corners = n4 + 2;
+            hitData.recordsAt = places.recordsAt;
+            hitData.hotspotsAt = places.hotspotsAt;
+            hitData.normalsAt = places.normalsAt;
+            if (HIT & places.parts & HIT_DATA_RECORDS) {
+                for (uint32_t i = threadIdx.x; i < HIT_RECORD_QUADS * sv.triCount; i += WGS) {
+                    const uint32_t tri = i / HIT_RECORD_QUADS, k = i - HIT_RECORD_QUADS * tri;
+                    float4 q;
+                    if (k < 6) {
+                        q = sv.triAttr[6 * tri + k];
+                    } else {
+                        const float4* g = sv.triGeom + 3 * tri;
+                        q = make_float4(g[0].w, g[1].w, g[2].w, 0.0f);
+                    }
+                    ldsScene[places.recordsAt + i] = q;
+                }
+            }
+            if (HIT & places.parts & HIT_DATA_HOTSPOTS) {
+                for (uint32_t i = threadIdx.x; i < HIT_HOTSPOT_QUADS * sv.hotspotCount; i += WGS) {
+                    const uint32_t spot = i / HIT_HOTSPOT_QUADS, k = i - HIT_HOTSPOT_QUADS * spot;
+                    const wpt_hotspot& hs = sv.hotspots[spot];
+                    float4 q;
+                    if (k == 0)
+                        q = sv.hotspotFace[spot];
+                    else if (k == 1)
+                        q = make_float4(__uint_as_float(hs.prim), __uint_as_float(hs.transform), hs.p0[0], hs.p0[1]);
+                    else if (k == 2)
+                        q = make_float4(hs.p0[2], hs.p1[0], hs.p1[1], hs.p1[2]);
+                    else if (k == 3)
+                        q = make_float4(hs.p2[0], hs.p2[1], hs.p2[2], 0.0f);
+                    else
+                        q = make_float4(hs.M[4 * (k - 4)], hs.M[4 * (k - 4) + 1], hs.M[4 * (k - 4) + 2], hs.M[4 * (k - 4) + 3]);
+                    ldsScene[places.hotspotsAt + i] = q;
+                }
+            }
+            if (HIT & places.parts & HIT_DATA_NORMALS) {
+                for (uint32_t i = threadIdx.x; i < HIT_NORMAL_QUADS * normals; i += WGS) {
+                    const uint32_t instance = i / HIT_NORMAL_QUADS, k = i - HIT_NORMAL_QUADS * instance;
+                    const float* N = sv.instances[instance].N;
+                    ldsScene[places.normalsAt + i] = make_float4(N[3 * k], N[3 * k + 1], N[3 * k + 2], 0.0f);
+                }
             }
         }
     }
@@ -96,7 +145,6 @@
         else
             return sv.triGeom[i];
     };
-
     uint32_t walkStart = 0;
     if constexpr (LDSSCENE)
         walkStart = reinterpret_cast<const uint2*>(sv.wideNodes)[nodeCount + 1].x;
@@ -555,7 +603,10 @@
             }
             if (state == S_SHADE) {
                 realOrigin();
-                afterBlock(blockShade<F, COUNT>(sv, par, tri4, ps, best, lc, cTrav != 0 ? (int)args.waitBelow : 0, args.bins));
+                if constexpr (LARGE)
+                    afterBlock(blockShade<F, COUNT>(sv, par, hitData, ps, best, lc, cTrav != 0 ? (int)args.waitBelow : 0, args.bins));
+                else
+                    afterBlock(blockShade<F, COUNT>(sv, par, tri4, ps, best, lc, cTrav != 0 ? (int)args.waitBelow : 0, args.bins));
             }
             if (COUNT)
                 sched[12] += (unsigned long long)(clock64() - tBlock);
@@ -570,7 +621,10 @@
             sec<COUNT>(lc, SEC_NEE_END_LIGHT, state == S_NEEEND && ps.rayKind == RAY_NEE_LIGHT && best.prim == ps.getW(SLOT_NEE));
             if (state == S_NEEEND) {
                 realOrigin();
-                afterBlock(blockNeeEnd<F>(sv, par, tri4, ps, best, args.bins));
+                if constexpr (LARGE)
+                    afterBlock(blockNeeEnd<F>(sv, par, hitData, ps, best, args.bins));
+                else
+                    afterBlock(blockNeeEnd<F>(sv, par, tri4, ps, best, args.bins));
             }
             if (COUNT)
                 sched[13] += (unsigned long long)(clock64() - tBlock);
diff --git a/wurblpt_amd/csrc/wpt_scene_layout.h b/wurblpt_amd/csrc/wpt_scene_layout.h
--- a/wurblpt_amd/csrc/wpt_scene_layout.h
+++ b/wurblpt_amd/csrc/wpt_scene_layout.h
@@ -9,6 +9,7 @@
 
 #include "../../include/wurblpt_hip.h"
 #include "wpt_fold.h"
+#include "wpt_lds_places.h"
 #include "wpt_rgl.h"
 
 namespace wptl {
@@ -364,6 +365,15 @@
     return true;
 }
 
+inline uint32_t normalsNamed(const wpt_scene_desc* desc)
+{
+    uint32_t named = 0;
+    for (uint32_t i = 0; i < desc->tri_count; i++)
+        if ((desc->tri_geom[i].flags & WPT_TRI_TRANSFORM) && desc->tri_geom[i].instance >= named)
+            named = desc->tri_geom[i].instance + 1;
+    return named;
+}
+
 inline std::vector<Quad> wideNodes(const wpt_scene_desc* desc, const std::vector<uint32_t>& triNew, uint32_t* worstStack = nullptr)
 {
     const uint32_t n = desc->node_count;
diff --git a/wurblpt_amd/device.py b/wurblpt_amd/device.py
--- a/wurblpt_amd/device.py
+++ b/wurblpt_amd/device.py
@@ -12,6 +12,8 @@
 
 WALK_WIDE, WALK_FULL_SHADOW, WALK_COUNT_PRODUCT, WALK_TRIANGLES_AS_GIVEN, WALK_SELECT_CORNERS, WALK_NO_FOLD, WALK_NO_BYPASS = 1, 2, 4, 8, 16, 32, 64
 WALK_SMALL_WORKGROUPS = 128
+WALK_HIT_DATA_IN_HBM = 256
+HIT_DATA_RECORDS, HIT_DATA_HOTSPOTS, HIT_DATA_NORMALS = 1, 2, 4
 SLICES_DECLINE_ODD = 0x100
 
 EXPORTS = list(_abi.FUNCTIONS)
@@ -660,6 +662,10 @@
     ordered = C.c_uint32()
     lanes = lib().wpt_kernel_workgroup(C.byref(ordered))
     return int(lanes), bool(ordered.value)
+
+
+def kernel_hit_data():
+    return int(lib().wpt_kernel_hit_data())
 
 
 def fold_plan(host_scene, with_words=False):
```

After: 1577 Msamples/s, median of 6. +1.4%, better.
